# codename0og/codename-rvc-fork-3

Measured on AMD Instinct MI355X. Metric: 48 kHz audio samples/sec end-to-end VC, higher is better.
Workload: dtype f32 (vocoder ResBlock convs and upsamplers, HuBERT, RMVPE's U-Net convs: fp32 operands as exact bf16x3 splits on the bf16 matrix cores -- six products of order <= 2^-16 per multiply-add, fp32 accumulate; everything else fp32 / fp64)

## Files before the change

codename-rvc-fork-3_amd/csrc/decoder.h:

```cpp
#pragma once
#include <atomic>
#include <map>
#include <mutex>
#include <string>
#include <vector>

#include "conv.h"

namespace rvc {

constexpr int MRF_MAX_DIM = 9;

struct HostTensor {
    std::vector<float> data;
    std::vector<int64_t> shape;
    int64_t numel() const { int64_t n = 1; for (auto s : shape) n *= s; return n; }
};

struct DevBuf {
    float *p = nullptr;
    ~DevBuf() { if (p) (void)hipFree(p); }
    int upload(const std::vector<float> &h) {
        if (p) { (void)hipFree(p); p = nullptr; }
        hipError_t e = hipMalloc((void **)&p, h.size() * sizeof(float));
        if (e == hipSuccess) e = hipMemcpy(p, h.data(), h.size() * sizeof(float), hipMemcpyHostToDevice);
        return e == hipSuccess ? 0 : fail("device upload of %zu floats failed: %s", h.size(), hipGetErrorString(e));
    }
};

struct DevBuf16 {
    uint16_t *p = nullptr;
    ~DevBuf16() { if (p) (void)hipFree(p); }
    int upload(const std::vector<uint16_t> &h) {
        if (p) { (void)hipFree(p); p = nullptr; }
        hipError_t e = hipMalloc((void **)&p, h.size() * sizeof(uint16_t));
        if (e == hipSuccess) e = hipMemcpy(p, h.data(), h.size() * sizeof(uint16_t), hipMemcpyHostToDevice);
        return e == hipSuccess ? 0 : fail("device upload of %zu bf16 values failed: %s", h.size(), hipGetErrorString(e));
    }
};

struct ConvW {
    DevBuf w, b;
    DevBuf16 w16;
    DevBuf wu;
    DevBuf16 wu16;
    DevBuf16 wx;
    DevBuf16 wd;
    DevBuf16 wh;
    int c_in = 0, c_out = 0, k = 0;
};

struct Stage {
    int c_in = 0, c_out = 0, rate = 0, ksize = 0, pad = 0, opad = 0;
    int taps = 0;
    bool interleave = false;
    int nc_stride = 0, nc_k = 0, nc_pad = 0;
    int vk = 0, vk_rows = 0;
    int64_t S = 0, P = 0;
    DevBuf w, b;
    DevBuf16 wub;
    int ub_vk = 0;
    int nc_rows = 0;
    DevBuf nc_w;
    std::vector<ConvW> c1, c2;
    std::vector<DevBuf16> pair;
    int pair_splits = 3;
};

constexpr int MAX_BRANCH_LANES = 7;
struct BranchLanes {
    hipStream_t side[MAX_BRANCH_LANES] = {};
    hipEvent_t fork = nullptr;
    hipEvent_t last[MAX_BRANCH_LANES + 1] = {};
    int n_side = 0;
    int create(int n);
    ~BranchLanes();
};

struct RefineStage {
    int ch_in = 0, ch_out = 0, rate = 0, down_c = 0, down_k = 0, down_stride = 0, down_pad = 0;
    DevBuf down_w, down_b;
    ConvW input_conv;
    DevBuf adain1[4], adain2[4];
    std::vector<ConvW> c1, c2;
    std::vector<DevBuf16> pair;
};

}

struct rvc_decoder {
    rvc_decoder_config cfg;
    std::map<std::string, rvc::HostTensor> host;
    bool finalized = false;
    int arithmetic = 0;
    int upp = 1;
    int dim = 1;
    float lin_w[rvc::MRF_MAX_DIM] = {0};
    float lin_b = 0.f;
    rvc::ConvW pre;
    rvc::DevBuf cond_w, cond_b;
    std::vector<rvc::Stage> stages;
    rvc::DevBuf post_w;
    float post_b = 0.f;
    int post_cin = 0;
    float merge_w = 1.f;
    rvc::DevBuf pre_w, pre_b;
    rvc::ConvW mel;
    std::vector<rvc::RefineStage> rstages;
    std::atomic<int> concurrency{0};
    std::atomic<int> branch_parallel{0};
    std::mutex lanes_mu;
    std::map<hipStream_t, rvc::BranchLanes *> lanes;
    ~rvc_decoder() { for (auto &kv : lanes) delete kv.second; }
    int tap_stage = -2;
    float *tap_dev = nullptr;
};


namespace rvc {
const HostTensor *find(const rvc_decoder *d, const std::string &name);
int need(const rvc_decoder *d, const std::string &name, const HostTensor **out, std::vector<int64_t> shape);
int build_conv(const rvc_decoder *d, const std::string &prefix, int c_out, int c_in, int k, bool bias, ConvW *out, bool as_bf16 = false);

int launch_unfold_src(const float *har, int batch, int64_t L, int64_t S, int64_t P, int k_valid, int k_rows, int64_t nq, float *V,
                      hipStream_t stream);
int launch_cond_bias(const float *pre_b, const float *cond_w, const float *cond_b, const float *g, int batch, int gin, int c0,
                     float *out, hipStream_t stream);
int launch_conv_post(const float *x, const float *w, float bias, int batch, int c_in, int64_t L, float slope, float *out,
                     hipStream_t stream);

int refine_finalize(rvc_decoder *d);
size_t refine_workspace_bytes(const rvc_decoder *d, int batch, int64_t T);
int refine_forward(rvc_decoder *d, const float *z_dev, const float *f0_dev, const float *g_dev, const rvc_decoder_noise *noise,
                   int batch, int64_t T, float *out_dev, void *workspace_dev, size_t workspace_bytes, hipStream_t stream);
}
```

codename-rvc-fork-3_amd/csrc/decoder.hip:

```cpp
#include <stdlib.h>

#include "decoder.h"

namespace rvc {


constexpr int CARRY_CHUNK = 4096;
__global__ void __launch_bounds__(256)
nsf_carry_kernel(const float *__restrict__ f0, int64_t T, float sr, float upp, float *__restrict__ carry) {
    __shared__ double pre[CARRY_CHUNK];
    __shared__ double part[257];
    __shared__ double cum_s;
    constexpr int SEG = CARRY_CHUNK / 256;
    const int64_t b = blockIdx.x;
    const float *f = f0 + b * T;
    float *c = carry + b * T;
    if (threadIdx.x == 0) {
        c[0] = 0.f;
        cum_s = 0.0;
    }
    for (int64_t base = 0; base + 1 < T; base += CARRY_CHUNK) {
        const int n = (int)((T - 1 - base) < CARRY_CHUNK ? (T - 1 - base) : CARRY_CHUNK);
        for (int i = threadIdx.x; i < n; i += 256) {
            const float last = __fmul_rn(__fdiv_rn(f[base + i], sr), upp);
            pre[i] = (double)__fsub_rn(fmodf(__fadd_rn(last, 0.5f), 1.0f), 0.5f);
        }
        __syncthreads();
        const int lo = threadIdx.x * SEG, hi = lo + SEG < n ? lo + SEG : n;
        double run = 0.0;
        for (int i = lo; i < hi; ++i) {
            run += pre[i];
            pre[i] = run;
        }
        part[threadIdx.x + 1] = run;
        __syncthreads();
        if (threadIdx.x == 0) {
            double cum = cum_s;
            part[0] = cum;
            for (int i = 1; i <= 256; ++i) {
                cum += part[i];
                part[i] = cum;
            }
            cum_s = cum;
        }
        __syncthreads();
        const double off = part[threadIdx.x];
        for (int i = lo; i < hi; ++i) pre[i] += off;
        __syncthreads();
        for (int i = threadIdx.x; i < n; i += 256) c[base + i + 1] = fmodf((float)pre[i], 1.0f);
        __syncthreads();
    }
}

__global__ void __launch_bounds__(256)
nsf_source_kernel(const float *__restrict__ f0, const float *__restrict__ carry, const float *__restrict__ randn,
                  int64_t T, int upp, float sr, float lin_w, float lin_b, float *__restrict__ har) {
    const int64_t L = T * upp;
    const int64_t b = blockIdx.y;
    const int64_t t = (int64_t)blockIdx.x * blockDim.x + threadIdx.x;
    if (t >= L) return;
    const int64_t i = t / upp;
    const int j = (int)(t - i * upp);
    const float f = f0[b * T + i];
    const float r = __fdiv_rn(f, sr);
    const float phase = __fadd_rn(__fmul_rn(r, (float)(j + 1)), carry[b * T + i]);
    const float sine = __fmul_rn(sinf(__fmul_rn(6.2831853071795864769f, phase)), 0.1f);
    const float uv = f > 0.f ? 1.f : 0.f;
    const float amp = __fadd_rn(__fmul_rn(uv, 0.003f), __fmul_rn(1.f - uv, (float)(0.1 / 3)));
    const float v = __fadd_rn(__fmul_rn(sine, uv), __fmul_rn(amp, randn[b * L + t]));
    har[b * L + t] = tanhf(__fadd_rn(__fmul_rn(v, lin_w), lin_b));
}


struct MrfSrcParams {
    const float *f0; const float *rand_ini; const float *randn; float *har;
    double *p1; double *p2; int *wraps; float *tot_unused;
    int64_t T; int upp; int dim; float sr;
    float lin_w[MRF_MAX_DIM]; float lin_b;
};

__device__ __forceinline__ float mrf_rad(float f0, int h, float sr) {
    const float fh = (h == 0) ? f0 : __fmul_rn(f0, (float)(h + 1));
    const float q = __fdiv_rn(fh, sr);
    return q - floorf(q);
}

constexpr int MRF_CH = 384;
constexpr int MRF_CS = MRF_CH + 1;

template <int PASS>
__device__ __forceinline__ double mrf_prefix_term(const MrfSrcParams &p, int b, int h, int64_t i) {
    const float rho = mrf_rad(p.f0[b * p.T + i], h, p.sr);
    if constexpr (PASS == 1) {
        if (i == 0) {
            const float r0 = __fadd_rn(rho, h == 0 ? 0.f : p.rand_ini[b * p.dim + h]);
            return (double)r0 + (double)(p.upp - 1) * (double)rho;
        }
        return (double)p.upp * (double)rho;
    } else {
        const float rho_m1 = __fadd_rn(rho, -1.0f);
        const int w = p.wraps[((int64_t)b * p.dim + h) * p.T + i];
        if (i == 0) {
            const float r0 = __fadd_rn(rho, h == 0 ? 0.f : p.rand_ini[b * p.dim + h]);
            return (double)r0 + (double)(p.upp - 1 - w) * (double)rho + (double)w * (double)rho_m1;
        }
        return (double)(p.upp - w) * (double)rho + (double)w * (double)rho_m1;
    }
}

template <int PASS>
__global__ void __launch_bounds__(256) mrf_prefix_kernel(MrfSrcParams p) {
    __shared__ double term[MRF_MAX_DIM * MRF_CS];
    const int b = blockIdx.x, tid = threadIdx.x;
    double *const P = (PASS == 1 ? p.p1 : p.p2) + (int64_t)b * p.dim * p.T;
    double cum = 0.0;
    for (int64_t base = 0; base < p.T; base += MRF_CH) {
        const int n = (int)(p.T - base < MRF_CH ? p.T - base : MRF_CH);
        for (int idx = tid; idx < p.dim * n; idx += 256) {
            const int h = idx / n, i = idx - h * n;
            term[h * MRF_CS + i] = mrf_prefix_term<PASS>(p, b, h, base + i);
        }
        __syncthreads();
        if (tid < p.dim) {
            double *row = term + tid * MRF_CS;
            int i = 0;
            for (; i + 8 <= n; i += 8) {
                double v[8];
#pragma unroll
                for (int j = 0; j < 8; ++j) v[j] = row[i + j];
#pragma unroll
                for (int j = 0; j < 8; ++j) {
                    row[i + j] = cum;
                    cum += v[j];
                }
            }
            for (; i < n; ++i) {
                const double v = row[i];
                row[i] = cum;
                cum += v;
            }
        }
        __syncthreads();
        for (int idx = tid; idx < p.dim * n; idx += 256) {
            const int h = idx / n, i = idx - h * n;
            P[(int64_t)h * p.T + base + i] = term[h * MRF_CS + i];
        }
        __syncthreads();
    }
}

__device__ __forceinline__ float mrf_tmp(const MrfSrcParams &p, const double *P1, int b, int h, int64_t i, int j) {
    const float rho = mrf_rad(p.f0[b * p.T + i], h, p.sr);
    double s = P1[i];
    if (i == 0) {
        const float r0 = __fadd_rn(rho, h == 0 ? 0.f : p.rand_ini[b * p.dim + h]);
        s += (double)r0 + (double)j * (double)rho;
    } else {
        s += (double)(j + 1) * (double)rho;
    }
    const float c = (float)s;
    return c - floorf(c);
}

__global__ void __launch_bounds__(64) mrf_wraps_kernel(MrfSrcParams p) {
    const int64_t i = blockIdx.x;
    const int h = blockIdx.y, b = blockIdx.z;
    const double *P1 = p.p1 + ((int64_t)b * p.dim + h) * p.T;
    int cnt = 0;
    for (int j = threadIdx.x; j < p.upp; j += 64) {
        if (i == 0 && j == 0) continue;
        const float cur = mrf_tmp(p, P1, b, h, i, j);
        const float prev = (j == 0) ? mrf_tmp(p, P1, b, h, i - 1, p.upp - 1) : mrf_tmp(p, P1, b, h, i, j - 1);
        if (__fsub_rn(cur, prev) < 0.f) ++cnt;
    }
#pragma unroll
    for (int o = 32; o > 0; o >>= 1) cnt += __shfl_xor(cnt, o);
    if (threadIdx.x == 0) p.wraps[((int64_t)b * p.dim + h) * p.T + i] = cnt;
}


__global__ void __launch_bounds__(256) mrf_source_kernel(MrfSrcParams p) {
    __shared__ int wave_tot[4];
    const int64_t i = blockIdx.x;
    const int b = blockIdx.y;
    const int lane = threadIdx.x & 63, wave = threadIdx.x >> 6;
    const int64_t L = p.T * p.upp;
    const float f = p.f0[b * p.T + i];
    const float uv = f > 0.f ? 1.f : 0.f;
    const float amp = __fadd_rn(__fmul_rn(uv, 0.003f), __fdiv_rn(__fmul_rn(1.f - uv, 0.1f), 3.f));
    const int n_it = (p.upp + 255) / 256;
    float out_acc[4] = {0.f, 0.f, 0.f, 0.f};
    for (int h = 0; h < p.dim; ++h) {
        const double *P1 = p.p1 + ((int64_t)b * p.dim + h) * p.T;
        const double P2 = p.p2[((int64_t)b * p.dim + h) * p.T + i];
        const float rho = mrf_rad(f, h, p.sr);
        const float rho_m1 = __fadd_rn(rho, -1.0f);
        const float r0 = (i == 0) ? __fadd_rn(rho, h == 0 ? 0.f : p.rand_ini[b * p.dim + h]) : rho;
        const float lw = p.lin_w[h];
        int base = 0;
#pragma unroll
        for (int it = 0; it < 4; ++it) {
            if (it < n_it) {
                const int j = it * 256 + threadIdx.x;
                int flag = 0;
                if (j < p.upp && !(i == 0 && j == 0)) {
                    const float cur = mrf_tmp(p, P1, b, h, i, j);
                    const float prev = (j == 0) ? mrf_tmp(p, P1, b, h, i - 1, p.upp - 1) : mrf_tmp(p, P1, b, h, i, j - 1);
                    flag = __fsub_rn(cur, prev) < 0.f ? 1 : 0;
                }
                int incl = flag;
#pragma unroll
                for (int o = 1; o < 64; o <<= 1) {
                    const int v = __shfl_up(incl, o);
                    if (lane >= o) incl += v;
                }
                __syncthreads();
                if (lane == 63) wave_tot[wave] = incl;
                __syncthreads();
                int before = base;
                for (int w = 0; w < wave; ++w) before += wave_tot[w];
                const int total = wave_tot[0] + wave_tot[1] + wave_tot[2] + wave_tot[3];
                const int wcount = before + incl;
                if (j < p.upp) {
                    double s = P2;
                    if (i == 0) s += (double)r0 + (double)(j - wcount) * (double)rho + (double)wcount * (double)rho_m1;
                    else s += (double)(j + 1 - wcount) * (double)rho + (double)wcount * (double)rho_m1;
                    const float c = (float)s;
                    const float sine = __fmul_rn(sinf(__fmul_rn(__fmul_rn(c, 2.f), 3.14159265358979323846f)), 0.1f);
                    const int64_t t = i * p.upp + j;
                    const float nz = p.randn[((int64_t)b * L + t) * p.dim + h];
                    const float v = __fadd_rn(__fmul_rn(sine, uv), __fmul_rn(amp, nz));
                    out_acc[it] = fmaf(v, lw, out_acc[it]);
                }
                base += total;
            }
        }
    }
#pragma unroll
    for (int it = 0; it < 4; ++it) {
        const int j = it * 256 + threadIdx.x;
        if (it < n_it && j < p.upp) p.har[(int64_t)b * L + i * p.upp + j] = tanhf(out_acc[it] + p.lin_b);
    }
}

__global__ void __launch_bounds__(256)
unfold_src_kernel(const float *__restrict__ har, int64_t L, int64_t S, int64_t P, int k_valid, int k_rows, int64_t nq,
                  float *__restrict__ V) {
    const int64_t q = (int64_t)blockIdx.x * blockDim.x + threadIdx.x;
    const int k = blockIdx.y;
    const int64_t b = blockIdx.z;
    if (q >= nq) return;
    float v = 0.f;
    if (k < k_valid) {
        const int64_t idx = q * S + k - P;
        if (idx >= 0 && idx < L) v = har[b * L + idx];
    }
    V[(b * k_rows + k) * nq + q] = v;
}

__global__ void __launch_bounds__(64)
cond_bias_kernel(const float *__restrict__ pre_b, const float *__restrict__ cond_w, const float *__restrict__ cond_b,
                 const float *__restrict__ g, int gin, int c0, float *__restrict__ out) {
    const int co = blockIdx.x, b = blockIdx.y, lane = threadIdx.x;
    float s = 0.f;
    for (int c = lane; c < gin; c += 64) s = fmaf(cond_w[(int64_t)co * gin + c], g[(int64_t)b * gin + c], s);
#pragma unroll
    for (int o = 32; o > 0; o >>= 1) s += __shfl_xor(s, o);
    if (lane == 0) out[(int64_t)b * c0 + co] = pre_b[co] + (cond_b[co] + s);
}

constexpr int POST_OUT = 4;
__global__ void __launch_bounds__(256)
conv_post_kernel(const float *__restrict__ x, const float *__restrict__ w, float bias, int c_in, int64_t L, float slope,
                 float *__restrict__ out) {
    const int64_t b = blockIdx.y;
    const int64_t t0 = ((int64_t)blockIdx.x * blockDim.x + threadIdx.x) * POST_OUT;
    const int64_t blk0 = (int64_t)blockIdx.x * blockDim.x * POST_OUT;
    const float *xb = x + b * c_in * L;
    const bool fast = (L & 3) == 0 && (c_in & 3) == 0 && blk0 >= 4 && blk0 + (int64_t)blockDim.x * POST_OUT + 4 <= L;
    if (fast) {
        float acc[POST_OUT];
#pragma unroll
        for (int o = 0; o < POST_OUT; ++o) acc[o] = bias;
        for (int c0 = 0; c0 < c_in; c0 += 4) {
            f32x4 q[4][3];
#pragma unroll
            for (int u = 0; u < 4; ++u) {
                const f32x4 *xr = reinterpret_cast<const f32x4 *>(xb + (int64_t)(c0 + u) * L + t0 - 4);
#pragma unroll
                for (int j = 0; j < 3; ++j) q[u][j] = xr[j];
            }
#pragma unroll
            for (int u = 0; u < 4; ++u) {
                float v[12];
#pragma unroll
                for (int j = 0; j < 3; ++j)
#pragma unroll
                    for (int e = 0; e < 4; ++e) v[4 * j + e] = q[u][j][e];
#pragma unroll
                for (int i = 1; i < 11; ++i) v[i] = lrelu(v[i], slope);
#pragma unroll
                for (int k = 0; k < 7; ++k) {
                    const float wk = w[(c0 + u) * 7 + k];
#pragma unroll
                    for (int o = 0; o < POST_OUT; ++o) acc[o] = fmaf(wk, v[o + k + 1], acc[o]);
                }
            }
        }
        *reinterpret_cast<f32x4 *>(out + b * L + t0) = f32x4{tanhf(acc[0]), tanhf(acc[1]), tanhf(acc[2]), tanhf(acc[3])};
        return;
    }
    if (t0 >= L) return;
    float acc[POST_OUT];
#pragma unroll
    for (int o = 0; o < POST_OUT; ++o) acc[o] = bias;
    for (int ci = 0; ci < c_in; ++ci) {
        const float *xr = xb + (int64_t)ci * L;
        float v[POST_OUT + 6];
#pragma unroll
        for (int i = 0; i < POST_OUT + 6; ++i) {
            const int64_t tt = t0 + i - 3;
            const int64_t tc = tt < 0 ? 0 : (tt >= L ? L - 1 : tt);
            const float raw = xr[tc];
            v[i] = (tt >= 0 && tt < L) ? lrelu(raw, slope) : 0.f;
        }
#pragma unroll
        for (int k = 0; k < 7; ++k) {
            const float wk = w[ci * 7 + k];
#pragma unroll
            for (int o = 0; o < POST_OUT; ++o) acc[o] = fmaf(wk, v[o + k], acc[o]);
        }
    }
#pragma unroll
    for (int o = 0; o < POST_OUT; ++o)
        if (t0 + o < L) out[b * L + t0 + o] = tanhf(acc[o]);
}

int launch_unfold_src(const float *har, int batch, int64_t L, int64_t S, int64_t P, int k_valid, int k_rows, int64_t nq, float *V,
                      hipStream_t stream) {
    hipLaunchKernelGGL(unfold_src_kernel, dim3((unsigned)ceil_div(nq, 256), k_rows, batch), dim3(256), 0, stream, har, L, S, P,
                       k_valid, k_rows, nq, V);
    RVC_LAUNCH_CHECK();
    return 0;
}

int launch_cond_bias(const float *pre_b, const float *cond_w, const float *cond_b, const float *g, int batch, int gin, int c0,
                     float *out, hipStream_t stream) {
    hipLaunchKernelGGL(cond_bias_kernel, dim3(c0, batch), dim3(64), 0, stream, pre_b, cond_w, cond_b, g, gin, c0, out);
    RVC_LAUNCH_CHECK();
    return 0;
}

int launch_conv_post(const float *x, const float *w, float bias, int batch, int c_in, int64_t L, float slope, float *out,
                     hipStream_t stream) {
    hipLaunchKernelGGL(conv_post_kernel, dim3((unsigned)ceil_div(L, 256 * POST_OUT), batch), dim3(256), 0, stream, x, w, bias, c_in, L, slope,
                       out);
    RVC_LAUNCH_CHECK();
    return 0;
}


}

using namespace rvc;

namespace rvc {
const HostTensor *find(const rvc_decoder *d, const std::string &name) {
    auto it = d->host.find(name);
    return it == d->host.end() ? nullptr : &it->second;
}

int need(const rvc_decoder *d, const std::string &name, const HostTensor **out, std::vector<int64_t> shape) {
    const HostTensor *t = find(d, name);
    if (!t) return fail("decoder: tensor '%s' was never set", name.c_str());
    if (t->shape != shape) {
        std::string got, want;
        for (auto s : t->shape) got += std::to_string(s) + ",";
        for (auto s : shape) want += std::to_string(s) + ",";
        return fail("decoder: tensor '%s' has shape [%s], expected [%s]", name.c_str(), got.c_str(), want.c_str());
    }
    *out = t;
    return 0;
}

int build_conv(const rvc_decoder *d, const std::string &prefix, int c_out, int c_in, int k, bool bias, ConvW *out, bool as_bf16) {
    const HostTensor *w, *b;
    if (need(d, prefix + ".weight", &w, {c_out, c_in, k})) return 1;
    std::vector<float> packed((size_t)c_out * c_in * k);
    for (int co = 0; co < c_out; ++co)
        for (int ci = 0; ci < c_in; ++ci)
            for (int t = 0; t < k; ++t)
                packed[((size_t)t * c_in + ci) * c_out + co] = w->data[((size_t)co * c_in + ci) * k + t];
    if (as_bf16) {
        std::vector<uint16_t> half(packed.size());
        for (size_t i = 0; i < packed.size(); ++i) half[i] = bf16_rne(packed[i]);
        if (out->w16.upload(half)) return 1;
    } else if (out->w.upload(packed)) {
        return 1;
    }
    if (c_in == c_out && c_out % 32 == 0 && wino_supported(k, 1)) {
        if (as_bf16) {
            std::vector<uint32_t> words;
            wino_pack_host_bf16(w->data.data(), c_out, c_in, k, &words);
            std::vector<uint16_t> halves(words.size() * 2);
            memcpy(halves.data(), words.data(), words.size() * 4);
            if (out->wu16.upload(halves)) return 1;
            if (convbf1_supported(c_out, k, 1) && convbf1_preferred(CB1_BF16W, c_out, k)) {
                std::vector<uint16_t> frags;
                convbf1_pack_host(CB1_BF16W, w->data.data(), c_out, k, &frags);
                if (out->wd.upload(frags)) return 1;
            }
            if (winobf_enabled() && winobf_supported(c_in, c_out, k, 1)) {
                std::vector<float> vals((size_t)c_out * c_in * k);
                for (size_t i = 0; i < vals.size(); ++i) {
                    const uint32_t bits = (uint32_t)bf16_rne(w->data[i]) << 16;
                    memcpy(&vals[i], &bits, 4);
                }
                std::vector<uint16_t> frags;
                winobf_pack_host(vals.data(), c_out, c_in, k, &frags);
                if (out->wx.upload(frags)) return 1;
            }
        } else {
            wino_pack_host(w->data.data(), c_out, c_in, k, &packed);
            if (out->wu.upload(packed)) return 1;
            if (d->arithmetic == 1 && convbf1_supported(c_out, k, 1) && convbf1_preferred(CB1_F16X2, c_out, k)) {
                std::vector<uint16_t> frags;
                if (!convbf1_pack_host(CB1_F16X2, w->data.data(), c_out, k, &frags) && out->wh.upload(frags)) return 1;
            }
            if (winobf_enabled() && winobf_supported(c_in, c_out, k, 1)) {
                std::vector<uint16_t> frags;
                winobf_pack_host(w->data.data(), c_out, c_in, k, &frags);
                if (out->wx.upload(frags)) return 1;
            }
        }
    }
    if (c_in != c_out && !as_bf16 && k >= 7 && winobf_enabled() && winobf_supported(c_in, c_out, k, 1)) {
        std::vector<uint16_t> frags;
        winobf_pack_host(w->data.data(), c_out, c_in, k, &frags);
        if (out->wx.upload(frags)) return 1;
    }
    if (bias) {
        if (need(d, prefix + ".bias", &b, {c_out})) return 1;
        if (out->b.upload(b->data)) return 1;
    }
    out->c_in = c_in; out->c_out = c_out; out->k = k;
    return 0;
}
}

extern "C" int rvc_decoder_create(const rvc_decoder_config *cfg, rvc_decoder **out) {
    if (!cfg || !out) return fail("rvc_decoder_create: null pointer");
    if (cfg->kind != RVC_DEC_NSF && cfg->kind != RVC_DEC_MRF && cfg->kind != RVC_DEC_REFINE)
        return fail("rvc_decoder_create: unknown decoder kind %d", cfg->kind);
    if (cfg->n_ups < 1 || cfg->n_ups > 8) return fail("rvc_decoder_create: n_ups out of range");
    if (cfg->n_res_kernels < 1 || cfg->n_res_kernels > 4 || cfg->n_res_dilations < 1 || cfg->n_res_dilations > 4)
        return fail("rvc_decoder_create: resblock configuration out of range");
    if (cfg->weight_storage != 0 && cfg->weight_storage != 1) return fail("rvc_decoder_create: weight_storage must be 0 (fp32) or 1 (bf16)");
    if (cfg->weight_storage == 1 && cfg->kind == RVC_DEC_REFINE)
        return fail("rvc_decoder_create: bf16 weight storage is built for the NSF / MRF decoders (BASELINE cfg 4), not RefineGAN");
    if (cfg->in_channels % 8 || cfg->upsample_initial_channel % (32 << cfg->n_ups))
        return fail("rvc_decoder_create: channel counts must keep every stage a multiple of 32");
    rvc_decoder *d = new rvc_decoder();
    d->cfg = *cfg;
    d->upp = 1;
    for (int i = 0; i < cfg->n_ups; ++i) d->upp *= cfg->upsample_rates[i];
    if (d->upp > 1024) { delete d; return fail("rvc_decoder_create: prod(upsample_rates) > 1024"); }
    d->dim = cfg->kind == RVC_DEC_MRF ? 9 : 1;
    *out = d;
    return 0;
}

extern "C" int rvc_decoder_set_arithmetic(rvc_decoder *dec, int mode) {
    if (!dec) return fail("rvc_decoder_set_arithmetic: null decoder");
    if (mode != 0 && mode != 1) return fail("rvc_decoder_set_arithmetic: mode must be 0 (exact) or 1 (fp16 pairs), got %d", mode);
    if (dec->finalized) return fail("rvc_decoder_set_arithmetic: decoder already finalized (the tap slabs are packed at finalize)");
    if (mode == 1 && dec->cfg.weight_storage == 1)
        return fail("rvc_decoder_set_arithmetic: fp16 pairs are for fp32 taps; a weight_storage = 1 handle's bf16 taps already cost three products");
    dec->arithmetic = mode;
    return 0;
}

extern "C" int rvc_decoder_set_tensor(rvc_decoder *dec, const char *name, const float *data_host, const int64_t *shape,
                                      int ndim) {
    if (!dec || !name || !data_host || !shape || ndim < 1 || ndim > 4) return fail("rvc_decoder_set_tensor: bad argument");
    if (dec->finalized) return fail("rvc_decoder_set_tensor: decoder already finalized");
    HostTensor t;
    t.shape.assign(shape, shape + ndim);
    const int64_t n = t.numel();
    if (n <= 0) return fail("rvc_decoder_set_tensor: empty tensor '%s'", name);
    t.data.assign(data_host, data_host + n);
    dec->host[name] = std::move(t);
    return 0;
}

extern "C" int rvc_decoder_finalize(rvc_decoder *d) {
    if (!d) return fail("rvc_decoder_finalize: null decoder");
    if (d->finalized) return 0;
    if (d->cfg.kind == RVC_DEC_REFINE) {
        if (refine_finalize(d)) return 1;
        d->host.clear();
        d->finalized = true;
        return 0;
    }
    const rvc_decoder_config &c = d->cfg;
    const bool mrf = c.kind == RVC_DEC_MRF;
    const HostTensor *t;
    if (need(d, "m_source.l_linear.weight", &t, {1, d->dim})) return 1;
    for (int h = 0; h < d->dim; ++h) d->lin_w[h] = t->data[h];
    if (need(d, "m_source.l_linear.bias", &t, {1})) return 1;
    d->lin_b = t->data[0];
    const int c0 = c.upsample_initial_channel;
    if (build_conv(d, "conv_pre", c0, c.in_channels, 7, true, &d->pre)) return 1;
    if (need(d, "cond.weight", &t, {c0, c.gin_channels, 1})) return 1;
    if (d->cond_w.upload(t->data)) return 1;
    if (need(d, "cond.bias", &t, {c0})) return 1;
    if (d->cond_b.upload(t->data)) return 1;
    d->stages.clear();
    d->stages.resize(c.n_ups);
    for (int i = 0; i < c.n_ups; ++i) {
        Stage &s = d->stages[i];
        s.c_in = c0 >> i;
        s.c_out = c0 >> (i + 1);
        s.rate = c.upsample_rates[i];
        s.ksize = c.upsample_kernel_sizes[i];
        s.pad = (s.rate % 2 == 0) ? (s.ksize - s.rate) / 2 : s.rate / 2 + s.rate % 2;
        s.opad = s.rate % 2;
        s.taps = (s.ksize + s.rate - 1) / s.rate;
        if (s.taps > 2) return fail("decoder: upsample kernel %d with rate %d needs %d polyphase taps (max 2)", s.ksize, s.rate, s.taps);
        if (s.taps < 2) s.taps = 2;
        int stride_f0 = 1;
        for (int j = i + 1; j < c.n_ups; ++j) stride_f0 *= c.upsample_rates[j];
        s.nc_stride = stride_f0;
        s.nc_k = stride_f0 == 1 ? 1 : stride_f0 * 2 - stride_f0 % 2;
        s.nc_pad = stride_f0 == 1 ? 0 : (s.nc_k - stride_f0) / 2;
        s.vk = (s.rate - 1) * s.nc_stride + s.nc_k;
        s.vk_rows = (s.vk + 7) / 8 * 8;
        s.S = (int64_t)s.rate * s.nc_stride;
        s.P = (int64_t)s.pad * s.nc_stride + s.nc_pad;
        static const int nc_sep_env = knob("RVC_NC_SEPARATE", 1);
        const bool nc_separate = nc_sep_env && s.vk_rows * 2 >= s.c_in;
        if (nc_separate) {
            s.nc_rows = (s.nc_k + 7) / 8 * 8;
            s.vk = 0;
            s.vk_rows = 0;
        }

        const std::string up = (mrf ? "upsamples." : "ups.") + std::to_string(i);
        const std::string nc = "noise_convs." + std::to_string(i);
        const HostTensor *uw, *ub, *nw, *nb;
        if (need(d, up + ".weight", &uw, {s.c_in, s.c_out, s.ksize})) return 1;
        if (need(d, up + ".bias", &ub, {s.c_out})) return 1;
        if (need(d, nc + ".weight", &nw, {s.c_out, 1, s.nc_k})) return 1;
        if (need(d, nc + ".bias", &nb, {s.c_out})) return 1;
        const int ctot = s.c_in + s.vk_rows;
        const int m_total = s.rate * s.c_out;
        s.interleave = s.rate % 2 == 0;
        auto mrow = [&](int ph, int co) { return s.interleave ? co * s.rate + ph : ph * s.c_out + co; };
        std::vector<float> packed((size_t)s.taps * ctot * m_total, 0.f);
        for (int tp = 0; tp < s.taps; ++tp) {
            const int j = s.taps - 1 - tp;
            for (int ci = 0; ci < s.c_in; ++ci)
                for (int ph = 0; ph < s.rate; ++ph) {
                    const int kk = ph + j * s.rate;
                    if (kk >= s.ksize) continue;
                    for (int co = 0; co < s.c_out; ++co)
                        packed[((size_t)tp * ctot + ci) * m_total + mrow(ph, co)] =
                            uw->data[((size_t)ci * s.c_out + co) * s.ksize + kk];
                }
        }
        const int tp0 = s.taps - 1;
        for (int kq = 0; kq < s.vk; ++kq)
            for (int ph = 0; ph < s.rate; ++ph) {
                const int k = kq - ph * s.nc_stride;
                if (k < 0 || k >= s.nc_k) continue;
                for (int co = 0; co < s.c_out; ++co)
                    packed[((size_t)tp0 * ctot + s.c_in + kq) * m_total + mrow(ph, co)] = nw->data[(size_t)co * s.nc_k + k];
            }
        if (s.w.upload(packed)) return 1;
        std::vector<float> bias(s.c_out);
        for (int co = 0; co < s.c_out; ++co) bias[co] = ub->data[co] + nb->data[co];
        {
            static const int ups_bf = knob("RVC_UPS_BF", 1);
            const int k_n = s.nc_rows > 0 ? 0 : s.nc_k;
            const int vk = upsbf_fold_noise(k_n) ? (s.rate - 1) * s.nc_stride + k_n : 0;
            if (ups_bf && s.opad == 0 && s.rate * s.c_out >= 128 && upsbf_supported(s.c_in, s.c_out, s.rate, s.ksize, vk)) {
                std::vector<uint16_t> frags;
                upsbf_pack_host(uw->data.data(), k_n ? nw->data.data() : nullptr, bias.data(), s.c_in, s.c_out, s.rate, s.ksize, vk, k_n, s.nc_stride, &frags);
                if (s.wub.upload(frags)) return 1;
                s.ub_vk = vk;
            }
        }
        if (s.nc_rows) {
            std::vector<float> ncw((size_t)s.nc_rows * s.c_out, 0.f);
            for (int k = 0; k < s.nc_k; ++k)
                for (int co = 0; co < s.c_out; ++co) ncw[(size_t)k * s.c_out + co] = nw->data[(size_t)co * s.nc_k + k];
            if (s.nc_w.upload(ncw)) return 1;
        }
        if (s.b.upload(bias)) return 1;

        const int nb_ = c.n_res_kernels * c.n_res_dilations;
        s.c1 = std::vector<ConvW>(nb_);
        s.c2 = std::vector<ConvW>(nb_);
        s.pair = std::vector<DevBuf16>(nb_);
        for (int m = 0; m < c.n_res_kernels; ++m)
            for (int j = 0; j < c.n_res_dilations; ++j) {
                std::string p1, p2;
                if (mrf) {
                    const std::string base = "mrfs." + std::to_string(i) + "." + std::to_string(m) + ".layers." + std::to_string(j);
                    p1 = base + ".conv1";
                    p2 = base + ".conv2";
                } else {
                    const std::string base = "resblocks." + std::to_string(i * c.n_res_kernels + m);
                    p1 = base + ".convs1." + std::to_string(j);
                    p2 = base + ".convs2." + std::to_string(j);
                }
                const int k = c.res_kernel_sizes[m];
                const bool b16 = c.weight_storage == 1 && (k == 3 || k == 7 || k == 11);
                if (build_conv(d, p1, s.c_out, s.c_out, k, true, &s.c1[m * c.n_res_dilations + j], b16)) return 1;
                if (build_conv(d, p2, s.c_out, s.c_out, k, true, &s.c2[m * c.n_res_dilations + j], b16)) return 1;
                const int nts = b16 ? 1 : 3;
                if (resblock_bf_enabled() && resblock_bf_supported(s.c_out, k, 1) && resblock_bf_preferred(s.c_out, k, nts)) {
                    const HostTensor *w1, *w2;
                    if (need(d, p1 + ".weight", &w1, {s.c_out, s.c_out, k}) || need(d, p2 + ".weight", &w2, {s.c_out, s.c_out, k})) return 1;
                    std::vector<uint16_t> frags;
                    resblock_bf_pack_host(w1->data.data(), w2->data.data(), s.c_out, k, &frags, nts);
                    s.pair_splits = nts;
                    if (s.pair[m * c.n_res_dilations + j].upload(frags)) return 1;
                }
            }
    }
    d->post_cin = c0 >> c.n_ups;
    if (need(d, "conv_post.weight", &t, {1, d->post_cin, 7})) return 1;
    if (d->post_w.upload(t->data)) return 1;
    d->post_b = 0.f;
    if (mrf) {
        if (need(d, "conv_post.bias", &t, {1})) return 1;
        d->post_b = t->data[0];
    }
    d->host.clear();
    d->finalized = true;
    return 0;
}

extern "C" int rvc_decoder_destroy(rvc_decoder *dec) {
    delete dec;
    return 0;
}

extern "C" int rvc_decoder_upp(const rvc_decoder *dec) { return dec ? dec->upp : 0; }

namespace {
struct Carve {
    size_t off = 0;
    size_t take(size_t bytes) { size_t o = off; off += align_up(bytes, 256); return o; }
};
struct Layout {
    size_t har, carry, biasp, V, p1, p2, wraps, buf[2 + 2 * (MAX_BRANCH_LANES + 1)], total;
    int n_buf;
    int64_t max_cl;
};
constexpr int64_t BRANCH_PARALLEL_MAX_ELEMS = (int64_t)3 * 256 * 128 * 256;
int branch_lanes_wanted(const rvc_decoder *d) {
    const int nk = d->cfg.n_res_kernels, want = d->branch_parallel.load(std::memory_order_relaxed);
    const int most = nk - 1 < MAX_BRANCH_LANES ? nk - 1 : MAX_BRANCH_LANES;
    return want < 0 || want > most ? most : want;
}
Layout make_layout(const rvc_decoder *d, int batch, int64_t T) {
    Layout l;
    Carve c;
    const int64_t L = T * d->upp;
    l.har = c.take((size_t)batch * L * 4);
    l.carry = c.take((size_t)batch * T * 4);
    l.biasp = c.take((size_t)batch * d->cfg.upsample_initial_channel * 4);
    int64_t len = T, max_cl = (int64_t)d->cfg.upsample_initial_channel * T, max_v = 0;
    for (const Stage &s : d->stages) {
        const int64_t nq = len + 1;
        max_v = std::max<int64_t>(max_v, (int64_t)s.vk_rows * nq);
        len = (len - 1) * s.rate - 2 * s.pad + s.ksize + s.opad;
        max_v = std::max<int64_t>(max_v, (int64_t)s.nc_rows * len);
        max_cl = std::max<int64_t>(max_cl, (int64_t)s.c_out * len);
    }
    l.V = c.take((size_t)batch * max_v * 4);
    const size_t scan = d->dim > 1 ? (size_t)batch * d->dim * T : 0;
    l.p1 = c.take(scan * 8);
    l.p2 = c.take(scan * 8);
    l.wraps = c.take(scan * 4);
    l.n_buf = 2 + 2 * (branch_lanes_wanted(d) + 1);
    for (int i = 0; i < l.n_buf; ++i) l.buf[i] = c.take((size_t)batch * max_cl * 4);
    l.total = c.off;
    l.max_cl = max_cl;
    return l;
}
}

extern "C" int rvc_decoder_workspace_bytes(const rvc_decoder *dec, int batch, int64_t n_frames, size_t *bytes) {
    if (!dec || !bytes || batch <= 0 || n_frames <= 0) return fail("rvc_decoder_workspace_bytes: bad argument");
    if (!dec->finalized) return fail("rvc_decoder_workspace_bytes: decoder not finalized");
    *bytes = dec->cfg.kind == RVC_DEC_REFINE ? refine_workspace_bytes(dec, batch, n_frames) : make_layout(dec, batch, n_frames).total;
    return 0;
}

extern "C" int rvc_decoder_set_tap(rvc_decoder *dec, int stage, float *tap_dev) {
    if (!dec) return fail("rvc_decoder_set_tap: null decoder");
    dec->tap_stage = tap_dev ? stage : -2;
    dec->tap_dev = tap_dev;
    return 0;
}

int rvc::BranchLanes::create(int n) {
    n_side = n;
    for (int i = 0; i < n; ++i) RVC_HIP(hipStreamCreateWithFlags(&side[i], hipStreamNonBlocking));
    RVC_HIP(hipEventCreateWithFlags(&fork, hipEventDisableTiming));
    for (int i = 0; i <= MAX_BRANCH_LANES; ++i) RVC_HIP(hipEventCreateWithFlags(&last[i], hipEventDisableTiming));
    return 0;
}
rvc::BranchLanes::~BranchLanes() {
    for (int i = 0; i < n_side; ++i) if (side[i]) { (void)hipStreamSynchronize(side[i]); (void)hipStreamDestroy(side[i]); }
    if (fork) (void)hipEventDestroy(fork);
    for (int i = 0; i <= MAX_BRANCH_LANES; ++i) if (last[i]) (void)hipEventDestroy(last[i]);
}

namespace {
int lanes_for(rvc_decoder *d, hipStream_t stream, int n_side, BranchLanes **out) {
    std::lock_guard<std::mutex> g(d->lanes_mu);
    BranchLanes *&l = d->lanes[stream];
    if (l && l->n_side != n_side) { delete l; l = nullptr; }
    if (!l) {
        l = new BranchLanes();
        if (l->create(n_side)) { delete l; l = nullptr; return 1; }
    }
    *out = l;
    return 0;
}
}

extern "C" int rvc_decoder_set_branch_parallel(rvc_decoder *dec, int side_streams) {
    if (!dec) return fail("rvc_decoder_set_branch_parallel: null decoder");
    dec->branch_parallel.store(side_streams, std::memory_order_relaxed);
    return 0;
}

extern "C" int rvc_decoder_set_concurrency_hint(rvc_decoder *dec, int utterances_in_flight) {
    if (!dec) return fail("rvc_decoder_set_concurrency_hint: null decoder");
    if (utterances_in_flight < 0) return fail("rvc_decoder_set_concurrency_hint: negative hint %d", utterances_in_flight);
    dec->concurrency.store(utterances_in_flight, std::memory_order_relaxed);
    return 0;
}

extern "C" int rvc_decoder_forward(rvc_decoder *d, const float *z_dev, const float *f0_dev, const float *g_dev,
                                   const rvc_decoder_noise *noise, int batch, int64_t T, float *out_dev,
                                   void *workspace_dev, size_t workspace_bytes, void *stream_) {
    if (!d || !z_dev || !f0_dev || !g_dev || !noise || !out_dev || !workspace_dev) return fail("rvc_decoder_forward: null pointer");
    ConcurrencyScope scope(d->concurrency.load(std::memory_order_relaxed));
    if (!d->finalized) return fail("rvc_decoder_forward: decoder not finalized");
    if (batch <= 0 || T <= 0) return fail("rvc_decoder_forward: empty batch");
    if (!noise->src_randn_dev) return fail("rvc_decoder_forward: src_randn_dev is required");
    if (d->cfg.kind == RVC_DEC_REFINE)
        return refine_forward(d, z_dev, f0_dev, g_dev, noise, batch, T, out_dev, workspace_dev, workspace_bytes, (hipStream_t)stream_);
    const rvc_decoder_config &c = d->cfg;
    const bool mrf = c.kind == RVC_DEC_MRF;
    if (mrf && !noise->src_rand_dev) return fail("rvc_decoder_forward: src_rand_dev is required for the MRF decoder");
    hipStream_t stream = (hipStream_t)stream_;
    const Layout lay = make_layout(d, batch, T);
    if (workspace_bytes < lay.total) return fail("rvc_decoder_forward: workspace too small (%zu < %zu)", workspace_bytes, lay.total);
    char *ws = (char *)workspace_dev;
    float *har = (float *)(ws + lay.har);
    float *carry = (float *)(ws + lay.carry);
    float *biasp = (float *)(ws + lay.biasp);
    float *V = (float *)(ws + lay.V);
    float *buf[2 + 2 * (MAX_BRANCH_LANES + 1)];
    for (int i = 0; i < lay.n_buf; ++i) buf[i] = (float *)(ws + lay.buf[i]);
    const int n_side = (lay.n_buf - 4) / 2;
    BranchLanes *lanes = nullptr;
    if (n_side > 0 && lanes_for(d, stream, n_side, &lanes)) return 1;
    const int64_t L = T * d->upp;
    const float sr = (float)c.sample_rate;

    if (!mrf) {
        hipLaunchKernelGGL(nsf_carry_kernel, dim3(batch), dim3(256), 0, stream, f0_dev, T, sr, (float)d->upp, carry);
        RVC_LAUNCH_CHECK();
        hipLaunchKernelGGL(nsf_source_kernel, dim3((unsigned)ceil_div(L, 256), batch), dim3(256), 0, stream, f0_dev, carry,
                           noise->src_randn_dev, T, d->upp, sr, d->lin_w[0], d->lin_b, har);
        RVC_LAUNCH_CHECK();
    } else {
        MrfSrcParams sp;
        sp.f0 = f0_dev; sp.rand_ini = noise->src_rand_dev; sp.randn = noise->src_randn_dev; sp.har = har;
        sp.p1 = (double *)(ws + lay.p1); sp.p2 = (double *)(ws + lay.p2); sp.wraps = (int *)(ws + lay.wraps);
        sp.tot_unused = nullptr;
        sp.T = T; sp.upp = d->upp; sp.dim = d->dim; sp.sr = sr;
        for (int h = 0; h < MRF_MAX_DIM; ++h) sp.lin_w[h] = d->lin_w[h];
        sp.lin_b = d->lin_b;
        hipLaunchKernelGGL(mrf_prefix_kernel<1>, dim3(batch), dim3(256), 0, stream, sp);
        RVC_LAUNCH_CHECK();
        hipLaunchKernelGGL(mrf_wraps_kernel, dim3((unsigned)T, d->dim, batch), dim3(64), 0, stream, sp);
        RVC_LAUNCH_CHECK();
        hipLaunchKernelGGL(mrf_prefix_kernel<3>, dim3(batch), dim3(256), 0, stream, sp);
        RVC_LAUNCH_CHECK();
        hipLaunchKernelGGL(mrf_source_kernel, dim3((unsigned)T, batch), dim3(256), 0, stream, sp);
        RVC_LAUNCH_CHECK();
    }
    if (d->tap_stage == -1 && d->tap_dev)
        RVC_HIP(hipMemcpyAsync(d->tap_dev, har, (size_t)batch * L * 4, hipMemcpyDeviceToDevice, stream));

    const int c0 = c.upsample_initial_channel;
    hipLaunchKernelGGL(cond_bias_kernel, dim3(c0, batch), dim3(64), 0, stream, d->pre.b.p, d->cond_w.p, d->cond_b.p, g_dev,
                       c.gin_channels, c0, biasp);
    RVC_LAUNCH_CHECK();
    float *cur = buf[0];
    {
        ConvParams p;
        p.x1 = z_dev; p.c1 = c.in_channels; p.slope1 = 1.f; p.x1_bstride = (int64_t)c.in_channels * T; p.l_in = T;
        p.w = d->pre.w.p; p.bias = biasp; p.bias_bstride = c0;
        p.y = cur; p.y_bstride = (int64_t)c0 * T; p.m_total = c0; p.c_out = c0; p.n_cols = T; p.l_out = T;
        p.kw = 7; p.dil = 1; p.padl = 3; p.batch = batch;
        if (launch_conv(p, stream)) return 1;
    }

    int64_t len = T;
    const int nd = c.n_res_dilations, nk = c.n_res_kernels;
    for (int i = 0; i < c.n_ups; ++i) {
        Stage &s = d->stages[i];
        const int64_t nq = len + 1;
        const int64_t len_out = (len - 1) * s.rate - 2 * s.pad + s.ksize + s.opad;
        float *X = buf[1];
        if (s.wub.p && fits_2gib((int64_t)s.c_in * len, 4) && fits_2gib((int64_t)s.c_out * len_out, 4) && fits_2gib(L, 4)) {
            if (launch_upsbf(cur, har, L, s.wub.p, s.b.p, X, batch, s.c_in, s.c_out, len, len_out, s.rate, s.ksize, s.pad, s.ub_vk, s.S, s.P, 0.1f, stream))
                return 1;
        } else {
        if (s.vk_rows) {
            hipLaunchKernelGGL(unfold_src_kernel, dim3((unsigned)ceil_div(nq, 256), s.vk_rows, batch), dim3(256), 0, stream, har, L,
                               s.S, s.P, s.vk, s.vk_rows, nq, V);
            RVC_LAUNCH_CHECK();
        }
        {
            ConvParams p;
            p.x1 = cur; p.c1 = s.c_in; p.slope1 = 0.1f; p.x1_bstride = (int64_t)s.c_in * len;
            if (s.vk_rows) { p.x2 = V; p.c2 = s.vk_rows; p.slope2 = 1.f; p.x2_bstride = (int64_t)s.vk_rows * nq; }
            p.l_in = len;
            p.w = s.w.p; p.bias = s.b.p;
            p.y = X; p.y_bstride = (int64_t)s.c_out * len_out;
            p.m_total = s.rate * s.c_out; p.c_out = s.c_out; p.n_cols = nq; p.l_out = len_out;
            p.kw = s.taps; p.dil = 1; p.padl = s.taps - 1;
            p.up_stride = s.rate; p.up_pad = s.pad; p.up_interleave = s.interleave ? 1 : 0; p.batch = batch;
            p.l_in2 = nq;
            if (launch_conv(p, stream)) return 1;
        }
        }
        if (s.nc_rows) {
            hipLaunchKernelGGL(unfold_src_kernel, dim3((unsigned)ceil_div(len_out, 256), s.nc_rows, batch), dim3(256), 0, stream, har,
                               L, (int64_t)s.nc_stride, (int64_t)s.nc_pad, s.nc_k, s.nc_rows, len_out, V);
            RVC_LAUNCH_CHECK();
            ConvParams p;
            p.x1 = V; p.c1 = s.nc_rows; p.slope1 = 1.f; p.x1_bstride = (int64_t)s.nc_rows * len_out; p.l_in = len_out;
            p.w = s.nc_w.p; p.accin = X; p.y = X; p.y_bstride = (int64_t)s.c_out * len_out;
            p.m_total = s.c_out; p.c_out = s.c_out; p.n_cols = len_out; p.l_out = len_out;
            p.kw = 1; p.dil = 1; p.padl = 0; p.batch = batch;
            if (launch_conv(p, stream)) return 1;
        }
        len = len_out;
        const int64_t bs = (int64_t)s.c_out * len;
        const bool short_stage = (int64_t)batch * bs <= BRANCH_PARALLEL_MAX_ELEMS;
        const bool par = lanes && short_stage;
        if (par) {
            RVC_HIP(hipEventRecord(lanes->fork, stream));
            for (int q = 0; q < n_side; ++q) RVC_HIP(hipStreamWaitEvent(lanes->side[q], lanes->fork, 0));
        }
        const hipStream_t main_stream = stream;
        for (int r = 0; r < nk; ++r) {
            const int m = r;
            const bool first_branch = r == 0, final_branch = r + 1 == nk;
            const int k = c.res_kernel_sizes[m];
            const float *xin = X;
            const int off = nk - 1 - n_side;
            const int lane = par && r > off ? r - off : 0, lane_prev = par && r - 1 > off ? r - 1 - off : 0;
            const hipStream_t stream = lane > 0 ? lanes->side[lane - 1] : main_stream;
            float *const Y = buf[2 + 2 * lane], *const T1 = buf[3 + 2 * lane];
            auto before_last = [&]() -> int {
                if (par && r > 0 && lane_prev != lane) RVC_HIP(hipStreamWaitEvent(stream, lanes->last[r - 1], 0));
                return 0;
            };
            auto after_last = [&]() -> int {
                if (par) RVC_HIP(hipEventRecord(lanes->last[r], stream));
                return 0;
            };
            bool f16_branch = true;
            for (int j = 0; j < nd; ++j) f16_branch = f16_branch && s.c1[m * nd + j].wh.p && s.c2[m * nd + j].wh.p;
            if (s.pair[m * nd].p && !f16_branch && resblock_bf_fits(s.c_out, len)) {
                for (int j = 0; j < nd; ++j) {
                    const bool last = j + 1 == nd;
                    float *yout = last ? cur : (j % 2 == 0 ? Y : T1);
                    const float *acc_in = (last && !first_branch) ? cur : nullptr;
                    const float scale = (last && final_branch) ? 1.f / (float)nk : 1.f;
                    if (last && before_last()) return 1;
                    if (launch_resblock_bf(xin, s.pair[m * nd + j].p, s.c1[m * nd + j].b.p, s.c2[m * nd + j].b.p, acc_in, yout, batch,
                                           s.c_out, len, k, c.res_dilations[j], 0.1f, scale, stream, s.pair_splits))
                        return 1;
                    xin = yout;
                }
                if (after_last()) return 1;
                continue;
            }
            if (resblock_layer_supported(s.c_out, k) && !s.c1[m * nd].w16.p) {
                for (int j = 0; j < nd; ++j) {
                    const bool last = j + 1 == nd;
                    float *yout = last ? cur : (j % 2 == 0 ? Y : T1);
                    const float *acc_in = (last && !first_branch) ? cur : nullptr;
                    const float scale = (last && final_branch) ? 1.f / (float)nk : 1.f;
                    if (last && before_last()) return 1;
                    if (launch_resblock_layer(xin, s.c1[m * nd + j].w.p, s.c1[m * nd + j].b.p, s.c2[m * nd + j].w.p,
                                              s.c2[m * nd + j].b.p, acc_in, yout, batch, s.c_out, len, k, c.res_dilations[j], 0.1f,
                                              scale, stream))
                        return 1;
                    xin = yout;
                }
                if (after_last()) return 1;
                continue;
            }
            for (int j = 0; j < nd; ++j) {
                const int dil = c.res_dilations[j];
                ConvParams p;
                p.x1 = xin; p.c1 = s.c_out; p.slope1 = 0.1f; p.x1_bstride = bs; p.l_in = len;
                p.w = s.c1[m * nd + j].w.p; p.w16 = s.c1[m * nd + j].w16.p; p.bias = s.c1[m * nd + j].b.p; p.w_wino = s.c1[m * nd + j].wu.p; p.w_winobf = s.c1[m * nd + j].wx.p; p.w_direct1 = s.c1[m * nd + j].wd.p; p.w_f16x2 = s.c1[m * nd + j].wh.p;
                p.w_wino16 = reinterpret_cast<const uint32_t *>(s.c1[m * nd + j].wu16.p);
                p.y = T1; p.y_bstride = bs; p.m_total = s.c_out; p.c_out = s.c_out; p.n_cols = len; p.l_out = len;
                p.kw = k; p.dil = dil; p.padl = (k - 1) / 2 * dil; p.batch = batch;
                if (launch_conv(p, stream)) return 1;
                ConvParams q;
                q.x1 = T1; q.c1 = s.c_out; q.slope1 = 0.1f; q.x1_bstride = bs; q.l_in = len;
                q.w = s.c2[m * nd + j].w.p; q.w16 = s.c2[m * nd + j].w16.p; q.bias = s.c2[m * nd + j].b.p; q.w_wino = s.c2[m * nd + j].wu.p; q.w_winobf = s.c2[m * nd + j].wx.p; q.w_direct1 = s.c2[m * nd + j].wd.p; q.w_f16x2 = s.c2[m * nd + j].wh.p;
                q.w_wino16 = reinterpret_cast<const uint32_t *>(s.c2[m * nd + j].wu16.p);
                q.res = xin;
                q.y_bstride = bs; q.m_total = s.c_out; q.c_out = s.c_out; q.n_cols = len; q.l_out = len;
                q.kw = k; q.dil = 1; q.padl = (k - 1) / 2;  q.batch = batch;
                if (j + 1 < nd) {
                    q.y = Y;
                } else {
                    q.y = cur;
                    q.accin = first_branch ? nullptr : cur;
                    q.out_scale = final_branch ? 1.f / (float)nk : 1.f;
                    if (before_last()) return 1;
                }
                if (launch_conv(q, stream)) return 1;
                xin = Y;
            }
            if (after_last()) return 1;
        }
        if (par) RVC_HIP(hipStreamWaitEvent(main_stream, lanes->last[nk - 1], 0));
        if (d->tap_stage == i && d->tap_dev)
            RVC_HIP(hipMemcpyAsync(d->tap_dev, cur, (size_t)batch * bs * 4, hipMemcpyDeviceToDevice, stream));
    }
    if (len != L) return fail("decoder: internal length mismatch (%lld vs %lld)", (long long)len, (long long)L);
    return launch_conv_post(cur, d->post_w.p, d->post_b, batch, d->post_cin, L, 0.01f, out_dev, stream);
}
```

codename-rvc-fork-3_amd/rvc_amd/_native.py:

```python
from __future__ import annotations

import ctypes
import threading
import os
from ctypes import POINTER, c_char_p, c_float, c_int, c_int64, c_size_t, c_void_p

import torch

_HERE = os.path.dirname(os.path.abspath(__file__))
LIB_PATH = os.path.join(_HERE, "_lib", "librvc_amd.so")
if os.environ.get("RVC_AMD_LIB"):
    LIB_PATH = os.path.abspath(os.environ["RVC_AMD_LIB"])
    print(f"[rvc_amd] RVC_AMD_LIB: loading {LIB_PATH} instead of the product library", flush=True)


class NativeError(RuntimeError):
    pass


if not os.path.isfile(LIB_PATH):
    raise ImportError(
        f"{LIB_PATH} is missing: build it with `python -c 'import __graft_entry__ as g; g.build()'` "
        "(hipcc --offload-arch=gfx950).  rvc_amd has no fallback path without its HIP library.")

_lib = ctypes.CDLL(LIB_PATH)


class DecoderConfig(ctypes.Structure):
    _fields_ = [
        ("kind", c_int), ("sample_rate", c_int), ("in_channels", c_int), ("upsample_initial_channel", c_int),
        ("gin_channels", c_int), ("n_ups", c_int), ("upsample_rates", c_int * 8), ("upsample_kernel_sizes", c_int * 8),
        ("n_res_kernels", c_int), ("res_kernel_sizes", c_int * 4), ("res_dilations", c_int * 4),
        ("n_res_dilations", c_int), ("weight_storage", c_int),
    ]


class DecoderNoise(ctypes.Structure):
    _fields_ = [("src_rand_dev", c_void_p), ("src_randn_dev", c_void_p), ("adain_randn_dev", c_void_p)]


SYMBOLS = {
    "rvc_abi_version": (c_int, []),
    "rvc_last_error": (c_char_p, []),
    "rvc_knn_index_aux_bytes": (c_int, [c_int64, c_int, POINTER(c_size_t)]),
    "rvc_knn_index_build": (c_int, [c_void_p, c_int64, c_int, c_void_p, c_size_t, c_void_p]),
    "rvc_knn_set_mode": (c_int, [c_int]),
    "rvc_knn_rank_candidates": (c_int, [c_void_p, c_void_p, c_int64, c_int, c_void_p, c_int64, c_void_p, c_int, c_int, c_void_p,
                                        c_void_p, c_void_p]),
    "rvc_knn_workspace_bytes": (c_int, [c_int64, c_int64, c_int, c_int, POINTER(c_size_t)]),
    "rvc_knn_search": (c_int, [c_void_p, c_void_p, c_int64, c_int, c_void_p, c_int64, c_int, c_void_p, c_void_p,
                               c_void_p, c_size_t, c_void_p]),
    "rvc_knn_blend": (c_int, [c_void_p, c_int, c_void_p, c_void_p, c_void_p, c_int64, c_int, c_float, c_void_p,
                              c_void_p]),
    "rvc_logmel_workspace_bytes": (c_int, [c_int, c_int64, POINTER(c_size_t)]),
    "rvc_logmel_rmvpe": (c_int, [c_void_p, c_int, c_int64, c_void_p, c_int64, c_void_p, c_size_t, c_void_p]),
    "rvc_mel_create": (c_int, [c_int, c_int, c_int, c_int, c_float, c_float, c_void_p, c_int, POINTER(c_void_p)]),
    "rvc_mel_destroy": (c_int, [c_void_p]),
    "rvc_mel_frames": (c_int, [c_void_p, c_int64, POINTER(c_int64)]),
    "rvc_mel_workspace_bytes": (c_int, [c_void_p, c_int, c_int64, POINTER(c_size_t)]),
    "rvc_mel_forward": (c_int, [c_void_p, c_void_p, c_int, c_int64, c_void_p, c_void_p, c_void_p, c_size_t, c_void_p]),
    "rvc_resample_poly_f64": (c_int, [c_void_p, c_int64, c_int, c_int, c_void_p, c_int64, c_void_p, c_int64, c_void_p]),
    "rvc_filtfilt_workspace_bytes": (c_int, [c_int64, POINTER(c_size_t)]),
    "rvc_filtfilt_order5": (c_int, [c_void_p, c_int64, c_void_p, c_void_p, c_void_p, c_size_t, c_void_p]),
    "rvc_bigru_workspace_bytes": (c_int, [c_int, POINTER(c_size_t)]),
    "rvc_bigru_forward": (c_int, [c_void_p, c_void_p, c_void_p, c_void_p, c_int, c_int64, c_int, c_void_p, c_size_t,
                                  c_void_p]),
    "rvc_bigru_status": (c_int, [c_void_p, c_int, POINTER(c_int), c_void_p]),
    "rvc_bigru_set_spin_limit": (c_int, [ctypes.c_uint]),
    "rvc_attention_workspace_bytes": (c_int, [c_int, c_int64, c_int, c_int, POINTER(c_size_t)]),
    "rvc_attention_qkv_f32": (c_int, [c_void_p, c_void_p, c_void_p, c_void_p, c_int, c_int64, c_int, c_int, c_float,
                                      c_void_p, c_size_t, c_void_p]),
    "rvc_bias_relu_add_f32": (c_int, [c_void_p, c_void_p, c_void_p, c_void_p, c_int, c_int, c_int64, c_int, c_void_p]),
    "rvc_gate_tanh_sigmoid_f32": (c_int, [c_void_p, c_void_p, c_int, c_int, c_int64, c_void_p]),
    "rvc_rownorm_gelu_f32": (c_int, [c_void_p, c_void_p, c_void_p, c_void_p, c_int, c_int, c_int64, ctypes.c_float, c_void_p]),
    "rvc_set_concurrency_hint": (c_int, [c_int]),
    "rvc_decoder_create": (c_int, [POINTER(DecoderConfig), POINTER(c_void_p)]),
    "rvc_decoder_set_tensor": (c_int, [c_void_p, c_char_p, c_void_p, POINTER(c_int64), c_int]),
    "rvc_decoder_finalize": (c_int, [c_void_p]),
    "rvc_decoder_destroy": (c_int, [c_void_p]),
    "rvc_decoder_upp": (c_int, [c_void_p]),
    "rvc_decoder_workspace_bytes": (c_int, [c_void_p, c_int, c_int64, POINTER(c_size_t)]),
    "rvc_decoder_forward": (c_int, [c_void_p, c_void_p, c_void_p, c_void_p, POINTER(DecoderNoise), c_int, c_int64,
                                    c_void_p, c_void_p, c_size_t, c_void_p]),
    "rvc_decoder_set_tap": (c_int, [c_void_p, c_int, c_void_p]),
    "rvc_decoder_set_concurrency_hint": (c_int, [c_void_p, c_int]),
    "rvc_decoder_set_branch_parallel": (c_int, [c_void_p, c_int]),
    "rvc_posconv_bf16x3_weight_bytes": (c_int, [c_int, c_int, c_int, POINTER(c_size_t)]),
    "rvc_posconv_bf16x3_pack_weight": (c_int, [c_void_p, c_int, c_int, c_int, c_void_p, c_void_p]),
    "rvc_posconv_gelu_bf16x3": (c_int, [c_void_p, c_void_p, c_void_p, c_void_p, c_int64, c_int, c_int, c_int, c_int, c_void_p]),
    "rvc_hubert_conv0_workspace_bytes": (c_int, [c_int, POINTER(c_size_t)]),
    "rvc_hubert_conv0_frames_bf16x3": (c_int, [c_void_p, c_int64, c_void_p, c_int, c_int, c_int, c_void_p, c_void_p, c_float, c_void_p,
                                               c_size_t, c_void_p, c_int64, c_void_p]),
    "rvc_conv1d_frames_bf16x3": (c_int, [c_void_p, c_int64, c_int64, c_int, c_int, c_int, c_void_p, c_void_p, c_void_p, c_void_p, c_int64,
                                         c_int, c_int, c_void_p]),
    "rvc_conv1d_pack_weight": (c_int, [c_void_p, c_int, c_int, c_int, c_void_p, c_void_p]),
    "rvc_conv1d_forward": (c_int, [c_void_p, c_void_p, c_void_p, c_void_p, c_void_p, c_void_p, c_int, c_int, c_int,
                                   c_int64, c_int, c_int, c_float, c_float, c_void_p]),
    "rvc_conv1d_wino_pack_weight": (c_int, [c_void_p, c_int, c_int, c_int, c_void_p, c_void_p]),
    "rvc_conv1d_wino_forward": (c_int, [c_void_p, c_void_p, c_void_p, c_void_p, c_void_p, c_void_p, c_int, c_int, c_int,
                                        c_int64, c_int, c_int, c_float, c_float, c_void_p]),
    "rvc_conv1d_winobf_weight_bytes": (c_int, [c_int, c_int, c_int, POINTER(c_size_t)]),
    "rvc_conv1d_winobf_pack_weight": (c_int, [c_void_p, c_int, c_int, c_int, c_void_p, c_void_p]),
    "rvc_conv1d_winobf_forward": (c_int, [c_void_p, c_void_p, c_void_p, c_void_p, c_void_p, c_void_p, c_int, c_int, c_int,
                                          c_int64, c_int, c_int, c_float, c_float, c_void_p]),
    "rvc_resblock_bf16x3_weight_bytes": (c_int, [c_int, c_int, POINTER(c_size_t)]),
    "rvc_resblock_bf16x3_pack_weight": (c_int, [c_void_p, c_void_p, c_int, c_int, c_void_p, c_void_p]),
    "rvc_resblock_bf16x3_forward": (c_int, [c_void_p, c_void_p, c_void_p, c_void_p, c_void_p, c_void_p, c_int, c_int, c_int64, c_int,
                                            c_int, c_float, c_float, c_void_p]),
    "rvc_resblock_bf16w_weight_bytes": (c_int, [c_int, c_int, POINTER(c_size_t)]),
    "rvc_resblock_bf16w_pack_weight": (c_int, [c_void_p, c_void_p, c_int, c_int, c_void_p, c_void_p]),
    "rvc_resblock_bf16w_forward": (c_int, [c_void_p, c_void_p, c_void_p, c_void_p, c_void_p, c_void_p, c_int, c_int, c_int64, c_int,
                                           c_int, c_float, c_float, c_void_p]),
    "rvc_resblock_bf16x3_set_enabled": (c_int, [c_int]),
    "rvc_upsample_bf16x3_weight_bytes": (c_int, [c_int, c_int, c_int, c_int, c_int, c_int, POINTER(c_size_t)]),
    "rvc_upsample_bf16x3_pack_weight": (c_int, [c_void_p, c_void_p, c_void_p, c_int, c_int, c_int, c_int, c_int, c_int, c_void_p, c_void_p]),
    "rvc_upsample_bf16x3_forward": (c_int, [c_void_p, c_void_p, c_int64, c_void_p, c_void_p, c_void_p, c_int, c_int, c_int, c_int64, c_int, c_int,
                                            c_int, c_int, c_int, c_int, c_float, c_void_p]),
    "rvc_conv1d_f16x2_weight_bytes": (c_int, [c_int, c_int, POINTER(c_size_t)]),
    "rvc_conv1d_f16x2_pack_weight": (c_int, [c_void_p, c_int, c_int, c_void_p, c_void_p]),
    "rvc_conv1d_f16x2_forward": (c_int, [c_void_p, c_void_p, c_void_p, c_void_p, c_void_p, c_void_p, c_int, c_int, c_int64, c_int,
                                         c_int, c_float, c_float, c_void_p]),
    "rvc_decoder_set_arithmetic": (c_int, [c_void_p, c_int]),
    "rvc_conv1d_bf16w_weight_bytes": (c_int, [c_int, c_int, POINTER(c_size_t)]),
    "rvc_conv1d_bf16w_pack_weight": (c_int, [c_void_p, c_int, c_int, c_void_p, c_void_p]),
    "rvc_conv1d_bf16w_forward": (c_int, [c_void_p, c_void_p, c_void_p, c_void_p, c_void_p, c_void_p, c_int, c_int, c_int64, c_int,
                                         c_int, c_float, c_float, c_void_p]),
    "rvc_gemm_bf16x3_weight_bytes": (c_int, [c_int, c_int, POINTER(c_size_t)]),
    "rvc_gemm_bf16x3_pack_weight": (c_int, [c_void_p, c_int, c_int, c_int, c_void_p, c_void_p]),
    "rvc_linear_bf16x3": (c_int, [c_void_p, c_void_p, c_void_p, c_void_p, c_void_p, c_int64, c_int, c_int, c_int, c_void_p]),
    "rvc_conv1d_bf16x3": (c_int, [c_void_p, c_void_p, c_void_p, c_void_p, c_int, c_int, c_int, c_int64, c_int, c_int, c_int, c_int,
                                  c_void_p]),
    "rvc_split_rows_bf16x3": (c_int, [c_void_p, c_void_p, c_int64, c_int64, c_int, c_void_p]),
    "rvc_linear_bf16x3_presplit": (c_int, [c_void_p, c_void_p, c_void_p, c_void_p, c_void_p, c_int64, c_int64, c_int, c_int, c_int, c_int,
                                           c_void_p]),
    "rvc_bias_residual_layernorm_bf16x3": (c_int, [c_void_p, c_int, c_void_p, c_void_p, c_void_p, c_void_p, c_float, c_void_p, c_void_p,
                                                   c_int64, c_int64, c_int, c_void_p]),
    "rvc_conv2d_packed_floats": (c_int, [c_int, c_int, c_int, c_int, POINTER(c_size_t)]),
    "rvc_conv2d_pack_weight": (c_int, [c_void_p, c_int, c_int, c_int, c_int, c_void_p, c_void_p]),
    "rvc_conv2d_workspace_bytes": (c_int, [c_int, c_int, c_int, c_int, c_int, c_int, c_int, POINTER(c_size_t)]),
    "rvc_conv2d_bf16x3_supported": (c_int, [c_int, c_int, c_int, c_int]),
    "rvc_conv2d_bf16x3_weight_bytes": (c_int, [c_int, c_int, c_int, c_int, POINTER(c_size_t)]),
    "rvc_conv2d_bf16x3_pack_weight": (c_int, [c_void_p, c_int, c_int, c_int, c_int, c_void_p, c_void_p]),
    "rvc_conv2d_bf16x3_workspace_bytes": (c_int, [c_int, c_int, c_int, c_int, c_int, POINTER(c_size_t)]),
    "rvc_conv2d_bf16x3_forward": (c_int, [c_void_p, c_void_p, c_void_p, c_void_p, c_void_p, c_int, c_int, c_int, c_int, c_int, c_int,
                                          c_void_p, c_size_t, c_void_p]),
    "rvc_conv2d_forward": (c_int, [c_void_p, c_void_p, c_void_p, c_void_p, c_void_p, c_int, c_int, c_int, c_int, c_int, c_int,
                                   c_int, c_int, c_void_p, c_size_t, c_void_p]),
    "rvc_comm_unique_id": (c_int, [c_void_p]),
    "rvc_comm_create": (c_int, [c_void_p, c_int, c_int, POINTER(c_void_p)]),
    "rvc_comm_destroy": (c_int, [c_void_p]),
    "rvc_comm_info": (c_int, [c_void_p, POINTER(c_int), POINTER(c_int), POINTER(c_int), c_char_p, c_size_t]),
    "rvc_index_broadcast": (c_int, [c_void_p, c_void_p, c_size_t, c_int, c_void_p]),
    "rvc_checksum64": (c_int, [c_void_p, c_size_t, c_void_p, c_void_p]),
    "rvc_glu_dwconv_silu_f32": (c_int, [c_void_p, c_void_p, c_void_p, c_void_p, c_int64, c_int, c_int, c_void_p]),
    "rvc_layernorm_rows_f32": (c_int, [c_void_p, c_void_p, c_void_p, c_float, c_void_p, c_int64, c_int, c_void_p]),
    "rvc_groupnorm_workspace_bytes": (c_int, [c_int, c_int64, c_int, POINTER(c_size_t)]),
    "rvc_groupnorm_lrelu_f32": (c_int, [c_void_p, c_void_p, c_void_p, c_int, c_float, c_float, c_void_p, c_int, c_int64, c_void_p,
                                        c_size_t, c_void_p]),
    "rvc_fcpe_decode_f32": (c_int, [c_void_p, c_void_p, c_int, c_int, c_float, c_float, c_void_p, c_void_p, c_int64, c_void_p]),
    "rvc_kmeans_workspace_bytes": (c_int, [c_int64, c_int64, c_int, POINTER(c_size_t)]),
    "rvc_kmeans_assign": (c_int, [c_void_p, c_int64, c_int, c_void_p, c_int64, c_void_p, c_void_p, c_void_p, c_size_t, c_void_p]),
    "rvc_kmeans_update": (c_int, [c_void_p, c_int64, c_int, c_void_p, c_void_p, c_int64, c_void_p, c_void_p, c_void_p, c_size_t,
                                  c_void_p]),
}

for _name, (_res, _args) in SYMBOLS.items():
    _fn = getattr(_lib, _name)
    _fn.restype = _res
    _fn.argtypes = _args

ABI_VERSION = 4
if _lib.rvc_abi_version() != ABI_VERSION:
    raise ImportError(f"librvc_amd.so ABI {_lib.rvc_abi_version()} != {ABI_VERSION}: rebuild it")


def _check(rc: int, what: str):
    if rc != 0:
        raise NativeError(f"{what}: {_lib.rvc_last_error().decode(errors='replace')}")


def _stream() -> int:
    return torch.cuda.current_stream().cuda_stream


def _dev_f32(t: torch.Tensor, name: str) -> torch.Tensor:
    if not t.is_cuda:
        raise NativeError(f"{name} must live in HBM (got a {t.device} tensor); the HIP path has no CPU fallback")
    if t.dtype != torch.float32:
        raise NativeError(f"{name} must be float32, got {t.dtype}")
    return t.contiguous()


class _Workspace:

    def __init__(self):
        self._buf = {}
        self._lock = threading.Lock()

    def get(self, tag: str, nbytes: int, device) -> torch.Tensor:
        key = (tag, str(device), torch.cuda.current_stream(device).cuda_stream)
        with self._lock:
            buf = self._buf.get(key)
            if buf is None or buf.numel() < nbytes:
                buf = torch.empty(max(nbytes, 256), dtype=torch.uint8, device=device)
                self._buf[key] = buf
        return buf


_ws = _Workspace()


def knn_index_build(index: torch.Tensor) -> torch.Tensor:
    index = _dev_f32(index, "index")
    need = c_size_t()
    _check(_lib.rvc_knn_index_aux_bytes(index.shape[0], index.shape[1], ctypes.byref(need)), "rvc_knn_index_aux_bytes")
    aux = torch.empty(need.value, dtype=torch.uint8, device=index.device)
    _check(_lib.rvc_knn_index_build(index.data_ptr(), index.shape[0], index.shape[1], aux.data_ptr(), aux.numel(), _stream()),
           "rvc_knn_index_build")
    return aux


knn_index_norms = knn_index_build


def knn_set_mode(mode: int) -> None:
    _check(_lib.rvc_knn_set_mode(int(mode)), "rvc_knn_set_mode")


def knn_search(index: torch.Tensor, aux: torch.Tensor, queries: torch.Tensor, k: int = 8):
    index, queries = _dev_f32(index, "index"), _dev_f32(queries, "queries")
    if not aux.is_cuda or aux.dtype != torch.uint8:
        raise NativeError("aux must be the uint8 HBM blob returned by knn_index_build")
    nq = queries.shape[0]
    d2 = torch.empty((nq, k), dtype=torch.float32, device=index.device)
    ids = torch.empty((nq, k), dtype=torch.int64, device=index.device)
    if nq == 0:
        return d2, ids
    need = c_size_t()
    _check(_lib.rvc_knn_workspace_bytes(index.shape[0], nq, index.shape[1], k, ctypes.byref(need)), "rvc_knn_workspace_bytes")
    ws = _ws.get("knn", need.value, index.device)
    _check(_lib.rvc_knn_search(index.data_ptr(), aux.data_ptr(), index.shape[0], index.shape[1], queries.data_ptr(),
                               nq, k, d2.data_ptr(), ids.data_ptr(), ws.data_ptr(), ws.numel(), _stream()),
           "rvc_knn_search")
    return d2, ids


def knn_rank_candidates(index: torch.Tensor, aux: torch.Tensor, queries: torch.Tensor, cand: torch.Tensor, k: int = 8):
    index, queries = _dev_f32(index, "index"), _dev_f32(queries, "queries")
    if not cand.is_cuda or cand.dtype != torch.int32 or cand.dim() != 2 or cand.shape[0] != queries.shape[0]:
        raise NativeError("cand must be an int32 HBM tensor [n_queries, cap]")
    cand = cand.contiguous()
    nq = queries.shape[0]
    d2 = torch.empty((nq, k), dtype=torch.float32, device=index.device)
    ids = torch.empty((nq, k), dtype=torch.int64, device=index.device)
    _check(_lib.rvc_knn_rank_candidates(index.data_ptr(), aux.data_ptr(), index.shape[0], index.shape[1], queries.data_ptr(), nq,
                                        cand.data_ptr(), cand.shape[1], k, d2.data_ptr(), ids.data_ptr(), _stream()),
           "rvc_knn_rank_candidates")
    return d2, ids


def knn_blend(index: torch.Tensor, feats: torch.Tensor, d2: torch.Tensor, ids: torch.Tensor, index_rate: float):
    index, feats, d2 = _dev_f32(index, "index"), _dev_f32(feats, "feats"), _dev_f32(d2, "d2")
    ids = ids.contiguous()
    out = torch.empty_like(feats)
    _check(_lib.rvc_knn_blend(index.data_ptr(), index.shape[1], feats.data_ptr(), d2.data_ptr(), ids.data_ptr(),
                              feats.shape[0], d2.shape[1], float(index_rate), out.data_ptr(), _stream()),
           "rvc_knn_blend")
    return out


def _kmeans_workspace(n_rows: int, n_centroids: int, dim: int, device) -> torch.Tensor:
    need = c_size_t()
    _check(_lib.rvc_kmeans_workspace_bytes(n_rows, n_centroids, dim, ctypes.byref(need)), "rvc_kmeans_workspace_bytes")
    return _ws.get("kmeans", need.value, device)


def kmeans_assign(x: torch.Tensor, centroids: torch.Tensor):
    x, centroids = _dev_f32(x, "x"), _dev_f32(centroids, "centroids")
    if x.dim() != 2 or centroids.dim() != 2 or x.shape[1] != centroids.shape[1]:
        raise NativeError(f"x {tuple(x.shape)} and centroids {tuple(centroids.shape)} must be [n, d] and [k, d]")
    n, d = x.shape
    ids = torch.empty(n, dtype=torch.int32, device=x.device)
    d2 = torch.empty(n, dtype=torch.float32, device=x.device)
    if n == 0:
        return ids, d2
    ws = _kmeans_workspace(n, centroids.shape[0], d, x.device)
    _check(_lib.rvc_kmeans_assign(x.data_ptr(), n, d, centroids.data_ptr(), centroids.shape[0], ids.data_ptr(), d2.data_ptr(),
                                  ws.data_ptr(), ws.numel(), _stream()), "rvc_kmeans_assign")
    return ids, d2


def kmeans_update(x: torch.Tensor, order: torch.Tensor, offsets: torch.Tensor, old: torch.Tensor) -> torch.Tensor:
    x, old = _dev_f32(x, "x"), _dev_f32(old, "old")
    n, d = x.shape
    k = old.shape[0]
    if (not order.is_cuda or order.dtype != torch.int32 or order.numel() != n or not offsets.is_cuda
            or offsets.dtype != torch.int64 or offsets.numel() != k + 1 or old.shape[1] != d):
        raise NativeError("order must be an int32 HBM tensor [n], offsets an int64 HBM tensor [k + 1], old [k, d]")
    if n == 0:
        return old.clone()
    order, offsets = order.contiguous(), offsets.contiguous()
    out = torch.empty_like(old)
    ws = _kmeans_workspace(n, k, d, x.device)
    _check(_lib.rvc_kmeans_update(x.data_ptr(), n, d, order.data_ptr(), offsets.data_ptr(), k, old.data_ptr(), out.data_ptr(),
                                  ws.data_ptr(), ws.numel(), _stream()), "rvc_kmeans_update")
    return out


def knn_roofline_report(n_rows: int, n_queries: int, dim: int, seconds: float, peak_hbm_gbs: float,
                        peak_f32_tflops: float, peak_f16_tflops: float, traffic=None, traffic_source=None) -> dict:
    screened = n_queries > 64 and n_rows >= 16384 and dim % 256 == 0
    stream = n_queries <= 64
    q_tile = 256 if screened else (32 if stream else 128)
    passes = -(-n_queries // q_tile)
    bytes_8d = passes * n_rows * dim * 4.0
    bytes_moved = passes * n_rows * dim * (2.0 if screened else 4.0) + (8.0 * n_queries * dim * 4 if screened else 0.0)
    flops = 2.0 * n_queries * n_rows * dim
    mfma_peak = peak_f16_tflops if screened else peak_f32_tflops
    hbm_gbs = bytes_moved / seconds / 1e9
    mfma_tf = flops / seconds / 1e12
    bound = "hbm" if stream else "mfma"
    out = {"kernel": ("knn_screen_kernel<false> (sample) + knn_select_kernel + knn_screen_kernel<true> (main, fp16 MFMA) + "
                      "knn_finalize_kernel (exact fp32 re-scoring)" if screened else
                      ("knn_direct_kernel" if stream else "knn_partial_kernel") + " + knn_finalize_kernel"),
           "regime": "fp16-screened, exact re-scoring" if screened else ("fp32 streaming" if stream else "fp32 GEMM"),
           "shape": f"{n_queries} queries x {n_rows} rows x {dim}", "bound": bound, "query_tile": q_tile, "passes": passes,
           "bytes_per_pass_8d": n_rows * dim * 4}
    if bound == "hbm":
        out.update({"achieved": round(hbm_gbs, 1), "peak": peak_hbm_gbs, "unit": "GB/s", "frac": round(hbm_gbs / peak_hbm_gbs, 4),
                    "frac_is": "physical: bytes the pass reads (n_rows x dim x 4) / search time / HBM peak"})
    else:
        out.update({"achieved": round(mfma_tf, 2), "peak": mfma_peak, "unit": "TFLOP/s", "frac": round(mfma_tf / mfma_peak, 4),
                    "frac_is": "2 x queries x rows x dim / search time / the dense " + ("fp16" if screened else "fp32") + " MFMA peak "
                               "(round 5 and earlier printed an HBM fraction here: now hbm_frac_physical / frac_8d)"})
    out.update({"bytes_moved_per_search": bytes_moved,
                "hbm_gbs_physical": round(hbm_gbs, 1), "hbm_frac_physical": round(hbm_gbs / peak_hbm_gbs, 4),
                "achieved_8d": round(bytes_8d / seconds / 1e9, 1), "frac_8d": round(bytes_8d / seconds / 1e9 / peak_hbm_gbs, 4),
                "frac_8d_is": "SURVEY 8d's formula (passes x n_rows x dim x 4 B / t / 8 TB/s): fp32 bytes the screened kernel never reads -- a footnote",
                "traffic": traffic, "traffic_source": traffic_source,
                "mfma_tflops": round(mfma_tf, 2), "mfma_frac": round(mfma_tf / mfma_peak, 4),
                "mfma_peak_used": "fp16 dense 2500 TF" if screened else "fp32 157.3 TF",
                "avg_search_ms": round(seconds * 1e3, 4)})
    return out


def logmel_rmvpe(audio: torch.Tensor, pad_to: int = 32) -> tuple[torch.Tensor, int]:
    audio = _dev_f32(audio, "audio")
    b, n = audio.shape
    t = n // 160 + 1
    t_pad = pad_to * ((t - 1) // pad_to + 1) if pad_to > 1 else t
    mel = torch.empty((b, 128, t_pad), dtype=torch.float32, device=audio.device)
    need = c_size_t()
    _check(_lib.rvc_logmel_workspace_bytes(b, n, ctypes.byref(need)), "rvc_logmel_workspace_bytes")
    ws = _ws.get("logmel", need.value, audio.device)
    _check(_lib.rvc_logmel_rmvpe(audio.data_ptr(), b, n, mel.data_ptr(), t_pad, ws.data_ptr(), ws.numel(), _stream()),
           "rvc_logmel_rmvpe")
    return mel, t


class MelTransform:

    def __init__(self, n_fft: int, hop: int, win_length: int, pad: int, mel_matrix, mag_eps: float = 0.0, log_floor: float = 1e-5):
        import numpy as np
        m = np.ascontiguousarray(mel_matrix, dtype=np.float32)
        if m.ndim != 2 or m.shape[1] != n_fft // 2 + 1:
            raise NativeError(f"mel matrix must be [n_mels, {n_fft // 2 + 1}], got {m.shape}")
        self.n_fft, self.hop, self.n_mels, self.bins = n_fft, hop, m.shape[0], n_fft // 2 + 1
        self._h = c_void_p()
        _check(_lib.rvc_mel_create(n_fft, hop, win_length, pad, float(mag_eps), float(log_floor), m.ctypes.data, m.shape[0],
                                   ctypes.byref(self._h)), "rvc_mel_create")

    def __del__(self):
        if getattr(self, "_h", None) and _lib is not None:
            _lib.rvc_mel_destroy(self._h)
            self._h = None

    def n_frames(self, n_samples: int) -> int:
        t = c_int64()
        _check(_lib.rvc_mel_frames(self._h, n_samples, ctypes.byref(t)), "rvc_mel_frames")
        return t.value

    def forward(self, audio: torch.Tensor, want_mel: bool = True, want_spec: bool = False):
        audio = _dev_f32(audio, "audio")
        b, n = audio.shape
        t = self.n_frames(n)
        mel = torch.empty((b, self.n_mels, t), dtype=torch.float32, device=audio.device) if want_mel else None
        spec = torch.empty((b, self.bins, t), dtype=torch.float32, device=audio.device) if want_spec else None
        need = c_size_t()
        _check(_lib.rvc_mel_workspace_bytes(self._h, b, n, ctypes.byref(need)), "rvc_mel_workspace_bytes")
        ws = _ws.get("mel", need.value, audio.device)
        _check(_lib.rvc_mel_forward(self._h, audio.data_ptr(), b, n, mel.data_ptr() if mel is not None else None,
                                    spec.data_ptr() if spec is not None else None, ws.data_ptr(), ws.numel(), _stream()),
               "rvc_mel_forward")
        return mel, spec


def resample_poly(x: torch.Tensor, up: int, down: int, h: torch.Tensor) -> torch.Tensor:
    if not (x.is_cuda and x.dtype == torch.float64 and x.dim() == 1 and h.is_cuda and h.dtype == torch.float64):
        raise NativeError("resample_poly wants 1-D float64 HBM tensors")
    x, h = x.contiguous(), h.contiguous()
    n_out = -(-x.numel() * up // down)
    y = torch.empty(n_out, dtype=torch.float64, device=x.device)
    _check(_lib.rvc_resample_poly_f64(x.data_ptr(), x.numel(), int(up), int(down), h.data_ptr(), h.numel(), y.data_ptr(), n_out,
                                      _stream()), "rvc_resample_poly_f64")
    return y


_ff_coef_cache = {}


def _filtfilt_coef(b, a):
    import numpy as np
    from scipy import signal
    key = (tuple(b), tuple(a))
    if key not in _ff_coef_cache:
        b = np.asarray(b, dtype=np.float64)
        a = np.asarray(a, dtype=np.float64)
        assert b.shape == (6,) and a.shape == (6,) and a[0] == 1.0
        _ff_coef_cache[key] = np.ascontiguousarray(np.concatenate([b, a, signal.lfilter_zi(b, a)]))
    return _ff_coef_cache[key]


def filtfilt_order5(x: torch.Tensor, b, a) -> torch.Tensor:
    if not x.is_cuda or x.dtype != torch.float64 or x.dim() != 1:
        raise NativeError("filtfilt_order5 wants a 1-D float64 HBM tensor")
    x = x.contiguous()
    coef = _filtfilt_coef(b, a)
    y = torch.empty_like(x)
    need = c_size_t()
    _check(_lib.rvc_filtfilt_workspace_bytes(x.numel(), ctypes.byref(need)), "rvc_filtfilt_workspace_bytes")
    ws = _ws.get("filtfilt", need.value, x.device)
    _check(_lib.rvc_filtfilt_order5(x.data_ptr(), x.numel(), coef.ctypes.data, y.data_ptr(), ws.data_ptr(),
                                    ws.numel(), _stream()), "rvc_filtfilt_order5")
    return y


def bigru_forward(gi: torch.Tensor, whh_t: torch.Tensor, bhh: torch.Tensor, multi_cu: bool = True) -> torch.Tensor:
    gi, whh_t, bhh = _dev_f32(gi, "gi"), _dev_f32(whh_t, "whh_t"), _dev_f32(bhh, "bhh")
    b, t = gi.shape[0], gi.shape[1]
    out = torch.empty((b, t, 512), dtype=torch.float32, device=gi.device)
    ws_ptr, ws_bytes = None, 0
    if multi_cu:
        need = c_size_t()
        _check(_lib.rvc_bigru_workspace_bytes(b, ctypes.byref(need)), "rvc_bigru_workspace_bytes")
        ws = _ws.get("bigru", need.value, gi.device)
        ws_ptr, ws_bytes = ws.data_ptr(), ws.numel()
    _check(_lib.rvc_bigru_forward(gi.data_ptr(), whh_t.data_ptr(), bhh.data_ptr(), out.data_ptr(), b, t, 256, ws_ptr,
                                  ws_bytes, _stream()), "rvc_bigru_forward")
    return out


def bigru_redone(batch: int = 1, device=None) -> int:
    device = device if device is not None else torch.device("cuda", torch.cuda.current_device())
    need = c_size_t()
    _check(_lib.rvc_bigru_workspace_bytes(batch, ctypes.byref(need)), "rvc_bigru_workspace_bytes")
    ws = _ws.get("bigru", need.value, device)
    n = c_int()
    _check(_lib.rvc_bigru_status(ws.data_ptr(), batch, ctypes.byref(n), _stream()), "rvc_bigru_status")
    return n.value


def bigru_set_spin_limit(polls: int) -> None:
    _check(_lib.rvc_bigru_set_spin_limit(int(polls)), "rvc_bigru_set_spin_limit")


def attention_qkv(qkv: torch.Tensor, n_heads: int, scale: float, emb_rel_k: torch.Tensor = None,
                  emb_rel_v: torch.Tensor = None) -> torch.Tensor:
    assert qkv.is_cuda and qkv.dtype == torch.float32 and qkv.is_contiguous() and qkv.dim() == 3
    b, t, c = qkv.shape
    hd = c // (3 * n_heads)
    rel = emb_rel_k is not None
    if rel:
        for e in (emb_rel_k, emb_rel_v):
            assert e.is_cuda and e.dtype == torch.float32 and e.is_contiguous() and tuple(e.shape) == (21, hd)
    out = torch.empty(b, t, n_heads * hd, dtype=torch.float32, device=qkv.device)
    need = c_size_t()
    _check(_lib.rvc_attention_workspace_bytes(b, t, n_heads, hd, ctypes.byref(need)), "rvc_attention_workspace_bytes")
    ws = _ws.get("attention", need.value, qkv.device)
    _check(_lib.rvc_attention_qkv_f32(qkv.data_ptr(), emb_rel_k.data_ptr() if rel else None,
                                      emb_rel_v.data_ptr() if rel else None, out.data_ptr(), b, t, n_heads, hd,
                                      float(scale), ws.data_ptr(), ws.numel(), _stream()), "rvc_attention_qkv_f32")
    return out


def bias_relu_add_(x: torch.Tensor, bias: torch.Tensor = None, res: torch.Tensor = None, relu: bool = True) -> torch.Tensor:
    assert x.is_cuda and x.dtype == torch.float32 and x.is_contiguous() and x.dim() >= 3
    b, c = x.shape[0], x.shape[1]
    inner = x.numel() // (b * c)
    if res is not None:
        assert res.is_cuda and res.dtype == torch.float32 and res.is_contiguous() and res.shape == x.shape
    _check(_lib.rvc_bias_relu_add_f32(x.data_ptr(), bias.data_ptr() if bias is not None else None,
                                      res.data_ptr() if res is not None else None, x.data_ptr(), b, c, inner, int(relu),
                                      _stream()), "rvc_bias_relu_add_f32")
    return x


def rownorm_gelu_(x: torch.Tensor, gamma: torch.Tensor = None, beta: torch.Tensor = None, eps: float = 1e-5) -> torch.Tensor:
    assert x.is_cuda and x.dtype == torch.float32 and x.is_contiguous() and x.dim() == 3
    b, c, length = x.shape
    _check(_lib.rvc_rownorm_gelu_f32(x.data_ptr(), gamma.data_ptr() if gamma is not None else None,
                                     beta.data_ptr() if beta is not None else None, x.data_ptr(), b, c, length, float(eps), _stream()),
           "rvc_rownorm_gelu_f32")
    return x


def gate_tanh_sigmoid(x: torch.Tensor) -> torch.Tensor:
    assert x.is_cuda and x.dtype == torch.float32 and x.is_contiguous() and x.dim() == 3 and x.shape[1] % 2 == 0
    b, c2, t = x.shape
    out = torch.empty(b, c2 // 2, t, dtype=torch.float32, device=x.device)
    _check(_lib.rvc_gate_tanh_sigmoid_f32(x.data_ptr(), out.data_ptr(), b, c2 // 2, t, _stream()), "rvc_gate_tanh_sigmoid_f32")
    return out


def set_concurrency_hint(utterances_in_flight: int) -> None:
    _check(_lib.rvc_set_concurrency_hint(int(utterances_in_flight)), "rvc_set_concurrency_hint")


COMM_ID_BYTES = 128


def comm_unique_id() -> bytes:
    buf = ctypes.create_string_buffer(COMM_ID_BYTES)
    _check(_lib.rvc_comm_unique_id(buf), "rvc_comm_unique_id")
    return buf.raw


class Comm:

    def __init__(self, unique_id: bytes, n_ranks: int, rank: int):
        assert len(unique_id) == COMM_ID_BYTES
        self._h = c_void_p()
        _check(_lib.rvc_comm_create(ctypes.create_string_buffer(unique_id, COMM_ID_BYTES), int(n_ranks), int(rank),
                                    ctypes.byref(self._h)), "rvc_comm_create")

    def info(self) -> dict:
        n, r, v = c_int(), c_int(), c_int()
        path = ctypes.create_string_buffer(512)
        _check(_lib.rvc_comm_info(self._h, ctypes.byref(n), ctypes.byref(r), ctypes.byref(v), path, 512), "rvc_comm_info")
        return {"n_ranks": n.value, "rank": r.value, "rccl_version": v.value, "library": path.value.decode()}

    def broadcast_(self, t: torch.Tensor, root: int = 0) -> torch.Tensor:
        if not t.is_cuda or not t.is_contiguous():
            raise NativeError("Comm.broadcast_ wants a contiguous HBM tensor")
        _check(_lib.rvc_index_broadcast(self._h, t.data_ptr(), t.numel() * t.element_size(), int(root), _stream()),
               "rvc_index_broadcast")
        return t

    def destroy(self):
        h, self._h = self._h, None
        if h:
            _check(_lib.rvc_comm_destroy(h), "rvc_comm_destroy")

    def __del__(self):
        if getattr(self, "_h", None) and _lib is not None:
            _lib.rvc_comm_destroy(self._h)
            self._h = None


def checksum64(t: torch.Tensor) -> torch.Tensor:
    if not t.is_cuda or not t.is_contiguous():
        raise NativeError("checksum64 wants a contiguous HBM tensor")
    out = torch.empty(2, dtype=torch.int64, device=t.device)
    _check(_lib.rvc_checksum64(t.data_ptr(), t.numel() * t.element_size(), out.data_ptr(), _stream()), "rvc_checksum64")
    return out


def conv1d_pack_weight(w: torch.Tensor, device) -> torch.Tensor:
    w = w.detach().float().cpu().contiguous()
    packed = torch.empty(w.numel(), dtype=torch.float32, device=device)
    _check(_lib.rvc_conv1d_pack_weight(w.data_ptr(), w.shape[0], w.shape[1], w.shape[2], packed.data_ptr(), _stream()),
           "rvc_conv1d_pack_weight")
    return packed


def conv1d_forward(x, w_packed, bias, c_out, k, dilation=1, slope_in=1.0, res=None, acc=None, out_scale=1.0):
    return conv1d_forward_into(x, w_packed, bias, c_out, k, dilation, slope_in, res=res, acc=acc, out_scale=out_scale)


def conv1d_forward_into(x, w_packed, bias, c_out, k, dilation=1, slope_in=1.0, res=None, acc=None, out_scale=1.0, out=None):
    x = _dev_f32(x, "x")
    b, c_in, length = x.shape
    y = out if out is not None else torch.empty((b, c_out, length), dtype=torch.float32, device=x.device)
    _check(_lib.rvc_conv1d_forward(x.data_ptr(), w_packed.data_ptr(), bias.data_ptr() if bias is not None else None,
                                   res.data_ptr() if res is not None else None,
                                   acc.data_ptr() if acc is not None else None, y.data_ptr(), b, c_in, c_out, length, k,
                                   dilation, float(slope_in), float(out_scale), _stream()), "rvc_conv1d_forward")
    return y


def conv1d_wino_pack_weight(w: torch.Tensor, device) -> torch.Tensor:
    w = w.detach().float().cpu().contiguous()
    c_out, c_in, k = w.shape
    u = torch.empty(3 * ((k + 2) // 3) * c_in * c_out, dtype=torch.float32, device=device)
    _check(_lib.rvc_conv1d_wino_pack_weight(w.data_ptr(), c_out, c_in, k, u.data_ptr(), _stream()), "rvc_conv1d_wino_pack_weight")
    return u


def conv1d_wino_forward(x, u_packed, bias, c_out, k, dilation=1, slope_in=1.0, res=None, acc=None, out_scale=1.0, out=None):
    x = _dev_f32(x, "x")
    b, c_in, length = x.shape
    y = out if out is not None else torch.empty((b, c_out, length), dtype=torch.float32, device=x.device)
    _check(_lib.rvc_conv1d_wino_forward(x.data_ptr(), u_packed.data_ptr(), bias.data_ptr() if bias is not None else None,
                                        res.data_ptr() if res is not None else None,
                                        acc.data_ptr() if acc is not None else None, y.data_ptr(), b, c_in, c_out, length, k,
                                        dilation, float(slope_in), float(out_scale), _stream()), "rvc_conv1d_wino_forward")
    return y


def conv1d_winobf_pack_weight(w: torch.Tensor, device) -> torch.Tensor:
    w = w.detach().float().cpu().contiguous()
    c_out, c_in, k = w.shape
    n = c_size_t()
    _check(_lib.rvc_conv1d_winobf_weight_bytes(c_out, c_in, k, ctypes.byref(n)), "rvc_conv1d_winobf_weight_bytes")
    u = torch.empty(n.value // 2, dtype=torch.int16, device=device)
    _check(_lib.rvc_conv1d_winobf_pack_weight(w.data_ptr(), c_out, c_in, k, u.data_ptr(), _stream()), "rvc_conv1d_winobf_pack_weight")
    return u


def conv1d_winobf_forward(x, u_packed, bias, c_out, k, dilation=1, slope_in=1.0, res=None, acc=None, out_scale=1.0, out=None):
    x = _dev_f32(x, "x")
    b, c_in, length = x.shape
    y = out if out is not None else torch.empty((b, c_out, length), dtype=torch.float32, device=x.device)
    _check(_lib.rvc_conv1d_winobf_forward(x.data_ptr(), u_packed.data_ptr(), bias.data_ptr() if bias is not None else None,
                                          res.data_ptr() if res is not None else None,
                                          acc.data_ptr() if acc is not None else None, y.data_ptr(), b, c_in, c_out, length, k,
                                          dilation, float(slope_in), float(out_scale), _stream()), "rvc_conv1d_winobf_forward")
    return y


def resblock_bf16x3_pack_weight(w1: torch.Tensor, w2: torch.Tensor, device, bf16_taps: bool = False) -> torch.Tensor:
    w1 = w1.detach().float().cpu().contiguous()
    w2 = w2.detach().float().cpu().contiguous()
    c, c_in, k = w1.shape
    if c != c_in or w2.shape != w1.shape:
        raise NativeError(f"resblock pair: square convs of one shape expected, got {tuple(w1.shape)} and {tuple(w2.shape)}")
    stem = "rvc_resblock_bf16w" if bf16_taps else "rvc_resblock_bf16x3"
    n = c_size_t()
    _check(getattr(_lib, stem + "_weight_bytes")(c, k, ctypes.byref(n)), stem + "_weight_bytes")
    u = torch.empty(n.value // 2, dtype=torch.int16, device=device)
    _check(getattr(_lib, stem + "_pack_weight")(w1.data_ptr(), w2.data_ptr(), c, k, u.data_ptr(), _stream()), stem + "_pack_weight")
    return u


def resblock_bf16x3_forward(x, u_packed, b1, b2, k, dilation=1, slope=0.1, acc=None, out_scale=1.0, out=None, bf16_taps: bool = False):
    x = _dev_f32(x, "x")
    b, c, length = x.shape
    y = out if out is not None else torch.empty_like(x)
    if y.data_ptr() == x.data_ptr():
        raise NativeError("resblock pair: x and y must not alias")
    name = "rvc_resblock_bf16w_forward" if bf16_taps else "rvc_resblock_bf16x3_forward"
    _check(getattr(_lib, name)(x.data_ptr(), u_packed.data_ptr(), b1.data_ptr() if b1 is not None else None,
                               b2.data_ptr() if b2 is not None else None, acc.data_ptr() if acc is not None else None,
                               y.data_ptr(), b, c, length, k, dilation, float(slope), float(out_scale), _stream()), name)
    return y


def _conv1d_direct_pack(stem: str, label: str, w: torch.Tensor, device) -> torch.Tensor:
    w = w.detach().float().cpu().contiguous()
    c, c_in, k = w.shape
    if c != c_in:
        raise NativeError(f"{label}: a square conv expected, got {tuple(w.shape)}")
    n = c_size_t()
    _check(getattr(_lib, stem + "_weight_bytes")(c, k, ctypes.byref(n)), stem + "_weight_bytes")
    u = torch.empty(n.value // 2, dtype=torch.int16, device=device)
    _check(getattr(_lib, stem + "_pack_weight")(w.data_ptr(), c, k, u.data_ptr(), _stream()), stem + "_pack_weight")
    return u


def _conv1d_direct_forward(stem: str, label: str, x, u_packed, bias, k, dilation, slope_in, res, acc, out_scale, out):
    x = _dev_f32(x, "x")
    b, c, length = x.shape
    y = out if out is not None else torch.empty_like(x)
    if y.data_ptr() == x.data_ptr():
        raise NativeError(f"{label}: x and y must not alias")
    _check(getattr(_lib, stem + "_forward")(x.data_ptr(), u_packed.data_ptr(), bias.data_ptr() if bias is not None else None,
                                            res.data_ptr() if res is not None else None, acc.data_ptr() if acc is not None else None,
                                            y.data_ptr(), b, c, length, k, dilation, float(slope_in), float(out_scale), _stream()),
           stem + "_forward")
    return y


def conv1d_bf16w_pack_weight(w: torch.Tensor, device) -> torch.Tensor:
    return _conv1d_direct_pack("rvc_conv1d_bf16w", "conv1d_bf16w", w, device)


def conv1d_bf16w_forward(x, u_packed, bias, k, dilation=1, slope_in=1.0, res=None, acc=None, out_scale=1.0, out=None):
    return _conv1d_direct_forward("rvc_conv1d_bf16w", "conv1d_bf16w", x, u_packed, bias, k, dilation, slope_in, res, acc, out_scale, out)


def conv1d_f16x2_pack_weight(w: torch.Tensor, device) -> torch.Tensor:
    return _conv1d_direct_pack("rvc_conv1d_f16x2", "conv1d_f16x2", w, device)


def conv1d_f16x2_forward(x, u_packed, bias, k, dilation=1, slope_in=1.0, res=None, acc=None, out_scale=1.0, out=None):
    return _conv1d_direct_forward("rvc_conv1d_f16x2", "conv1d_f16x2", x, u_packed, bias, k, dilation, slope_in, res, acc, out_scale, out)


def upsample_bf16x3_pack_weight(up_w: torch.Tensor, noise_w, bias, rate: int, nc_stride: int, device):
    up_w = up_w.detach().float().cpu().contiguous()
    c_in, c_out, ksize = up_w.shape
    nc_k, nw = 0, None
    if noise_w is not None:
        nw = noise_w.detach().float().cpu().reshape(c_out, -1).contiguous()
        nc_k = nw.shape[1]
    b = bias.detach().float().cpu().contiguous() if bias is not None else None
    n = c_size_t()
    _check(_lib.rvc_upsample_bf16x3_weight_bytes(c_in, c_out, rate, ksize, nc_k, nc_stride, ctypes.byref(n)), "rvc_upsample_bf16x3_weight_bytes")
    u = torch.empty(n.value // 2, dtype=torch.int16, device=device)
    _check(_lib.rvc_upsample_bf16x3_pack_weight(up_w.data_ptr(), nw.data_ptr() if nw is not None else None, b.data_ptr() if b is not None else None,
                                                c_in, c_out, rate, ksize, nc_k, nc_stride, u.data_ptr(), _stream()), "rvc_upsample_bf16x3_pack_weight")
    return u, (nw.to(device) if nw is not None else None), (b.to(device) if b is not None else None)


def upsample_bf16x3_forward(x, har, packed, c_out, rate, ksize, pad, nc_stride=1, nc_pad=0, slope=0.1):
    u, nw, bias = packed
    x = _dev_f32(x, "x")
    b, c_in, length = x.shape
    l_out = (length - 1) * rate - 2 * pad + ksize
    y = torch.empty((b, c_out, l_out), dtype=torch.float32, device=x.device)
    if har is not None:
        har = _dev_f32(har, "har")
    _check(_lib.rvc_upsample_bf16x3_forward(x.data_ptr(), har.data_ptr() if har is not None else None, har.shape[-1] if har is not None else 0,
                                            u.data_ptr(), bias.data_ptr() if bias is not None else None,
                                            y.data_ptr(), b, c_in, c_out, length, rate, ksize, pad, nw.shape[1] if nw is not None else 0, nc_stride,
                                            nc_pad, float(slope), _stream()), "rvc_upsample_bf16x3_forward")
    return y


def resblock_bf16x3_set_enabled(enabled: bool) -> None:
    _check(_lib.rvc_resblock_bf16x3_set_enabled(1 if enabled else 0), "rvc_resblock_bf16x3_set_enabled")


def gemm_bf16x3_pack_weight(w: torch.Tensor, device) -> torch.Tensor:
    w = w.detach().float().cpu().contiguous()
    taps = w.shape[2] if w.dim() == 3 else 1
    m, k_total = w.shape[0], w.shape[1] * taps
    n = c_size_t()
    _check(_lib.rvc_gemm_bf16x3_weight_bytes(m, k_total, ctypes.byref(n)), "rvc_gemm_bf16x3_weight_bytes")
    a = torch.empty(n.value // 2, dtype=torch.int16, device=device)
    _check(_lib.rvc_gemm_bf16x3_pack_weight(w.data_ptr(), m, k_total, taps, a.data_ptr(), _stream()), "rvc_gemm_bf16x3_pack_weight")
    return a


def linear_bf16x3(x: torch.Tensor, a_packed: torch.Tensor, bias, out_features: int, act: str = "none", res=None) -> torch.Tensor:
    x = _dev_f32(x, "x")
    in_features = x.shape[-1]
    n_rows = x.numel() // in_features
    y = torch.empty(x.shape[:-1] + (out_features,), dtype=torch.float32, device=x.device)
    if res is not None:
        res = _dev_f32(res, "res")
        assert res.shape == y.shape
    _check(_lib.rvc_linear_bf16x3(x.data_ptr(), a_packed.data_ptr(), bias.data_ptr() if bias is not None else None,
                                  res.data_ptr() if res is not None else None, y.data_ptr(), n_rows, in_features, out_features,
                                  {"none": 0, "gelu": 1}[act], _stream()), "rvc_linear_bf16x3")
    return y


def glu_dwconv_silu(x: torch.Tensor, w: torch.Tensor, bias: torch.Tensor) -> torch.Tensor:
    x, w, bias = _dev_f32(x, "x"), _dev_f32(w, "w"), _dev_f32(bias, "bias")
    n_rows, c = x.shape[0], x.shape[1] // 2
    y = torch.empty((n_rows, c), dtype=torch.float32, device=x.device)
    _check(_lib.rvc_glu_dwconv_silu_f32(x.data_ptr(), w.data_ptr(), bias.data_ptr(), y.data_ptr(), n_rows, c, w.shape[1], _stream()),
           "rvc_glu_dwconv_silu_f32")
    return y


def layernorm_rows(x: torch.Tensor, gamma: torch.Tensor, beta: torch.Tensor, eps: float = 1e-5) -> torch.Tensor:
    x = _dev_f32(x, "x")
    f = x.shape[-1]
    y = torch.empty_like(x)
    _check(_lib.rvc_layernorm_rows_f32(x.data_ptr(), _dev_f32(gamma, "gamma").data_ptr(), _dev_f32(beta, "beta").data_ptr(), float(eps),
                                       y.data_ptr(), x.numel() // f, f, _stream()), "rvc_layernorm_rows_f32")
    return y


def groupnorm_lrelu(x: torch.Tensor, gamma: torch.Tensor, beta: torch.Tensor, groups: int, eps: float = 1e-5,
                    slope: float = 0.01) -> torch.Tensor:
    x = _dev_f32(x, "x")
    c, length = x.shape
    need = c_size_t()
    _check(_lib.rvc_groupnorm_workspace_bytes(c, length, groups, ctypes.byref(need)), "rvc_groupnorm_workspace_bytes")
    ws = _ws.get("groupnorm", need.value, x.device)
    y = torch.empty_like(x)
    _check(_lib.rvc_groupnorm_lrelu_f32(x.data_ptr(), _dev_f32(gamma, "gamma").data_ptr(), _dev_f32(beta, "beta").data_ptr(), groups,
                                        float(eps), float(slope), y.data_ptr(), c, length, ws.data_ptr(), ws.numel(), _stream()),
           "rvc_groupnorm_lrelu_f32")
    return y


def fcpe_decode(logits: torch.Tensor, cent_table: torch.Tensor, out_dims: int, threshold: float, f0_min: float,
                want_latent: bool = False):
    logits, cent_table = _dev_f32(logits, "logits"), _dev_f32(cent_table, "cent_table")
    n_rows, ld = logits.shape
    if cent_table.numel() != out_dims:
        raise NativeError(f"cent_table has {cent_table.numel()} entries, out_dims is {out_dims}")
    f0 = torch.empty(n_rows, dtype=torch.float32, device=logits.device)
    latent = torch.empty((n_rows, out_dims), dtype=torch.float32, device=logits.device) if want_latent else None
    _check(_lib.rvc_fcpe_decode_f32(logits.data_ptr(), cent_table.data_ptr(), out_dims, ld, float(threshold), float(f0_min),
                                    f0.data_ptr(), latent.data_ptr() if latent is not None else None, n_rows, _stream()),
           "rvc_fcpe_decode_f32")
    return f0, latent


def rows_padded(n_rows: int, tile: int = 128) -> int:
    return -(-n_rows // tile) * tile


def planes_empty(n_rows: int, features: int, device) -> torch.Tensor:
    return torch.empty((3, rows_padded(n_rows), features), dtype=torch.bfloat16, device=device)


def split_rows_bf16x3(x: torch.Tensor, out: torch.Tensor | None = None) -> torch.Tensor:
    x = _dev_f32(x, "x")
    n_rows, k = x.shape
    xs = out if out is not None else planes_empty(n_rows, k, x.device)
    _check(_lib.rvc_split_rows_bf16x3(x.data_ptr(), xs.data_ptr(), n_rows, xs.shape[1], k, _stream()), "rvc_split_rows_bf16x3")
    return xs


def linear_bf16x3_presplit(xs: torch.Tensor, a_packed: torch.Tensor, bias, n_rows: int, out_features: int, mode: str = "f32",
                           k_parts: int = 1, out: torch.Tensor | None = None) -> torch.Tensor:
    _, n_pad, in_features = xs.shape
    m = {"f32": 0, "gelu_planes": 1, "parts": 2, "gelu_f32": 3}[mode]
    if m in (0, 3):
        y = out if out is not None else torch.empty((n_rows, out_features), dtype=torch.float32, device=xs.device)
    elif m == 1:
        y = out if out is not None else torch.empty((3, n_pad, out_features), dtype=torch.bfloat16, device=xs.device)
    else:
        y = out if out is not None else torch.empty((k_parts, n_rows, out_features), dtype=torch.float32, device=xs.device)
    _check(_lib.rvc_linear_bf16x3_presplit(xs.data_ptr(), a_packed.data_ptr(), bias.data_ptr() if bias is not None else None,
                                           y.data_ptr() if m != 1 else None, y.data_ptr() if m == 1 else None, n_rows, n_pad,
                                           in_features, out_features, m, k_parts, _stream()), "rvc_linear_bf16x3_presplit")
    return y


def posconv_bf16x3_pack_weight(w: torch.Tensor, groups: int, device) -> torch.Tensor:
    w = w.detach().float().cpu().contiguous()
    d, cg, taps = w.shape
    need = c_size_t()
    _check(_lib.rvc_posconv_bf16x3_weight_bytes(d, groups, taps, ctypes.byref(need)), "rvc_posconv_bf16x3_weight_bytes")
    a = torch.empty(need.value // 2, dtype=torch.int16, device=device)
    with torch.cuda.device(a.device):
        _check(_lib.rvc_posconv_bf16x3_pack_weight(w.data_ptr(), d, groups, taps, a.data_ptr(), _stream()), "rvc_posconv_bf16x3_pack_weight")
    return a


def posconv_gelu_bf16x3(x: torch.Tensor, a_packed: torch.Tensor, bias, groups: int, taps: int, padding: int) -> torch.Tensor:
    x = _dev_f32(x, "x")
    t, d = x.shape
    y = torch.empty_like(x)
    _check(_lib.rvc_posconv_gelu_bf16x3(x.data_ptr(), a_packed.data_ptr(), bias.data_ptr() if bias is not None else None, y.data_ptr(),
                                        t, d, groups, taps, padding, _stream()), "rvc_posconv_gelu_bf16x3")
    return y


def hubert_conv0_frames_bf16x3(wav: torch.Tensor, w: torch.Tensor, gamma, beta, eps: float, stride: int = 5) -> tuple[torch.Tensor, int]:
    wav = _dev_f32(wav, "wav")
    w2 = _dev_f32(w.reshape(w.shape[0], -1), "w")
    c, taps = w2.shape
    n = wav.numel()
    frames = (n - taps) // stride + 1
    ys = planes_empty(frames, c, wav.device)
    need = c_size_t()
    _check(_lib.rvc_hubert_conv0_workspace_bytes(c, ctypes.byref(need)), "rvc_hubert_conv0_workspace_bytes")
    ws = _ws.get("hubert_conv0", need.value, wav.device)
    _check(_lib.rvc_hubert_conv0_frames_bf16x3(wav.data_ptr(), n, w2.data_ptr(), c, taps, stride,
                                               gamma.data_ptr() if gamma is not None else None,
                                               beta.data_ptr() if beta is not None else None, float(eps), ws.data_ptr(), ws.numel(),
                                               ys.data_ptr(), ys.shape[1], _stream()), "rvc_hubert_conv0_frames_bf16x3")
    return ys, frames


def conv1d_frames_bf16x3(xs: torch.Tensor, n_frames_in: int, a_packed: torch.Tensor, bias, out_channels: int, taps: int, stride: int,
                         mode: str = "gelu_planes") -> tuple[torch.Tensor, int]:
    _, n_pad_in, c = xs.shape
    m = {"f32": 0, "gelu_planes": 1, "gelu_f32": 3}[mode]
    frames = (n_frames_in - taps) // stride + 1
    if frames <= 0:
        raise NativeError("conv1d_frames_bf16x3: the input is shorter than one window")
    y = planes_empty(frames, out_channels, xs.device) if m == 1 else torch.empty((frames, out_channels), dtype=torch.float32, device=xs.device)
    _check(_lib.rvc_conv1d_frames_bf16x3(xs.data_ptr(), n_frames_in, n_pad_in, c, taps, stride, a_packed.data_ptr(),
                                         bias.data_ptr() if bias is not None else None, y.data_ptr() if m != 1 else None,
                                         y.data_ptr() if m == 1 else None, rows_padded(frames), out_channels, m, _stream()),
           "rvc_conv1d_frames_bf16x3")
    return y, frames


def bias_residual_layernorm_bf16x3(parts: torch.Tensor, bias, res, gamma, beta, eps: float, want_planes: bool = True,
                                   y: torch.Tensor | None = None, ys: torch.Tensor | None = None):
    n_parts, n_rows, m = parts.shape
    y = y if y is not None else torch.empty((n_rows, m), dtype=torch.float32, device=parts.device)
    if want_planes and ys is None:
        ys = planes_empty(n_rows, m, parts.device)
    _check(_lib.rvc_bias_residual_layernorm_bf16x3(parts.data_ptr(), n_parts, bias.data_ptr() if bias is not None else None,
                                                   res.data_ptr() if res is not None else None,
                                                   gamma.data_ptr() if gamma is not None else None,
                                                   beta.data_ptr() if beta is not None else None, float(eps), y.data_ptr(),
                                                   ys.data_ptr() if ys is not None else None, n_rows, ys.shape[1] if ys is not None else n_rows,
                                                   m, _stream()), "rvc_bias_residual_layernorm_bf16x3")
    return y, ys


def conv1d_bf16x3(x: torch.Tensor, a_packed: torch.Tensor, bias, c_out: int, k: int, stride: int = 1, padding: int = 0,
                  act: str = "none") -> torch.Tensor:
    x = _dev_f32(x, "x")
    b, c_in, l_in = x.shape
    l_out = max((l_in + 2 * padding - k) // stride + 1, 0)
    y = torch.empty((b, c_out, l_out), dtype=torch.float32, device=x.device)
    if y.numel() == 0:
        return y
    _check(_lib.rvc_conv1d_bf16x3(x.data_ptr(), a_packed.data_ptr(), bias.data_ptr() if bias is not None else None, y.data_ptr(), b,
                                  c_in, c_out, l_in, k, stride, padding, {"none": 0, "gelu": 1}[act], _stream()), "rvc_conv1d_bf16x3")
    return y


def conv2d_pack_weight(w: torch.Tensor, device) -> torch.Tensor:
    w = w.detach().float().cpu().contiguous()
    c_out, c_in, kh, kw = w.shape
    n = c_size_t()
    _check(_lib.rvc_conv2d_packed_floats(c_out, c_in, kh, kw, ctypes.byref(n)), "rvc_conv2d_packed_floats")
    out = torch.empty(n.value, dtype=torch.float32, device=device)
    _check(_lib.rvc_conv2d_pack_weight(w.data_ptr(), c_out, c_in, kh, kw, out.data_ptr(), _stream()), "rvc_conv2d_pack_weight")
    return out


def conv2d_supported(c_in: int, width: int) -> bool:
    return c_in % 8 == 0 and 4 <= width <= 128 and width & (width - 1) == 0


def conv2d_forward(x, w_packed, bias, c_out, ksize=3, relu=False, res=None, out=None):
    x = _dev_f32(x, "x")
    b, c_in, h, wd = x.shape
    y = out if out is not None else torch.empty((b, c_out, h, wd), dtype=torch.float32, device=x.device)
    need = c_size_t()
    _check(_lib.rvc_conv2d_workspace_bytes(b, c_in, c_out, h, wd, ksize, ksize, ctypes.byref(need)), "rvc_conv2d_workspace_bytes")
    ws = _ws.get("conv2d", need.value, x.device) if need.value else None
    _check(_lib.rvc_conv2d_forward(x.data_ptr(), w_packed.data_ptr(), bias.data_ptr() if bias is not None else None,
                                   res.data_ptr() if res is not None else None, y.data_ptr(), b, c_in, c_out, h, wd, ksize, ksize,
                                   1 if relu else 0, ws.data_ptr() if ws is not None else None, need.value, _stream()),
           "rvc_conv2d_forward")
    return y


def conv2d_bf16x3_supported(c_in: int, c_out: int, height: int, width: int) -> bool:
    return bool(_lib.rvc_conv2d_bf16x3_supported(c_in, c_out, height, width))


def conv2d_bf16x3_packable(c_in: int, c_out: int) -> bool:
    m_pad = (c_out + 31) // 32 * 32
    return c_in % 16 == 0 and (m_pad in (32, 64) or m_pad % 128 == 0)


def conv2d_bf16x3_pack_weight(w: torch.Tensor, device) -> torch.Tensor:
    w = w.detach().float().cpu().contiguous()
    c_out, c_in, kh, kw = w.shape
    n = c_size_t()
    _check(_lib.rvc_conv2d_bf16x3_weight_bytes(c_out, c_in, kh, kw, ctypes.byref(n)), "rvc_conv2d_bf16x3_weight_bytes")
    out = torch.empty(n.value // 2, dtype=torch.int16, device=device)
    _check(_lib.rvc_conv2d_bf16x3_pack_weight(w.data_ptr(), c_out, c_in, kh, kw, out.data_ptr(), _stream()), "rvc_conv2d_bf16x3_pack_weight")
    return out


def conv2d_bf16x3_forward(x, u, bias, c_out, relu=False, res=None, out=None):
    x = _dev_f32(x, "x")
    b, c_in, h, wd = x.shape
    y = out if out is not None else torch.empty((b, c_out, h, wd), dtype=torch.float32, device=x.device)
    need = c_size_t()
    _check(_lib.rvc_conv2d_bf16x3_workspace_bytes(b, c_in, c_out, h, wd, ctypes.byref(need)), "rvc_conv2d_bf16x3_workspace_bytes")
    ws = _ws.get("conv2d", need.value, x.device) if need.value else None
    _check(_lib.rvc_conv2d_bf16x3_forward(x.data_ptr(), u.data_ptr(), bias.data_ptr() if bias is not None else None,
                                          res.data_ptr() if res is not None else None, y.data_ptr(), b, c_in, c_out, h, wd,
                                          1 if relu else 0, ws.data_ptr() if ws is not None else None, need.value, _stream()),
           "rvc_conv2d_bf16x3_forward")
    return y


DEC_KINDS = {"HiFi-GAN": 0, "MRF HiFi-GAN": 1, "RefineGAN": 2}
DEC_ARITHMETIC = {"exact": 0, "fp16x2": 1}


class Decoder:

    def __init__(self, vocoder: str, sr: int, folded_weights: dict, *, in_channels=192, upsample_initial_channel=512,
                 gin_channels=256, upsample_rates=(12, 10, 2, 2), upsample_kernel_sizes=(24, 20, 4, 4),
                 res_kernel_sizes=(3, 7, 11), res_dilations=(1, 3, 5), weight_storage: str = "f32",
                 arithmetic: str = "exact"):
        if not torch.cuda.is_available():
            raise NativeError("rvc_amd.Decoder needs a HIP device (no CPU fallback)")
        if arithmetic not in DEC_ARITHMETIC:
            raise NativeError(f"rvc_amd.Decoder: arithmetic must be one of {sorted(DEC_ARITHMETIC)}, got {arithmetic!r}")
        cfg = DecoderConfig()
        cfg.kind = DEC_KINDS[vocoder]
        cfg.sample_rate = sr
        cfg.in_channels = in_channels
        cfg.upsample_initial_channel = upsample_initial_channel
        cfg.gin_channels = gin_channels
        cfg.n_ups = len(upsample_rates)
        for i, (u, k) in enumerate(zip(upsample_rates, upsample_kernel_sizes)):
            cfg.upsample_rates[i] = int(u)
            cfg.upsample_kernel_sizes[i] = int(k)
        cfg.n_res_kernels = len(res_kernel_sizes)
        for i, k in enumerate(res_kernel_sizes):
            cfg.res_kernel_sizes[i] = int(k)
        cfg.weight_storage = {"f32": 0, "bf16": 1}[weight_storage]
        cfg.n_res_dilations = len(res_dilations)
        for i, d in enumerate(res_dilations):
            cfg.res_dilations[i] = int(d)
        self._h = c_void_p()
        self.vocoder = vocoder
        _check(_lib.rvc_decoder_create(ctypes.byref(cfg), ctypes.byref(self._h)), "rvc_decoder_create")
        self.arithmetic = arithmetic
        if arithmetic != "exact":
            _check(_lib.rvc_decoder_set_arithmetic(self._h, DEC_ARITHMETIC[arithmetic]), "rvc_decoder_set_arithmetic")
        for name, t in folded_weights.items():
            t = t.detach().float().cpu().contiguous()
            shape = (c_int64 * t.dim())(*t.shape)
            _check(_lib.rvc_decoder_set_tensor(self._h, name.encode(), t.data_ptr(), shape, t.dim()),
                   f"rvc_decoder_set_tensor({name})")
        _check(_lib.rvc_decoder_finalize(self._h), "rvc_decoder_finalize")
        self.upp = _lib.rvc_decoder_upp(self._h)

    def __del__(self):
        h = getattr(self, "_h", None)
        if h and _lib is not None:
            _lib.rvc_decoder_destroy(h)
            self._h = None

    def set_concurrency_hint(self, utterances_in_flight: int):
        _check(_lib.rvc_decoder_set_concurrency_hint(self._h, int(utterances_in_flight)), "rvc_decoder_set_concurrency_hint")

    def set_branch_parallel(self, side_streams: int):
        _check(_lib.rvc_decoder_set_branch_parallel(self._h, int(side_streams)), "rvc_decoder_set_branch_parallel")

    def set_tap(self, stage: int, tap: torch.Tensor | None):
        _check(_lib.rvc_decoder_set_tap(self._h, stage, tap.data_ptr() if tap is not None else None),
               "rvc_decoder_set_tap")

    def forward(self, z: torch.Tensor, f0: torch.Tensor, g: torch.Tensor, *, src_randn: torch.Tensor,
                src_rand: torch.Tensor | None = None, adain_randn: torch.Tensor | None = None) -> torch.Tensor:
        z, f0, g = _dev_f32(z, "z"), _dev_f32(f0, "f0"), _dev_f32(g, "g")
        b, _, t = z.shape
        noise = DecoderNoise()
        src_randn = _dev_f32(src_randn, "src_randn")
        noise.src_randn_dev = src_randn.data_ptr()
        if src_rand is not None:
            src_rand = _dev_f32(src_rand, "src_rand")
            noise.src_rand_dev = src_rand.data_ptr()
        if adain_randn is not None:
            adain_randn = _dev_f32(adain_randn, "adain_randn")
            noise.adain_randn_dev = adain_randn.data_ptr()
        out = torch.empty((b, 1, t * self.upp), dtype=torch.float32, device=z.device)
        need = c_size_t()
        _check(_lib.rvc_decoder_workspace_bytes(self._h, b, t, ctypes.byref(need)), "rvc_decoder_workspace_bytes")
        ws = _ws.get("decoder", need.value, z.device)
        _check(_lib.rvc_decoder_forward(self._h, z.data_ptr(), f0.data_ptr(), g.data_ptr(), ctypes.byref(noise), b, t,
                                        out.data_ptr(), ws.data_ptr(), ws.numel(), _stream()), "rvc_decoder_forward")
        return out
```

codename-rvc-fork-3_amd/rvc_amd/infer/infer.py:

```python
from __future__ import annotations

import os
import time
import traceback
import wave

import numpy as np
import torch

from rvc_amd.configs.config import Config
from rvc_amd.infer.pipeline import Pipeline as VC
from rvc_amd.lib.audio import load_audio_infer
from rvc_amd.lib.algorithm.synthesizers import Synthesizer
from rvc_amd.lib.hubert import HubertModelWithFinalProj
from rvc_amd.lib.tools.split_audio import merge_audio, process_audio


def _write_wav(path, audio, sr):
    pcm = np.clip(audio, -1.0, 1.0)
    pcm = (pcm * 32767.0).astype("<i2")
    with wave.open(path, "wb") as f:
        f.setnchannels(1)
        f.setsampwidth(2)
        f.setframerate(int(sr))
        f.writeframes(pcm.tobytes())


class VoiceConverter:
    def __init__(self, device: str | None = None):
        self.config = Config(device)
        self.hubert_model = None
        self.last_embedder_model = None
        self.tgt_sr = None
        self.net_g = None
        self.vc = None
        self.cpt = None
        self.version = None
        self.n_spk = None
        self.use_f0 = None
        self.loaded_model = None
        self.dec_weight_dtype = "f32"
        self.dec_arithmetic = "exact"
        self.branch_streams = 0

    def load_hubert(self, embedder_model: str, embedder_model_custom: str = None):
        root = os.path.join(os.getcwd(), "rvc", "models", "embedders")
        path = embedder_model_custom if embedder_model == "custom" and embedder_model_custom else \
            os.path.join(root, {"chinese-hubert-base": "chinese_hubert_base", "japanese-hubert-base": "japanese_hubert_base",
                                "korean-hubert-base": "korean_hubert_base"}.get(embedder_model, embedder_model))
        sd = torch.load(os.path.join(path, "pytorch_model.bin"), map_location="cpu", weights_only=True)
        self.load_hubert_state_dict(sd)

    def load_hubert_state_dict(self, sd):
        self.hubert_model = HubertModelWithFinalProj(sd, device=self.config.device).float().eval()

    def get_vc(self, weight_root, sid):
        if not self.loaded_model or self.loaded_model != weight_root:
            self.load_model(weight_root)
            if self.cpt is not None:
                self.setup_network()
                self.setup_vc_instance()
            self.loaded_model = weight_root

    def load_model(self, weight_root):
        self.cpt = torch.load(weight_root, map_location="cpu", weights_only=True) if os.path.isfile(weight_root) else None

    def load_checkpoint_dict(self, cpt: dict):
        self.cpt = dict(cpt)
        self.cpt["config"] = list(cpt["config"])
        self.setup_network()
        self.setup_vc_instance()
        self.loaded_model = cpt.get("model_name", "<dict>")

    def setup_network(self):
        if self.cpt is not None:
            self.tgt_sr = self.cpt["config"][-1]
            self.cpt["config"][-3] = self.cpt["weight"]["emb_g.weight"].shape[0]
            self.use_f0 = self.cpt.get("f0", 1)
            self.version = self.cpt.get("version", "v1")
            self.text_enc_hidden_dim = 768 if self.version == "v2" else 256
            self.vocoder = self.cpt.get("vocoder", "HiFi-GAN")
            self.net_g = Synthesizer(*self.cpt["config"], use_f0=self.use_f0,
                                     text_enc_hidden_dim=self.text_enc_hidden_dim, vocoder=self.vocoder)
            del self.net_g.enc_q
            self.net_g.dec_weight_dtype = self.dec_weight_dtype
            self.net_g.dec_arithmetic = self.dec_arithmetic
            self.net_g.load_state_dict(self.cpt["weight"], strict=False)
            self.net_g = self.net_g.to(self.config.device).float()
            self.net_g.eval()

    def setup_vc_instance(self):
        if self.cpt is not None:
            self.vc = VC(self.tgt_sr, self.config)
            self.n_spk = self.cpt["config"][-3]

    def convert_array(self, audio: np.ndarray, *, index_path: str = "", pitch: int = 0, f0_file=None,
                      f0_method: str = "rmvpe", index_rate: float = 0.75, volume_envelope: float = 1,
                      protect: float = 0.5, hop_length: int = 128, f0_autotune: bool = False,
                      f0_autotune_strength: float = 1, filter_radius: float = 3.0, sid: int = 0, noise_seed=None,
                      split_audio: bool = False):
        if torch.is_tensor(audio):
            audio = audio.to(device=self.config.device, dtype=torch.float64)
            audio_max = audio.abs().max() / 0.95
            audio = torch.where(audio_max > 1, audio / audio_max, audio)
        else:
            audio = np.asarray(audio, dtype=np.float64).copy()
            audio_max = np.abs(audio).max() / 0.95
            if audio_max > 1:
                audio /= audio_max
        file_index = index_path.strip().strip('"').strip("\n").strip('"').strip().replace("trained", "added")

        def run(chunk):
            return self.vc.pipeline(model=self.hubert_model, net_g=self.net_g, sid=sid, audio=chunk, pitch=pitch,
                                    f0_method=f0_method, file_index=file_index, index_rate=index_rate,
                                    pitch_guidance=self.use_f0, filter_radius=filter_radius,
                                    volume_envelope=volume_envelope, version=self.version, protect=protect,
                                    hop_length=hop_length, f0_autotune=f0_autotune,
                                    f0_autotune_strength=f0_autotune_strength, f0_file=f0_file, noise_seed=noise_seed)

        if not split_audio:
            return run(audio)
        host = audio.cpu().numpy() if torch.is_tensor(audio) else audio
        chunks, intervals = process_audio(host, 16000)
        print(f"Audio split into {len(chunks)} chunks for processing.")
        converted = []
        for c in chunks:
            out = run(torch.from_numpy(np.ascontiguousarray(c)).to(audio.device) if torch.is_tensor(audio) else c)
            converted.append(out.cpu().numpy() if torch.is_tensor(out) else out)
            print(f"Converted audio chunk {len(converted)}")
        merged = merge_audio(chunks, converted, intervals, 16000, self.tgt_sr)
        return torch.from_numpy(merged).to(audio.device) if torch.is_tensor(audio) else merged

    def convert_batch(self, audios, *, inflight: int = 3, **kwargs):
        import threading
        audios = list(audios)
        results = [None] * len(audios)
        errors = []
        dev = self.config.device
        n_workers = max(1, min(int(inflight), len(audios)))
        if kwargs.get("noise_seed") is not None:
            n_workers = 1
        if not hasattr(self, "_batch_streams"):
            self._batch_streams = []
            self._batch_slots = {}
        while len(self._batch_streams) < n_workers:
            self._batch_streams.append(torch.cuda.Stream(device=dev))
        ready = torch.cuda.Event()
        ready.record(torch.cuda.current_stream(dev))
        lock, cursor = threading.Lock(), [0]

        def work(tid):
            slots = self._batch_slots.setdefault(tid, [dict(inp=None, out=None, up=None, done=None, idx=None, n=0) for _ in range(2)])
            for slot in slots:
                slot["idx"] = None

            def finish(slot):
                if slot["idx"] is not None:
                    slot["done"].synchronize()
                    results[slot["idx"]] = slot["out"][:slot["n"]].numpy().copy()
                    slot["idx"] = None

            try:
                stream = self._batch_streams[tid]
                stream.wait_event(ready)
                k = 0
                with torch.cuda.stream(stream):
                    while True:
                        with lock:
                            i = cursor[0]
                            cursor[0] += 1
                        if i >= len(audios):
                            break
                        a = audios[i]
                        long_host = not torch.is_tensor(a) and len(a) + self.vc.window > self.vc.t_max
                        if torch.is_tensor(a) or long_host or kwargs.get("split_audio") or kwargs.get("noise_seed") is not None:
                            results[i] = self.convert_array(a, **kwargs)
                            continue
                        slot = slots[k & 1]
                        k += 1
                        finish(slot)
                        a = np.ascontiguousarray(a, dtype=np.float64)
                        if slot["inp"] is None or slot["inp"].numel() < a.shape[0]:
                            slot["inp"] = torch.empty(max(a.shape[0], 1 << 16), dtype=torch.float64, pin_memory=True)
                            slot["up"] = torch.cuda.Event()
                        else:
                            slot["up"].synchronize()
                        slot["inp"][:a.shape[0]].numpy()[:] = a
                        a_dev = slot["inp"][:a.shape[0]].to(dev, non_blocking=True)
                        slot["up"].record(stream)
                        out = self.convert_array(a_dev, **kwargs).contiguous()
                        if slot["out"] is None or slot["out"].numel() < out.shape[0] or slot["out"].dtype != out.dtype:
                            slot["out"] = torch.empty(max(out.shape[0], 1 << 16), dtype=out.dtype, pin_memory=True)
                            slot["done"] = torch.cuda.Event()
                        slot["out"][:out.shape[0]].copy_(out, non_blocking=True)
                        slot["done"].record(stream)
                        slot["idx"], slot["n"] = i, out.shape[0]
                for slot in slots:
                    finish(slot)
            except Exception as error:
                errors.append(error)

        self.net_g.dec.set_concurrency_hint(n_workers)
        self.net_g.dec.set_branch_parallel(self.branch_streams or 0)
        threads = [threading.Thread(target=work, args=(t,)) for t in range(n_workers)]
        try:
            for t in threads:
                t.start()
            for t in threads:
                t.join()
        finally:
            self.net_g.dec.set_concurrency_hint(0)
        for stream in self._batch_streams[:n_workers]:
            torch.cuda.current_stream(dev).wait_stream(stream)
        if errors:
            raise errors[0]
        return results

    def convert_audio(self, audio_input_path: str, audio_output_path: str, model_path: str, index_path: str,
                      pitch: int = 0, f0_file: str = None, f0_method: str = "rmvpe", index_rate: float = 0.75,
                      volume_envelope: float = 1, protect: float = 0.5, hop_length: int = 128,
                      split_audio: bool = False, f0_autotune: bool = False, f0_autotune_strength: float = 1,
                      filter_radius: float = 3.0, embedder_model: str = "contentvec",
                      embedder_model_custom: str = None, clean_audio: bool = False, clean_strength: float = 0.5,
                      export_format: str = "WAV", post_process: bool = False, resample_sr: int = 0, sid: int = 0,
                      **kwargs):
        if not model_path:
            print("No model path provided. Aborting conversion.")
            return
        self.get_vc(model_path, sid)
        try:
            start_time = time.time()
            print(f"Converting audio '{audio_input_path}'...")
            if clean_audio or post_process or export_format != "WAV":
                raise NotImplementedError("clean_audio / post_process / non-WAV export are outside the hot path "
                                          "(SURVEY §2 items 2, 9)")
            audio = load_audio_infer(audio_input_path, 16000, device=self.config.device)
            if not self.hubert_model or embedder_model != self.last_embedder_model:
                self.load_hubert(embedder_model, embedder_model_custom)
                self.last_embedder_model = embedder_model
            if self.tgt_sr != resample_sr >= 16000:
                self.tgt_sr = resample_sr
            audio_opt = self.convert_array(audio, index_path=index_path, pitch=pitch, f0_file=f0_file,
                                           f0_method=f0_method, index_rate=index_rate,
                                           volume_envelope=volume_envelope, protect=protect, hop_length=hop_length,
                                           f0_autotune=f0_autotune, f0_autotune_strength=f0_autotune_strength,
                                           filter_radius=filter_radius, sid=sid, split_audio=split_audio)
            _write_wav(audio_output_path, audio_opt, self.tgt_sr)
            print(f"Conversion completed at '{audio_output_path}' in {time.time() - start_time:.2f} seconds.")
        except Exception as error:
            print(f"An error occurred during audio conversion: {error}")
            print(traceback.format_exc())

    def convert_audio_batch(self, audio_input_paths: str, audio_output_path: str, **kwargs):
        import threading
        inflight = max(1, int(kwargs.pop("inflight", 3)))
        try:
            start_time = time.time()
            print(f"Converting audio batch '{audio_input_paths}'...")
            audio_files = [f for f in sorted(os.listdir(audio_input_paths)) if f.lower().endswith("wav")]
            print(f"Detected {len(audio_files)} audio files for inference.")
            jobs = []
            for a in audio_files:
                new_input = os.path.join(audio_input_paths, a)
                new_output = os.path.join(audio_output_path, os.path.splitext(a)[0] + "_output.wav")
                if not os.path.exists(new_output):
                    jobs.append((new_input, new_output))
            if jobs:
                self.convert_audio(audio_input_path=jobs[0][0], audio_output_path=jobs[0][1], **kwargs)
            rest = jobs[1:]
            n_workers = min(inflight, len(rest))
            dev = self.config.device

            def work(tid):
                with torch.cuda.stream(torch.cuda.Stream(device=dev)):
                    for src, dst in rest[tid::n_workers]:
                        self.convert_audio(audio_input_path=src, audio_output_path=dst, **kwargs)

            threads = [threading.Thread(target=work, args=(t,)) for t in range(n_workers)]
            for t in threads:
                t.start()
            for t in threads:
                t.join()
            print(f"Batch conversion completed in {time.time() - start_time:.2f} seconds.")
        except Exception as error:
            print(f"An error occurred during audio batch conversion: {error}")
            print(traceback.format_exc())
```

codename-rvc-fork-3_amd/rvc_amd/infer/pipeline.py:

```python
from __future__ import annotations

import os
import threading

import numpy as np
import torch
import torch.nn.functional as F
from scipy import signal

from rvc_amd import _native
from rvc_amd.lib.predictors.FCPE import FCPE
from rvc_amd.lib.predictors.RMVPE import RMVPE0Predictor

FILTER_ORDER = 5
CUTOFF_FREQUENCY = 48
SAMPLE_RATE = 16000
bh, ah = signal.butter(N=FILTER_ORDER, Wn=CUTOFF_FREQUENCY, btype="high", fs=SAMPLE_RATE)


REF_FREQS = [49.00, 51.91, 55.00, 58.27, 61.74, 65.41, 69.30, 73.42, 77.78, 82.41, 87.31, 92.50, 98.00, 103.83, 110.00,
             116.54, 123.47, 130.81, 138.59, 146.83, 155.56, 164.81, 174.61, 185.00, 196.00, 207.65, 220.00, 233.08,
             246.94, 261.63, 277.18, 293.66, 311.13, 329.63, 349.23, 369.99, 392.00, 415.30, 440.00, 466.16, 493.88,
             523.25, 554.37, 587.33, 622.25, 659.25, 698.46, 739.99, 783.99, 830.61, 880.00, 932.33, 987.77, 1046.50]


class Autotune:

    def __init__(self, ref_freqs):
        self.ref_freqs = ref_freqs
        self.note_dict = self.ref_freqs

    def autotune_f0(self, f0, f0_autotune_strength):
        notes = np.asarray(self.note_dict, dtype=np.float64)
        f0 = np.asarray(f0, dtype=np.float64)
        closest = notes[np.argmin(np.abs(notes[None, :] - f0[:, None]), axis=1)]
        return f0 + (closest - f0) * f0_autotune_strength


class AudioProcessor:

    @staticmethod
    def _rms(y: torch.Tensor, frame_length: int, hop_length: int) -> torch.Tensor:
        y = F.pad(y, (frame_length // 2, frame_length // 2))
        return y.unfold(0, frame_length, hop_length).pow(2).mean(-1).sqrt()

    @staticmethod
    def change_rms(source_audio, source_rate: int, target_audio, target_rate: int, rate: float):
        as_numpy = not torch.is_tensor(target_audio)
        if as_numpy:
            target_audio = torch.from_numpy(np.ascontiguousarray(target_audio))
        if not torch.is_tensor(source_audio):
            source_audio = torch.from_numpy(np.ascontiguousarray(source_audio)).to(target_audio.device)
        n = target_audio.shape[0]
        rms1 = AudioProcessor._rms(source_audio, source_rate // 2 * 2, source_rate // 2).float()
        rms2 = AudioProcessor._rms(target_audio, target_rate // 2 * 2, target_rate // 2).float()
        rms1 = F.interpolate(rms1.view(1, 1, -1), size=n, mode="linear").view(-1)
        rms2 = F.interpolate(rms2.view(1, 1, -1), size=n, mode="linear").view(-1)
        rms2 = torch.maximum(rms2, torch.zeros_like(rms2) + 1e-6)
        out = target_audio * (torch.pow(rms1, 1 - rate) * torch.pow(rms2, rate - 1))
        return out.numpy() if as_numpy else out


def _reflect_pad(x: torch.Tensor, pad: int) -> torch.Tensor:
    n = x.shape[0]
    if pad < n:
        return F.pad(x.view(1, 1, -1), (pad, pad), mode="reflect").view(-1)
    period = 2 * (n - 1)
    m = torch.remainder(torch.arange(-pad, n + pad, device=x.device), period)
    return x[torch.where(m < n, m, period - m)]


class _PinnedIO:

    def __init__(self):
        self._buf = {}
        self._lock = threading.Lock()

    def _get(self, kind, n, dtype):
        key = (kind, torch.cuda.current_stream().cuda_stream)
        with self._lock:
            b = self._buf.get(key)
            if b is None or b.numel() < n or b.dtype != dtype:
                b = torch.empty(max(n, 1 << 16), dtype=dtype, pin_memory=True)
                self._buf[key] = b
        return b

    def upload(self, audio: np.ndarray, device) -> torch.Tensor:
        stage = self._get("in", audio.shape[0], torch.float64)[:audio.shape[0]]
        stage.numpy()[:] = audio
        return stage.to(device, non_blocking=True)

    def download(self, out: torch.Tensor) -> np.ndarray:
        stage = self._get("out", out.shape[0], out.dtype)[:out.shape[0]]
        stage.copy_(out, non_blocking=True)
        torch.cuda.current_stream().synchronize()
        return stage.numpy().copy()


_pinned = _PinnedIO()


class FeatureIndex:

    def __init__(self, big_npy, device, ivf=None, search_mode: str = "exact"):
        if isinstance(big_npy, np.ndarray):
            big_npy = torch.from_numpy(np.ascontiguousarray(big_npy, dtype=np.float32))
        self.vectors = big_npy.to(device=device, dtype=torch.float32).contiguous()
        self.aux = _native.knn_index_build(self.vectors)
        self.ntotal = int(self.vectors.shape[0])
        self.search_mode = search_mode
        self.ivf = None
        if ivf is not None:
            cent = torch.from_numpy(np.array(ivf.centroids, dtype=np.float32)).to(self.vectors.device)
            if int(ivf.nprobe) > 8:
                raise ValueError(f"IVF index asks for nprobe = {ivf.nprobe}; this build probes at most 8 lists (the reference writes 1)")
            self.ivf = {"centroids": cent, "aux": _native.knn_index_build(cent), "nprobe": max(1, int(ivf.nprobe)),
                        "lists": torch.from_numpy(np.array(ivf.padded_lists())).to(self.vectors.device)}
        elif search_mode == "ivf":
            raise ValueError("search_mode='ivf' needs the inverted lists of a faiss .index file")
        torch.cuda.current_stream(self.vectors.device).synchronize()

    def __bool__(self):
        return True

    def search_device(self, queries: torch.Tensor, k: int = 8):
        if self.search_mode == "ivf" and self.ivf is not None:
            _, near = _native.knn_search(self.ivf["centroids"], self.ivf["aux"], queries, k)
            probe = near[:, :self.ivf["nprobe"]]
            cand = self.ivf["lists"][probe.clamp_min(0)].masked_fill((probe < 0).unsqueeze(-1), -1)
            cand = cand.reshape(queries.shape[0], -1)
            return _native.knn_rank_candidates(self.vectors, self.aux, queries, cand, k)
        return _native.knn_search(self.vectors, self.aux, queries, k)

    def search(self, npy: np.ndarray, k: int = 8):
        d2, ids = self.search_device(torch.from_numpy(np.ascontiguousarray(npy, dtype=np.float32)).to(self.vectors.device), k)
        return d2.cpu().numpy(), ids.cpu().numpy()

    def reconstruct_n(self, start: int, n: int):
        return self.vectors[start:start + n].cpu().numpy()


def _load_index_file(path: str):
    if path.endswith(".npy"):
        return np.load(path), None
    from rvc_amd.lib.faiss_index import read_index
    ivf = read_index(path)
    return ivf.reconstruct_n(0, ivf.ntotal), ivf


class Pipeline:
    def __init__(self, tgt_sr, config):
        self.x_pad, self.x_query, self.x_center, self.x_max = config.x_pad, config.x_query, config.x_center, config.x_max
        self.sample_rate = 16000
        self.window = 160
        self.t_pad = self.sample_rate * self.x_pad
        self.t_pad_tgt = tgt_sr * self.x_pad
        self.t_pad2 = self.t_pad * 2
        self.t_query = self.sample_rate * self.x_query
        self.t_center = self.sample_rate * self.x_center
        self.t_max = self.sample_rate * self.x_max
        self.time_step = self.window / self.sample_rate * 1000
        self.f0_min, self.f0_max = 50, 1100
        self.f0_mel_min = 1127 * np.log(1 + self.f0_min / 700)
        self.f0_mel_max = 1127 * np.log(1 + self.f0_max / 700)
        self.device = config.device
        rmvpe_path = os.path.join("rvc", "models", "predictors", "rmvpe.pt")
        self.model_rmvpe = RMVPE0Predictor(rmvpe_path if os.path.isfile(rmvpe_path) else None, device=self.device)
        self.model_fcpe = None
        self._lock = threading.Lock()
        self._index_cache = {}
        self._preset_index = None
        self._f0_streams = {}
        self._coarse_thr = torch.from_numpy(self._coarse_thresholds()).to(self.device)
        self.index_search = "exact"
        self.debug_taps = None
        self.ref_freqs = REF_FREQS
        self.autotune = Autotune(self.ref_freqs)
        self.note_dict = self.autotune.note_dict

    def load_rmvpe_state_dict(self, sd):
        self.model_rmvpe.load_state_dict(sd)

    def load_fcpe_state_dict(self, ckpt):
        self.model_fcpe = FCPE(self.window, int(self.f0_min), int(self.f0_max), self.sample_rate, self.device, checkpoint=ckpt)

    def _fcpe(self):
        with self._lock:
            if self.model_fcpe is None:
                self.model_fcpe = FCPE(self.window, int(self.f0_min), int(self.f0_max), self.sample_rate, self.device,
                                       model_path=os.path.join("rvc", "models", "predictors", "fcpe.pt"))
            return self.model_fcpe

    def set_index(self, big_npy):
        self._preset_index = FeatureIndex(big_npy, self.device) if big_npy is not None else None

    def _get_index(self, file_index, index_rate):
        if index_rate <= 0:
            return None
        if file_index != "" and os.path.exists(file_index):
            key = (file_index, os.path.getmtime(file_index))
            with self._lock:
                index = self._index_cache.get(key)
                if index is None:
                    try:
                        big_npy, ivf = _load_index_file(file_index)
                        index = FeatureIndex(big_npy, self.device, ivf=ivf,
                                             search_mode=self.index_search if ivf is not None else "exact")
                    except Exception as error:
                        print(f"An error occurred reading the FAISS index: {error}")
                        return None
                    self._index_cache = {key: index}
            return index
        return self._preset_index

    def get_f0(self, input_audio_path, x, p_len, pitch, f0_method, filter_radius, hop_length, f0_autotune,
               f0_autotune_strength, inp_f0=None):
        if f0_method == "fcpe":
            f0 = self._fcpe().compute_f0(x, p_len=p_len, filter_radius=filter_radius)
            return self._postprocess_f0(f0, pitch, f0_autotune, inp_f0, f0_autotune_strength)
        if f0_method != "rmvpe":
            raise NotImplementedError(f"f0_method={f0_method!r}: only 'rmvpe' and 'fcpe' are implemented")
        if torch.is_tensor(x):
            f0 = self.model_rmvpe.infer_from_audio_device(x, thred=0.03).cpu().numpy()
        else:
            f0 = self.model_rmvpe.infer_from_audio(x, thred=0.03)
        return self._postprocess_f0(f0, pitch, f0_autotune, inp_f0, f0_autotune_strength)

    def _postprocess_f0(self, f0, pitch, f0_autotune=False, inp_f0=None, f0_autotune_strength=1):
        if f0_autotune is True:
            f0 = Autotune.autotune_f0(self, f0, f0_autotune_strength)
        f0 *= pow(2, pitch / 12)
        tf0 = self.sample_rate // self.window
        if inp_f0 is not None:
            delta_t = np.round((inp_f0[:, 0].max() - inp_f0[:, 0].min()) * tf0 + 1).astype("int16")
            replace_f0 = np.interp(list(range(delta_t)), inp_f0[:, 0] * 100, inp_f0[:, 1])
            shape = f0[self.x_pad * tf0: self.x_pad * tf0 + len(replace_f0)].shape[0]
            f0[self.x_pad * tf0: self.x_pad * tf0 + len(replace_f0)] = replace_f0[:shape]
        f0bak = f0.copy()
        f0_mel = 1127 * np.log(1 + f0 / 700)
        f0_mel[f0_mel > 0] = (f0_mel[f0_mel > 0] - self.f0_mel_min) * 254 / (self.f0_mel_max - self.f0_mel_min) + 1
        f0_mel[f0_mel <= 1] = 1
        f0_mel[f0_mel > 255] = 255
        return np.rint(f0_mel).astype(int), f0bak

    def _coarse_thresholds(self) -> np.ndarray:
        def coarse(f0):
            f0_mel = 1127 * np.log(1 + f0 / 700)
            f0_mel[f0_mel > 0] = (f0_mel[f0_mel > 0] - self.f0_mel_min) * 254 / (self.f0_mel_max - self.f0_mel_min) + 1
            f0_mel[f0_mel <= 1] = 1
            f0_mel[f0_mel > 255] = 255
            return np.rint(f0_mel).astype(np.int64)

        want = np.arange(2, 256, dtype=np.int64)
        lo = np.zeros(254, dtype=np.int64)
        hi = np.full(254, np.float64(1e6).view(np.int64), dtype=np.int64)
        while np.any(hi - lo > 1):
            mid = lo + (hi - lo) // 2
            ge = coarse(mid.view(np.float64).copy()) >= want
            hi, lo = np.where(ge, mid, hi), np.where(ge, lo, mid)
        return hi.view(np.float64)

    def _postprocess_f0_device(self, f0, pitch):
        f0 = f0 * pow(2, pitch / 12)
        coarse = torch.searchsorted(self._coarse_thr, f0, right=True) + 1
        return coarse, f0

    def _extract_features(self, model, audio0, index, big_npy, index_rate, version):
        if torch.is_tensor(audio0):
            feats = audio0.to(self.device).float()
        else:
            feats = torch.from_numpy(np.ascontiguousarray(audio0)).float().to(self.device)
        feats = feats.mean(-1) if feats.dim() == 2 else feats
        assert feats.dim() == 1, feats.dim()
        n_audio = feats.shape[0]
        feats = model(feats.view(1, -1))["last_hidden_state"]
        feats = model.final_proj(feats[0]).unsqueeze(0) if version == "v1" else feats
        feats0 = feats
        if index:
            feats = self._retrieve_speaker_embeddings(feats, index, big_npy, index_rate)
        feats = F.interpolate(feats.permute(0, 2, 1), scale_factor=2).permute(0, 2, 1)
        return feats, feats0, n_audio

    def _synthesize(self, net_g, sid, feats, feats0, n_audio, pitch, pitchf, protect, noise):
        p_len = min(n_audio // self.window, feats.shape[1])
        pitch, pitchf = pitch[:, :p_len], pitchf[:, :p_len]
        if protect < 0.5:
            feats0 = F.interpolate(feats0.permute(0, 2, 1), scale_factor=2).permute(0, 2, 1)
            pitchff = torch.where(pitchf < 1, torch.full_like(pitchf, protect),
                                  torch.where(pitchf > 0, torch.ones_like(pitchf), pitchf))
            feats = feats * pitchff.unsqueeze(-1) + feats0 * (1 - pitchff.unsqueeze(-1))
            feats = feats.to(feats0.dtype)
        p_len_t = torch.full((1,), p_len, device=self.device, dtype=torch.long)
        return net_g.infer(feats.float(), p_len_t, pitch, pitchf.float(), sid, noise=noise,
                           phone_lengths_host=[p_len])[0][0, 0]

    def voice_conversion(self, model, net_g, sid, audio0, pitch, pitchf, index, big_npy, index_rate, version, protect,
                         noise=None, as_tensor=False):
        with torch.no_grad():
            if pitch is None or pitchf is None:
                raise NotImplementedError("models without pitch guidance are not supported (SURVEY §2 item 3b)")
            feats, feats0, n_audio = self._extract_features(model, audio0, index, big_npy, index_rate, version)
            audio1 = self._synthesize(net_g, sid, feats, feats0, n_audio, pitch, pitchf, protect, noise)
            if as_tensor:
                return audio1
            return audio1.data.cpu().float().numpy()

    def _retrieve_speaker_embeddings(self, feats, index, big_npy, index_rate):
        if not isinstance(index, FeatureIndex):
            index = FeatureIndex(big_npy, self.device)
        q = feats[0].contiguous()
        if isinstance(getattr(self, "debug_taps", None), dict):
            self.debug_taps["knn_queries"] = q
        d2, ids = index.search_device(q, 8)
        return _native.knn_blend(index.vectors, q, d2, ids, float(index_rate)).unsqueeze(0)

    def pipeline(self, model, net_g, sid, audio, pitch, f0_method, file_index, index_rate, pitch_guidance,
                 filter_radius, volume_envelope, version, protect, hop_length, f0_autotune, f0_autotune_strength,
                 f0_file, *, noise_seed=None):
        if not pitch_guidance:
            raise NotImplementedError("models without pitch guidance are not supported (SURVEY §2 item 3b)")
        index = self._get_index(file_index, index_rate)
        big_npy = index.vectors if index is not None else None
        as_tensor = torch.is_tensor(audio)
        n_in = int(audio.shape[0])
        long_input = n_in + self.window > self.t_max
        if long_input:
            host = audio.detach().to(dtype=torch.float64).cpu().numpy() if as_tensor else np.ascontiguousarray(audio, dtype=np.float64)
            filtered = np.ascontiguousarray(signal.filtfilt(bh, ah, host))
            with torch.cuda.device(self.device):
                audio = _pinned.upload(filtered, self.device)
        else:
            if as_tensor:
                audio = audio.to(device=self.device, dtype=torch.float64)
            else:
                with torch.cuda.device(self.device):
                    audio = _pinned.upload(np.ascontiguousarray(audio, dtype=np.float64), self.device)
            audio = _native.filtfilt_order5(audio, bh, ah)
        n_audio = audio.shape[0]
        opt_ts = []
        if long_input:
            pad = F.pad(audio.view(1, 1, -1), (self.window // 2, self.window // 2), mode="reflect").view(-1)
            audio_sum = torch.zeros_like(audio)
            for i in range(self.window):
                audio_sum += pad[i: i + n_audio]
            ts = torch.arange(self.t_center, n_audio, self.t_center, device=self.device)
            if ts.numel():
                pos = ts[:, None] - self.t_query + torch.arange(2 * self.t_query, device=self.device)[None, :]
                inside = pos < n_audio
                seg = torch.where(inside, audio_sum[pos.clamp(max=n_audio - 1)].abs(), torch.full((), float("inf"), dtype=audio_sum.dtype, device=self.device))
                is_min = seg == seg.min(dim=1, keepdim=True).values
                first = torch.where(is_min, torch.arange(2 * self.t_query, device=self.device)[None, :], 2 * self.t_query).min(dim=1).values
                opt_ts = (ts - self.t_query + first).tolist()
        s = 0
        audio_opt = []
        t = None
        audio_pad = _reflect_pad(audio, self.t_pad)
        p_len = audio_pad.shape[0] // self.window
        inp_f0 = None
        if hasattr(f0_file, "name"):
            try:
                with open(f0_file.name, "r") as f:
                    lines = f.read().strip("\n").split("\n")
                inp_f0 = np.array([[float(i) for i in line.split(",")] for line in lines], dtype="float32")
            except Exception as error:
                print(f"An error occurred reading the F0 file: {error}")
        sid = torch.full((1,), int(sid), device=self.device, dtype=torch.long)
        audio_dev = audio_pad.float()

        noise = None
        if noise_seed is not None:
            torch.manual_seed(int(noise_seed))
            noise = "cpu"

        plan = []
        for t in opt_ts:
            t = t // self.window * self.window
            plan.append((slice(s, t + self.t_pad2 + self.window), slice(s // self.window, (t + self.t_pad2) // self.window)))
            s = t
        plan.append((slice(t, None), slice(t // self.window if t is not None else None, None)))

        with torch.no_grad():
            main = torch.cuda.current_stream()
            with self._lock:
                side = self._f0_streams.get(main.cuda_stream)
                if side is None:
                    side = self._f0_streams[main.cuda_stream] = torch.cuda.Stream(device=self.device)
            if f0_method not in ("rmvpe", "fcpe"):
                raise NotImplementedError(f"f0_method={f0_method!r}: only 'rmvpe' and 'fcpe' are implemented")
            if f0_method == "fcpe":
                pitch, pitchf = self.get_f0("input_audio_path", audio_dev, p_len, pitch, f0_method, filter_radius, hop_length,
                                            f0_autotune, f0_autotune_strength, inp_f0)
                pitch, pitchf = pitch[:p_len], pitchf[:p_len]
                pitch = torch.tensor(pitch, device=self.device).unsqueeze(0).long()
                pitchf = torch.tensor(pitchf, device=self.device).unsqueeze(0).float()
                feats_list = [self._extract_features(model, audio_dev[a], index, big_npy, index_rate, version) for a, _ in plan]
            else:
                gi, n_f0 = self.model_rmvpe.front_half_device(audio_dev)
                side.wait_stream(main)
                gi.record_stream(side)
                with torch.cuda.stream(side):
                    f0_dev = self.model_rmvpe.back_half_device(gi, n_f0, thred=0.03, taps=self.debug_taps)
                    if self.debug_taps is not None:
                        self.debug_taps["f0_raw"] = f0_dev
                    if inp_f0 is None and f0_autotune is not True:
                        pitch, pitchf = self._postprocess_f0_device(f0_dev, pitch)
                        pitch = pitch[:p_len].unsqueeze(0)
                        pitchf = pitchf[:p_len].unsqueeze(0).float()
                feats_list = [self._extract_features(model, audio_dev[a], index, big_npy, index_rate, version) for a, _ in plan]
                if inp_f0 is None and f0_autotune is not True:
                    main.wait_stream(side)
                    pitch.record_stream(main)
                    pitchf.record_stream(main)
                else:
                    with torch.cuda.stream(side):
                        f0_host = f0_dev.cpu().numpy()
                    pitch, pitchf = self._postprocess_f0(f0_host, pitch, f0_autotune, inp_f0, f0_autotune_strength)
                    pitch, pitchf = pitch[:p_len], pitchf[:p_len]
                    pitch = torch.tensor(pitch, device=self.device).unsqueeze(0).long()
                    pitchf = torch.tensor(pitchf, device=self.device).unsqueeze(0).float()
            for (feats, feats0, n_audio), (_, ps) in zip(feats_list, plan):
                if noise_seed is not None:
                    for _ in range(12):
                        torch.rand([])
                seg = self._synthesize(net_g, sid, feats, feats0, n_audio, pitch[:, ps], pitchf[:, ps], protect, noise)
                audio_opt.append(seg[self.t_pad_tgt: -self.t_pad_tgt])
        out = torch.cat(audio_opt) if len(audio_opt) > 1 else audio_opt[0]
        if volume_envelope != 1:
            out = AudioProcessor.change_rms(audio, self.sample_rate, out, self.sample_rate, volume_envelope)
        audio_max = out.abs().max() / 0.99
        out = torch.where(audio_max > 1, out / audio_max, out)
        if as_tensor:
            return out
        with torch.cuda.device(self.device):
            return _pinned.download(out.contiguous())
```

codename-rvc-fork-3_amd/rvc_amd/lib/algorithm/synthesizers.py:

```python
from __future__ import annotations

from typing import Dict, Optional

import numpy as np
import torch
import torch.nn.functional as F

from rvc_amd.lib.algorithm.encoders import prepare_attention_weights, text_encoder
from rvc_amd.lib.algorithm.residuals import flow_reverse, prepare_flow_weights
from rvc_amd.lib.algorithm.weights import fold_weight_norm


class Synthesizer:
    def __init__(self, spec_channels, segment_size, inter_channels, hidden_channels, filter_channels, n_heads,
                 n_layers, kernel_size, p_dropout, resblock, resblock_kernel_sizes, resblock_dilation_sizes,
                 upsample_rates, upsample_initial_channel, upsample_kernel_sizes, spk_embed_dim, gin_channels, sr,
                 use_f0, text_enc_hidden_dim=768, vocoder="HiFi-GAN", randomized=True, checkpointing=False, **kwargs):
        if not use_f0:
            raise NotImplementedError("models without pitch guidance are not supported (nor by the reference fork)")
        self.inter_channels, self.hidden_channels = inter_channels, hidden_channels
        self.n_heads, self.n_layers, self.kernel_size = n_heads, n_layers, kernel_size
        self.resblock_kernel_sizes = list(resblock_kernel_sizes)
        self.resblock_dilations = list(resblock_dilation_sizes[0])
        self.upsample_rates, self.upsample_kernel_sizes = list(upsample_rates), list(upsample_kernel_sizes)
        self.upsample_initial_channel = upsample_initial_channel
        self.gin_channels, self.sr, self.vocoder = gin_channels, int(sr), vocoder
        self.use_f0 = use_f0
        self.upp = int(np.prod(upsample_rates))
        self.enc_q = None
        self.device = torch.device("cpu")
        self.w: Dict[str, torch.Tensor] = {}
        self._dec_weights: Optional[Dict[str, torch.Tensor]] = None
        self.dec = None
        self.dec_weight_dtype = "f32"
        self.dec_arithmetic = "exact"

    def load_state_dict(self, state_dict, strict: bool = False):
        w = fold_weight_norm({k: v for k, v in state_dict.items() if not k.startswith("enc_q.")})
        self._dec_weights = {k[4:]: v for k, v in w.items() if k.startswith("dec.")}
        if self.dec_weight_dtype == "bf16":
            self._dec_weights = {k: v.float().bfloat16().float() for k, v in self._dec_weights.items()}
        self.w = {k: v for k, v in w.items() if not k.startswith("dec.")}
        self.dec = None
        if self.device.type == "cuda":
            self._to_device()
        return self

    def _to_device(self):
        from rvc_amd import _native
        self.w = {k: v.to(self.device) for k, v in self.w.items()}
        prepare_attention_weights(self.w, self.n_layers)
        prepare_flow_weights(self.w)
        torch.cuda.synchronize(self.device)
        if self._dec_weights is not None and self.dec is None:
            with torch.cuda.device(self.device):
                self.dec = _native.Decoder(self.vocoder, self.sr, self._dec_weights, in_channels=self.inter_channels,
                                           upsample_initial_channel=self.upsample_initial_channel,
                                           gin_channels=self.gin_channels, upsample_rates=self.upsample_rates,
                                           upsample_kernel_sizes=self.upsample_kernel_sizes,
                                           res_kernel_sizes=self.resblock_kernel_sizes,
                                           res_dilations=self.resblock_dilations, weight_storage=self.dec_weight_dtype,
                                           arithmetic=self.dec_arithmetic)

    def to(self, device):
        device = torch.device(device)
        if device.type != "cuda":
            raise RuntimeError("rvc_amd.Synthesizer runs on a HIP device only: the vocoder has no CPU path "
                               "(the CPU restatement lives in oracle/ and is test infrastructure)")
        self.device = device
        self._to_device()
        return self

    def float(self):
        return self

    def eval(self):
        return self

    def remove_weight_norm(self):
        return self

    def _adain_shapes(self, b, t):
        shapes, length, ch = [], t, self.upsample_initial_channel
        for r in self.upsample_rates:
            length *= r
            ch //= 2
            shapes += [(b, ch, length)] * (2 * len(self.resblock_kernel_sizes))
        return shapes

    def _draw(self, noise, b, t, t_dec=None):
        t_dec = t if t_dec is None else t_dec
        L = t_dec * self.upp
        dim = 9 if self.vocoder == "MRF HiFi-GAN" else 1
        refine = self.vocoder == "RefineGAN"
        dev = self.device
        if isinstance(noise, dict):
            return {k: (v.to(dev) if v is not None else None) for k, v in noise.items()}
        if noise == "cpu":
            z = torch.randn(b, self.inter_channels, t)
            if self.vocoder == "HiFi-GAN":
                src_rand = torch.rand(1, 1, 1)
                src_randn = torch.randn(b, L, 1)
            else:
                src_rand = torch.rand(b, dim)
                src_randn = torch.randn(b, L, dim)
            out = {"z": z.to(dev), "src_rand": src_rand.to(dev), "src_randn": src_randn.to(dev)}
            if refine:
                out["adain_randn"] = torch.cat([torch.randn(*sh).reshape(-1) for sh in self._adain_shapes(b, t_dec)]).to(dev)
            return out
        out = {"z": torch.randn(b, self.inter_channels, t, device=dev),
               "src_rand": torch.rand(b, dim, device=dev),
               "src_randn": torch.randn(b, L, dim, device=dev)}
        if refine:
            out["adain_randn"] = torch.randn(sum(int(np.prod(sh)) for sh in self._adain_shapes(b, t_dec)), device=dev)
        return out

    @torch.no_grad()
    def infer(self, phone, phone_lengths, pitch=None, nsff0=None, sid=None, rate=None, noise=None, *,
              phone_lengths_host=None):
        if self.dec is None:
            raise RuntimeError("Synthesizer.infer before load_state_dict(...).to('cuda:N')")
        w = self.w
        g = F.embedding(sid, w["emb_g.weight"]).unsqueeze(-1)
        m_p, logs_p, x_mask = text_encoder(w, phone, pitch, phone_lengths, hidden=self.hidden_channels,
                                           out_channels=self.inter_channels, n_heads=self.n_heads,
                                           n_layers=self.n_layers, kernel_size=self.kernel_size,
                                           lengths_host=phone_lengths_host)
        b, _, t = m_p.shape
        head = int(t * (1.0 - rate.item())) if rate is not None else 0
        nz = self._draw(noise, b, t, t - head)
        z_p = (m_p + torch.exp(logs_p) * nz["z"] * 0.66666) * x_mask
        if rate is not None:
            z_p, x_mask = z_p[:, :, head:], x_mask[:, :, head:]
            nsff0 = nsff0[:, head:]
        full = phone_lengths_host is not None and rate is None and all(int(n) == t for n in phone_lengths_host)
        z = flow_reverse(w, z_p, x_mask, g, half=self.inter_channels // 2, hidden=self.hidden_channels, full=full)
        o = self.dec.forward((z * x_mask).contiguous(), nsff0.float().contiguous(), g[:, :, 0].contiguous(),
                             src_randn=nz["src_randn"].contiguous(), src_rand=nz.get("src_rand"),
                             adain_randn=nz.get("adain_randn"))
        return o, x_mask, (z, z_p, m_p, logs_p)
```

include/rvc_amd.h:

```cpp
#ifndef RVC_AMD_H
#define RVC_AMD_H

#include <stddef.h>
#include <stdint.h>

#ifdef __cplusplus
extern "C" {
#endif

#define RVC_AMD_ABI_VERSION 4


int rvc_abi_version(void);
const char *rvc_last_error(void);


int rvc_knn_index_aux_bytes(int64_t n_rows, int dim, size_t *bytes);
int rvc_knn_index_build(const float *index_dev, int64_t n_rows, int dim, void *aux_dev, size_t aux_bytes, void *stream);

int rvc_knn_workspace_bytes(int64_t n_rows, int64_t n_queries, int dim, int k, size_t *bytes);

int rvc_knn_search(const float *index_dev, const void *aux_dev, int64_t n_rows, int dim,
                   const float *queries_dev, int64_t n_queries, int k,
                   float *out_d2_dev, int64_t *out_ids_dev,
                   void *workspace_dev, size_t workspace_bytes, void *stream);

int rvc_knn_rank_candidates(const float *index_dev, const void *aux_dev, int64_t n_rows, int dim, const float *queries_dev,
                            int64_t n_queries, const int32_t *cand_ids_dev, int cap, int k, float *out_d2_dev,
                            int64_t *out_ids_dev, void *stream);

int rvc_knn_set_mode(int mode);

int rvc_knn_blend(const float *index_dev, int dim, const float *feats_dev, const float *d2_dev,
                  const int64_t *ids_dev, int64_t n_queries, int k, float index_rate,
                  float *out_dev, void *stream);

int rvc_logmel_workspace_bytes(int batch, int64_t n_samples, size_t *bytes);
int rvc_logmel_rmvpe(const float *audio_dev, int batch, int64_t n_samples, float *mel_dev,
                     int64_t n_frames_padded, void *workspace_dev, size_t workspace_bytes, void *stream);

typedef struct rvc_mel rvc_mel;
int rvc_mel_create(int n_fft, int hop, int win_length, int pad, float mag_eps, float log_floor, const float *mel_host, int n_mels,
                   rvc_mel **out);
int rvc_mel_destroy(rvc_mel *h);
int rvc_mel_frames(const rvc_mel *h, int64_t n_samples, int64_t *n_frames);
int rvc_mel_workspace_bytes(const rvc_mel *h, int batch, int64_t n_samples, size_t *bytes);
int rvc_mel_forward(const rvc_mel *h, const float *audio_dev, int batch, int64_t n_samples, float *mel_dev, float *spec_dev,
                    void *workspace_dev, size_t workspace_bytes, void *stream);

int rvc_resample_poly_f64(const double *x_dev, int64_t n_in, int up, int down, const double *h_dev, int64_t n_taps,
                          double *y_dev, int64_t n_out, void *stream);

int rvc_filtfilt_workspace_bytes(int64_t n, size_t *bytes);
int rvc_filtfilt_order5(const double *x_dev, int64_t n, const double *coef_host, double *y_dev,
                        void *workspace_dev, size_t workspace_bytes, void *stream);

int rvc_bigru_workspace_bytes(int batch, size_t *bytes);
int rvc_bigru_status(const void *workspace_dev, int batch, int *n_redone_host, void *stream);
int rvc_bigru_set_spin_limit(unsigned polls);
int rvc_bigru_forward(const float *gi_dev, const float *whhT_dev, const float *bhh_dev, float *out_dev,
                      int batch, int64_t n_steps, int hidden, void *workspace_dev, size_t workspace_bytes, void *stream);

int rvc_attention_workspace_bytes(int batch, int64_t n_frames, int n_heads, int head_dim, size_t *bytes);
int rvc_attention_qkv_f32(const float *qkv_dev, const float *emb_rel_k_dev, const float *emb_rel_v_dev, float *out_dev,
                          int batch, int64_t n_frames, int n_heads, int head_dim, float scale, void *workspace_dev,
                          size_t workspace_bytes, void *stream);

int rvc_bias_relu_add_f32(const float *x_dev, const float *bias_dev, const float *res_dev, float *out_dev, int batch,
                          int channels, int64_t inner, int relu, void *stream);

int rvc_rownorm_gelu_f32(const float *x_dev, const float *gamma_dev, const float *beta_dev, float *out_dev, int batch, int channels,
                         int64_t length, float eps, void *stream);

int rvc_gate_tanh_sigmoid_f32(const float *x_dev, float *out_dev, int batch, int hidden, int64_t length, void *stream);

int rvc_set_concurrency_hint(int utterances_in_flight);

typedef struct rvc_decoder rvc_decoder;

enum { RVC_DEC_NSF = 0, RVC_DEC_MRF = 1, RVC_DEC_REFINE = 2 };

typedef struct rvc_decoder_config {
    int kind;
    int sample_rate;
    int in_channels;
    int upsample_initial_channel;
    int gin_channels;
    int n_ups;
    int upsample_rates[8];
    int upsample_kernel_sizes[8];
    int n_res_kernels;
    int res_kernel_sizes[4];
    int res_dilations[4];
    int n_res_dilations;
    int weight_storage;
} rvc_decoder_config;

int rvc_decoder_create(const rvc_decoder_config *cfg, rvc_decoder **out);
int rvc_decoder_set_tensor(rvc_decoder *dec, const char *name, const float *data_host,
                           const int64_t *shape, int ndim);
int rvc_decoder_finalize(rvc_decoder *dec);
int rvc_decoder_destroy(rvc_decoder *dec);

int rvc_decoder_upp(const rvc_decoder *dec);
int rvc_decoder_workspace_bytes(const rvc_decoder *dec, int batch, int64_t n_frames, size_t *bytes);

typedef struct rvc_decoder_noise {
    const float *src_rand_dev;
    const float *src_randn_dev;
    const float *adain_randn_dev;
} rvc_decoder_noise;

int rvc_decoder_forward(rvc_decoder *dec, const float *z_dev, const float *f0_dev, const float *g_dev,
                        const rvc_decoder_noise *noise, int batch, int64_t n_frames, float *out_dev,
                        void *workspace_dev, size_t workspace_bytes, void *stream);

int rvc_decoder_set_concurrency_hint(rvc_decoder *dec, int utterances_in_flight);

int rvc_decoder_set_branch_parallel(rvc_decoder *dec, int side_streams);

int rvc_decoder_set_arithmetic(rvc_decoder *dec, int mode);

int rvc_decoder_set_tap(rvc_decoder *dec, int stage, float *tap_dev);

int rvc_conv1d_pack_weight(const float *w_host, int c_out, int c_in, int k, float *w_packed_dev, void *stream);
int rvc_conv1d_forward(const float *x_dev, const float *w_packed_dev, const float *bias_dev,
                       const float *res_dev, const float *acc_dev, float *y_dev,
                       int batch, int c_in, int c_out, int64_t length, int k, int dilation,
                       float slope_in, float out_scale, void *stream);

typedef struct rvc_comm rvc_comm;
#define RVC_COMM_ID_BYTES 128
int rvc_comm_unique_id(unsigned char *id_host );
int rvc_comm_create(const unsigned char *id_host, int n_ranks, int rank, rvc_comm **out);
int rvc_comm_destroy(rvc_comm *comm);
int rvc_comm_info(const rvc_comm *comm, int *n_ranks, int *rank, int *rccl_version, char *library_path,
                  size_t library_path_bytes);
int rvc_index_broadcast(rvc_comm *comm, void *buf_dev, size_t bytes, int root, void *stream);
int rvc_checksum64(const void *buf_dev, size_t bytes, uint64_t *out2_dev, void *stream);

int rvc_conv2d_packed_floats(int c_out, int c_in, int kh, int kw, size_t *out);
int rvc_conv2d_pack_weight(const float *w_host, int c_out, int c_in, int kh, int kw, float *w_dev, void *stream);
int rvc_conv2d_workspace_bytes(int batch, int c_in, int c_out, int height, int width, int kh, int kw, size_t *out);
int rvc_conv2d_forward(const float *x_dev, const float *w_packed_dev, const float *bias_dev, const float *res_dev,
                       float *y_dev, int batch, int c_in, int c_out, int height, int width, int kh, int kw, int relu,
                       void *workspace_dev, size_t workspace_bytes, void *stream);

int rvc_conv2d_bf16x3_supported(int c_in, int c_out, int height, int width);
int rvc_conv2d_bf16x3_weight_bytes(int c_out, int c_in, int kh, int kw, size_t *bytes);
int rvc_conv2d_bf16x3_pack_weight(const float *w_host, int c_out, int c_in, int kh, int kw, void *u_dev, void *stream);
int rvc_conv2d_bf16x3_workspace_bytes(int batch, int c_in, int c_out, int height, int width, size_t *out);
int rvc_conv2d_bf16x3_forward(const float *x_dev, const void *u_dev, const float *bias_dev, const float *res_dev, float *y_dev,
                              int batch, int c_in, int c_out, int height, int width, int relu, void *workspace_dev,
                              size_t workspace_bytes, void *stream);

int rvc_conv1d_wino_pack_weight(const float *w_host, int c_out, int c_in, int k, float *u_dev, void *stream);
int rvc_conv1d_wino_forward(const float *x_dev, const float *u_dev, const float *bias_dev, const float *res_dev,
                            const float *acc_dev, float *y_dev, int batch, int c_in, int c_out, int64_t length, int k,
                            int dilation, float slope_in, float out_scale, void *stream);

int rvc_conv1d_winobf_weight_bytes(int c_out, int c_in, int k, size_t *bytes);
int rvc_conv1d_winobf_pack_weight(const float *w_host, int c_out, int c_in, int k, void *u_dev, void *stream);
int rvc_conv1d_winobf_forward(const float *x_dev, const void *u_dev, const float *bias_dev, const float *res_dev,
                              const float *acc_dev, float *y_dev, int batch, int c_in, int c_out, int64_t length, int k,
                              int dilation, float slope_in, float out_scale, void *stream);

int rvc_resblock_bf16x3_weight_bytes(int c, int k, size_t *bytes);
int rvc_resblock_bf16x3_pack_weight(const float *w1_host, const float *w2_host, int c, int k, void *u_dev, void *stream);
int rvc_resblock_bf16x3_forward(const float *x_dev, const void *u_dev, const float *b1_dev, const float *b2_dev,
                                const float *acc_dev, float *y_dev, int batch, int c, int64_t length, int k, int dilation,
                                float slope, float out_scale, void *stream);
int rvc_resblock_bf16w_weight_bytes(int c, int k, size_t *bytes);
int rvc_resblock_bf16w_pack_weight(const float *w1_host, const float *w2_host, int c, int k, void *u_dev, void *stream);
int rvc_resblock_bf16w_forward(const float *x_dev, const void *u_dev, const float *b1_dev, const float *b2_dev,
                               const float *acc_dev, float *y_dev, int batch, int c, int64_t length, int k, int dilation,
                               float slope, float out_scale, void *stream);
int rvc_conv1d_bf16w_weight_bytes(int c, int k, size_t *bytes);
int rvc_conv1d_bf16w_pack_weight(const float *w_host, int c, int k, void *u_dev, void *stream);
int rvc_conv1d_bf16w_forward(const float *x_dev, const void *u_dev, const float *bias_dev, const float *res_dev,
                             const float *acc_dev, float *y_dev, int batch, int c, int64_t length, int k, int dilation,
                             float slope_in, float out_scale, void *stream);
int rvc_conv1d_f16x2_weight_bytes(int c, int k, size_t *bytes);
int rvc_conv1d_f16x2_pack_weight(const float *w_host, int c, int k, void *u_dev, void *stream);
int rvc_conv1d_f16x2_forward(const float *x_dev, const void *u_dev, const float *bias_dev, const float *res_dev,
                             const float *acc_dev, float *y_dev, int batch, int c, int64_t length, int k, int dilation,
                             float slope_in, float out_scale, void *stream);
int rvc_upsample_bf16x3_weight_bytes(int c_in, int c_out, int rate, int ksize, int nc_k, int nc_stride, size_t *bytes);
int rvc_upsample_bf16x3_pack_weight(const float *up_w_host, const float *noise_w_host, const float *bias_host, int c_in, int c_out,
                                    int rate, int ksize, int nc_k, int nc_stride, void *u_dev, void *stream);
int rvc_upsample_bf16x3_forward(const float *x_dev, const float *har_dev, int64_t har_len, const void *u_dev, const float *bias_dev,
                                float *y_dev, int batch, int c_in, int c_out, int64_t length_in, int rate, int ksize, int pad,
                                int nc_k, int nc_stride, int nc_pad, float slope_in, void *stream);
int rvc_resblock_bf16x3_set_enabled(int enabled);

int rvc_gemm_bf16x3_weight_bytes(int m, int k_total, size_t *bytes);
int rvc_gemm_bf16x3_pack_weight(const float *w_host, int m, int k_total, int conv_taps, void *a_dev, void *stream);
int rvc_linear_bf16x3(const float *x_dev, const void *a_dev, const float *bias_dev, const float *res_dev, float *y_dev,
                      int64_t n_rows, int in_features, int out_features, int act, void *stream);
int rvc_conv1d_bf16x3(const float *x_dev, const void *a_dev, const float *bias_dev, float *y_dev, int batch, int c_in,
                      int c_out, int64_t l_in, int k, int stride, int padding, int act, void *stream);

int rvc_split_rows_bf16x3(const float *x_dev, void *xs_dev, int64_t n_rows, int64_t n_rows_padded, int k, void *stream);
int rvc_linear_bf16x3_presplit(const void *xs_dev, const void *a_dev, const float *bias_dev, float *y_dev, void *ys_dev,
                               int64_t n_rows, int64_t n_rows_padded, int in_features, int out_features, int mode, int k_parts,
                               void *stream);
int rvc_bias_residual_layernorm_bf16x3(const float *parts_dev, int n_parts, const float *bias_dev, const float *res_dev,
                                       const float *gamma_dev, const float *beta_dev, float eps, float *y_dev, void *ys_dev,
                                       int64_t n_rows, int64_t n_rows_padded, int features, void *stream);

int rvc_hubert_conv0_workspace_bytes(int channels, size_t *bytes);
int rvc_hubert_conv0_frames_bf16x3(const float *wav_dev, int64_t n_samples, const float *w_dev, int channels, int taps, int stride,
                                   const float *gamma_dev, const float *beta_dev, float eps, void *workspace_dev,
                                   size_t workspace_bytes, void *ys_dev, int64_t n_frames_padded, void *stream);
int rvc_conv1d_frames_bf16x3(const void *xs_dev, int64_t n_frames_in, int64_t n_frames_in_padded, int channels, int taps, int stride,
                             const void *a_dev, const float *bias_dev, float *y_dev, void *ys_dev, int64_t n_frames_out_padded,
                             int out_channels, int mode, void *stream);

int rvc_posconv_bf16x3_weight_bytes(int d, int groups, int taps, size_t *bytes);
int rvc_posconv_bf16x3_pack_weight(const float *w_host, int d, int groups, int taps, void *a_dev, void *stream);
int rvc_posconv_gelu_bf16x3(const float *x_dev, const void *a_dev, const float *bias_dev, float *y_dev, int64_t n_frames, int d,
                            int groups, int taps, int padding, void *stream);

int rvc_glu_dwconv_silu_f32(const float *x_dev, const float *w_dev, const float *bias_dev, float *y_dev, int64_t n_rows, int C, int K,
                            void *stream);
int rvc_layernorm_rows_f32(const float *x_dev, const float *gamma_dev, const float *beta_dev, float eps, float *y_dev, int64_t n_rows,
                           int F, void *stream);
int rvc_groupnorm_workspace_bytes(int C, int64_t L, int groups, size_t *bytes);
int rvc_groupnorm_lrelu_f32(const float *x_dev, const float *gamma_dev, const float *beta_dev, int groups, float eps, float slope,
                            float *y_dev, int C, int64_t L, void *workspace_dev, size_t workspace_bytes, void *stream);
int rvc_fcpe_decode_f32(const float *logits_dev, const float *cent_table_dev, int out_dims, int ld, float threshold, float f0_min,
                        float *f0_dev, float *latent_dev, int64_t n_rows, void *stream);

int rvc_kmeans_workspace_bytes(int64_t n_rows, int64_t n_centroids, int dim, size_t *bytes);
int rvc_kmeans_assign(const float *x_dev, int64_t n_rows, int dim, const float *centroids_dev, int64_t n_centroids,
                      int32_t *out_ids_dev, float *out_d2_dev, void *workspace_dev, size_t workspace_bytes, void *stream);
int rvc_kmeans_update(const float *x_dev, int64_t n_rows, int dim, const int32_t *order_dev, const int64_t *offsets_dev,
                      int64_t n_centroids, const float *old_centroids_dev, float *out_centroids_dev, void *workspace_dev,
                      size_t workspace_bytes, void *stream);

#ifdef __cplusplus
}
#endif
#endif
```

Baseline: 59.86 million.

## Run vocoder only on kept window plus receptive-field margin, skipping trimmed padding

Result: faster. 61.59 million (median of 6 runs) (+2.9%).

```diff
diff --git a/codename-rvc-fork-3_amd/csrc/decoder.h b/codename-rvc-fork-3_amd/csrc/decoder.h
--- a/codename-rvc-fork-3_amd/csrc/decoder.h
+++ b/codename-rvc-fork-3_amd/csrc/decoder.h
@@ -127,7 +127,7 @@
 int launch_cond_bias(const float *pre_b, const float *cond_w, const float *cond_b, const float *g, int batch, int gin, int c0,
                      float *out, hipStream_t stream);
 int launch_conv_post(const float *x, const float *w, float bias, int batch, int c_in, int64_t L, float slope, float *out,
-                     hipStream_t stream);
+                     hipStream_t stream, int64_t o_lo = 0, int64_t n_out = -1);
 
 int refine_finalize(rvc_decoder *d);
 size_t refine_workspace_bytes(const rvc_decoder *d, int batch, int64_t T);
diff --git a/codename-rvc-fork-3_amd/csrc/decoder.hip b/codename-rvc-fork-3_amd/csrc/decoder.hip
--- a/codename-rvc-fork-3_amd/csrc/decoder.hip
+++ b/codename-rvc-fork-3_amd/csrc/decoder.hip
@@ -54,11 +54,12 @@
 
 __global__ void __launch_bounds__(256)
 nsf_source_kernel(const float *__restrict__ f0, const float *__restrict__ carry, const float *__restrict__ randn,
-                  int64_t T, int upp, float sr, float lin_w, float lin_b, float *__restrict__ har) {
-    const int64_t L = T * upp;
+                  int64_t T, int64_t i0, int64_t Tw, int upp, float sr, float lin_w, float lin_b, float *__restrict__ har) {
+    const int64_t L = T * upp, Lw = Tw * upp;
     const int64_t b = blockIdx.y;
-    const int64_t t = (int64_t)blockIdx.x * blockDim.x + threadIdx.x;
-    if (t >= L) return;
+    const int64_t tw = (int64_t)blockIdx.x * blockDim.x + threadIdx.x;
+    if (tw >= Lw) return;
+    const int64_t t = tw + i0 * upp;
     const int64_t i = t / upp;
     const int j = (int)(t - i * upp);
     const float f = f0[b * T + i];
@@ -68,7 +69,7 @@
     const float uv = f > 0.f ? 1.f : 0.f;
     const float amp = __fadd_rn(__fmul_rn(uv, 0.003f), __fmul_rn(1.f - uv, (float)(0.1 / 3)));
     const float v = __fadd_rn(__fmul_rn(sine, uv), __fmul_rn(amp, randn[b * L + t]));
-    har[b * L + t] = tanhf(__fadd_rn(__fmul_rn(v, lin_w), lin_b));
+    har[b * Lw + tw] = tanhf(__fadd_rn(__fmul_rn(v, lin_w), lin_b));
 }
 
 
@@ -76,6 +77,7 @@
     const float *f0; const float *rand_ini; const float *randn; float *har;
     double *p1; double *p2; int *wraps; float *tot_unused;
     int64_t T; int upp; int dim; float sr;
+    int64_t i0, Tw;
     float lin_w[MRF_MAX_DIM]; float lin_b;
 };
 
@@ -181,7 +183,7 @@
 
 __global__ void __launch_bounds__(256) mrf_source_kernel(MrfSrcParams p) {
     __shared__ int wave_tot[4];
-    const int64_t i = blockIdx.x;
+    const int64_t i = blockIdx.x + p.i0;
     const int b = blockIdx.y;
     const int lane = threadIdx.x & 63, wave = threadIdx.x >> 6;
     const int64_t L = p.T * p.upp;
@@ -239,7 +241,7 @@
 #pragma unroll
     for (int it = 0; it < 4; ++it) {
         const int j = it * 256 + threadIdx.x;
-        if (it < n_it && j < p.upp) p.har[(int64_t)b * L + i * p.upp + j] = tanhf(out_acc[it] + p.lin_b);
+        if (it < n_it && j < p.upp) p.har[((int64_t)b * p.Tw + (i - p.i0)) * p.upp + j] = tanhf(out_acc[it] + p.lin_b);
     }
 }
 
@@ -271,13 +273,15 @@
 
 constexpr int POST_OUT = 4;
 __global__ void __launch_bounds__(256)
-conv_post_kernel(const float *__restrict__ x, const float *__restrict__ w, float bias, int c_in, int64_t L, float slope,
-                 float *__restrict__ out) {
+conv_post_kernel(const float *__restrict__ x, const float *__restrict__ w, float bias, int c_in, int64_t L, int64_t o_lo, int64_t n_out,
+                 float slope, float *__restrict__ out) {
     const int64_t b = blockIdx.y;
-    const int64_t t0 = ((int64_t)blockIdx.x * blockDim.x + threadIdx.x) * POST_OUT;
-    const int64_t blk0 = (int64_t)blockIdx.x * blockDim.x * POST_OUT;
+    const int64_t t0 = o_lo + ((int64_t)blockIdx.x * blockDim.x + threadIdx.x) * POST_OUT;
+    const int64_t blk0 = o_lo + (int64_t)blockIdx.x * blockDim.x * POST_OUT;
+    const int64_t o_hi = o_lo + n_out;
     const float *xb = x + b * c_in * L;
-    const bool fast = (L & 3) == 0 && (c_in & 3) == 0 && blk0 >= 4 && blk0 + (int64_t)blockDim.x * POST_OUT + 4 <= L;
+    const bool fast = (L & 3) == 0 && (c_in & 3) == 0 && ((o_lo | n_out) & 3) == 0 && blk0 >= 4 &&
+                      blk0 + (int64_t)blockDim.x * POST_OUT + 4 <= L && blk0 + (int64_t)blockDim.x * POST_OUT <= o_hi;
     if (fast) {
         float acc[POST_OUT];
 #pragma unroll
@@ -307,10 +311,10 @@
                 }
             }
         }
-        *reinterpret_cast<f32x4 *>(out + b * L + t0) = f32x4{tanhf(acc[0]), tanhf(acc[1]), tanhf(acc[2]), tanhf(acc[3])};
+        *reinterpret_cast<f32x4 *>(out + b * n_out + (t0 - o_lo)) = f32x4{tanhf(acc[0]), tanhf(acc[1]), tanhf(acc[2]), tanhf(acc[3])};
         return;
     }
-    if (t0 >= L) return;
+    if (t0 >= o_hi) return;
     float acc[POST_OUT];
 #pragma unroll
     for (int o = 0; o < POST_OUT; ++o) acc[o] = bias;
@@ -333,7 +337,7 @@
     }
 #pragma unroll
     for (int o = 0; o < POST_OUT; ++o)
-        if (t0 + o < L) out[b * L + t0 + o] = tanhf(acc[o]);
+        if (t0 + o < o_hi) out[b * n_out + (t0 - o_lo) + o] = tanhf(acc[o]);
 }
 
 int launch_unfold_src(const float *har, int batch, int64_t L, int64_t S, int64_t P, int k_valid, int k_rows, int64_t nq, float *V,
@@ -352,9 +356,10 @@
 }
 
 int launch_conv_post(const float *x, const float *w, float bias, int batch, int c_in, int64_t L, float slope, float *out,
-                     hipStream_t stream) {
-    hipLaunchKernelGGL(conv_post_kernel, dim3((unsigned)ceil_div(L, 256 * POST_OUT), batch), dim3(256), 0, stream, x, w, bias, c_in, L, slope,
-                       out);
+                     hipStream_t stream, int64_t o_lo, int64_t n_out) {
+    if (n_out < 0) n_out = L - o_lo;
+    hipLaunchKernelGGL(conv_post_kernel, dim3((unsigned)ceil_div(n_out, 256 * POST_OUT), batch), dim3(256), 0, stream, x, w, bias, c_in, L,
+                       o_lo, n_out, slope, out);
     RVC_LAUNCH_CHECK();
     return 0;
 }
@@ -665,14 +670,14 @@
     const int most = nk - 1 < MAX_BRANCH_LANES ? nk - 1 : MAX_BRANCH_LANES;
     return want < 0 || want > most ? most : want;
 }
-Layout make_layout(const rvc_decoder *d, int batch, int64_t T) {
+Layout make_layout(const rvc_decoder *d, int batch, int64_t T, int64_t Tw) {
     Layout l;
     Carve c;
-    const int64_t L = T * d->upp;
+    const int64_t L = Tw * d->upp;
     l.har = c.take((size_t)batch * L * 4);
     l.carry = c.take((size_t)batch * T * 4);
     l.biasp = c.take((size_t)batch * d->cfg.upsample_initial_channel * 4);
-    int64_t len = T, max_cl = (int64_t)d->cfg.upsample_initial_channel * T, max_v = 0;
+    int64_t len = Tw, max_cl = (int64_t)std::max(d->cfg.upsample_initial_channel, d->cfg.in_channels) * Tw, max_v = 0;
     for (const Stage &s : d->stages) {
         const int64_t nq = len + 1;
         max_v = std::max<int64_t>(max_v, (int64_t)s.vk_rows * nq);
@@ -696,7 +701,7 @@
 extern "C" int rvc_decoder_workspace_bytes(const rvc_decoder *dec, int batch, int64_t n_frames, size_t *bytes) {
     if (!dec || !bytes || batch <= 0 || n_frames <= 0) return fail("rvc_decoder_workspace_bytes: bad argument");
     if (!dec->finalized) return fail("rvc_decoder_workspace_bytes: decoder not finalized");
-    *bytes = dec->cfg.kind == RVC_DEC_REFINE ? refine_workspace_bytes(dec, batch, n_frames) : make_layout(dec, batch, n_frames).total;
+    *bytes = dec->cfg.kind == RVC_DEC_REFINE ? refine_workspace_bytes(dec, batch, n_frames) : make_layout(dec, batch, n_frames, n_frames).total;
     return 0;
 }
 
@@ -747,21 +752,43 @@
     return 0;
 }
 
-extern "C" int rvc_decoder_forward(rvc_decoder *d, const float *z_dev, const float *f0_dev, const float *g_dev,
-                                   const rvc_decoder_noise *noise, int batch, int64_t T, float *out_dev,
-                                   void *workspace_dev, size_t workspace_bytes, void *stream_) {
-    if (!d || !z_dev || !f0_dev || !g_dev || !noise || !out_dev || !workspace_dev) return fail("rvc_decoder_forward: null pointer");
-    ConcurrencyScope scope(d->concurrency.load(std::memory_order_relaxed));
-    if (!d->finalized) return fail("rvc_decoder_forward: decoder not finalized");
-    if (batch <= 0 || T <= 0) return fail("rvc_decoder_forward: empty batch");
-    if (!noise->src_randn_dev) return fail("rvc_decoder_forward: src_randn_dev is required");
-    if (d->cfg.kind == RVC_DEC_REFINE)
-        return refine_forward(d, z_dev, f0_dev, g_dev, noise, batch, T, out_dev, workspace_dev, workspace_bytes, (hipStream_t)stream_);
+namespace {
+int window_margin(const rvc_decoder_config &c) {
+    auto fdiv = [](int64_t a, int64_t b) { return a >= 0 ? a / b : -((-a + b - 1) / b); };
+    int64_t upp = 1;
+    for (int i = 0; i < c.n_ups; ++i) upp *= c.upsample_rates[i];
+    int64_t a = -3, b = upp - 1 + 3;
+    int64_t ha = 0, hb = upp - 1;
+    int64_t stride = 1;
+    for (int i = c.n_ups - 1; i >= 0; --i) {
+        const int rate = c.upsample_rates[i], ks = c.upsample_kernel_sizes[i];
+        const int pad = rate % 2 == 0 ? (ks - rate) / 2 : rate / 2 + rate % 2;
+        int64_t field = 0;
+        for (int m = 0; m < c.n_res_kernels; ++m) {
+            const int h = (c.res_kernel_sizes[m] - 1) / 2;
+            int64_t f = 0;
+            for (int j = 0; j < c.n_res_dilations; ++j) f += (int64_t)h * c.res_dilations[j] + h;
+            field = std::max(field, f);
+        }
+        a -= field; b += field;
+        const int64_t nc_k = stride == 1 ? 1 : stride * 2 - stride % 2, nc_pad = stride == 1 ? 0 : (nc_k - stride) / 2;
+        ha = std::min(ha, a * stride - nc_pad);
+        hb = std::max(hb, b * stride + nc_k - 1 - nc_pad);
+        a = -fdiv(-(a + pad - ks + 1), rate);
+        b = fdiv(b + pad, rate);
+        stride *= rate;
+    }
+    a -= 3; b += 3;
+    return (int)std::max(std::max(-a, b), std::max(-fdiv(ha, upp), fdiv(hb, upp)));
+}
+
+int decoder_run(rvc_decoder *d, const float *z_dev, const float *f0_dev, const float *g_dev, const rvc_decoder_noise *noise, int batch,
+                int64_t T, int64_t ext_lo, int64_t Tw, int64_t o_lo, int64_t n_out, float *out_dev, void *workspace_dev,
+                size_t workspace_bytes, hipStream_t stream) {
     const rvc_decoder_config &c = d->cfg;
     const bool mrf = c.kind == RVC_DEC_MRF;
     if (mrf && !noise->src_rand_dev) return fail("rvc_decoder_forward: src_rand_dev is required for the MRF decoder");
-    hipStream_t stream = (hipStream_t)stream_;
-    const Layout lay = make_layout(d, batch, T);
+    const Layout lay = make_layout(d, batch, T, Tw);
     if (workspace_bytes < lay.total) return fail("rvc_decoder_forward: workspace too small (%zu < %zu)", workspace_bytes, lay.total);
     char *ws = (char *)workspace_dev;
     float *har = (float *)(ws + lay.har);
@@ -773,14 +800,14 @@
     const int n_side = (lay.n_buf - 4) / 2;
     BranchLanes *lanes = nullptr;
     if (n_side > 0 && lanes_for(d, stream, n_side, &lanes)) return 1;
-    const int64_t L = T * d->upp;
+    const int64_t L = Tw * d->upp;
     const float sr = (float)c.sample_rate;
 
     if (!mrf) {
         hipLaunchKernelGGL(nsf_carry_kernel, dim3(batch), dim3(256), 0, stream, f0_dev, T, sr, (float)d->upp, carry);
         RVC_LAUNCH_CHECK();
         hipLaunchKernelGGL(nsf_source_kernel, dim3((unsigned)ceil_div(L, 256), batch), dim3(256), 0, stream, f0_dev, carry,
-                           noise->src_randn_dev, T, d->upp, sr, d->lin_w[0], d->lin_b, har);
+                           noise->src_randn_dev, T, ext_lo, Tw, d->upp, sr, d->lin_w[0], d->lin_b, har);
         RVC_LAUNCH_CHECK();
     } else {
         MrfSrcParams sp;
@@ -788,6 +815,7 @@
         sp.p1 = (double *)(ws + lay.p1); sp.p2 = (double *)(ws + lay.p2); sp.wraps = (int *)(ws + lay.wraps);
         sp.tot_unused = nullptr;
         sp.T = T; sp.upp = d->upp; sp.dim = d->dim; sp.sr = sr;
+        sp.i0 = ext_lo; sp.Tw = Tw;
         for (int h = 0; h < MRF_MAX_DIM; ++h) sp.lin_w[h] = d->lin_w[h];
         sp.lin_b = d->lin_b;
         hipLaunchKernelGGL(mrf_prefix_kernel<1>, dim3(batch), dim3(256), 0, stream, sp);
@@ -796,7 +824,7 @@
         RVC_LAUNCH_CHECK();
         hipLaunchKernelGGL(mrf_prefix_kernel<3>, dim3(batch), dim3(256), 0, stream, sp);
         RVC_LAUNCH_CHECK();
-        hipLaunchKernelGGL(mrf_source_kernel, dim3((unsigned)T, batch), dim3(256), 0, stream, sp);
+        hipLaunchKernelGGL(mrf_source_kernel, dim3((unsigned)Tw, batch), dim3(256), 0, stream, sp);
         RVC_LAUNCH_CHECK();
     }
     if (d->tap_stage == -1 && d->tap_dev)
@@ -807,16 +835,21 @@
                        c.gin_channels, c0, biasp);
     RVC_LAUNCH_CHECK();
     float *cur = buf[0];
+    if (Tw != T) {
+        RVC_HIP(hipMemcpy2DAsync(buf[1], (size_t)Tw * 4, z_dev + ext_lo, (size_t)T * 4, (size_t)Tw * 4, (size_t)batch * c.in_channels,
+                                 hipMemcpyDeviceToDevice, stream));
+        z_dev = buf[1];
+    }
     {
         ConvParams p;
-        p.x1 = z_dev; p.c1 = c.in_channels; p.slope1 = 1.f; p.x1_bstride = (int64_t)c.in_channels * T; p.l_in = T;
+        p.x1 = z_dev; p.c1 = c.in_channels; p.slope1 = 1.f; p.x1_bstride = (int64_t)c.in_channels * Tw; p.l_in = Tw;
         p.w = d->pre.w.p; p.bias = biasp; p.bias_bstride = c0;
-        p.y = cur; p.y_bstride = (int64_t)c0 * T; p.m_total = c0; p.c_out = c0; p.n_cols = T; p.l_out = T;
+        p.y = cur; p.y_bstride = (int64_t)c0 * Tw; p.m_total = c0; p.c_out = c0; p.n_cols = Tw; p.l_out = Tw;
         p.kw = 7; p.dil = 1; p.padl = 3; p.batch = batch;
         if (launch_conv(p, stream)) return 1;
     }
 
-    int64_t len = T;
+    int64_t len = Tw;
     const int nd = c.n_res_dilations, nk = c.n_res_kernels;
     for (int i = 0; i < c.n_ups; ++i) {
         Stage &s = d->stages[i];
@@ -950,5 +983,53 @@
             RVC_HIP(hipMemcpyAsync(d->tap_dev, cur, (size_t)batch * bs * 4, hipMemcpyDeviceToDevice, stream));
     }
     if (len != L) return fail("decoder: internal length mismatch (%lld vs %lld)", (long long)len, (long long)L);
-    return launch_conv_post(cur, d->post_w.p, d->post_b, batch, d->post_cin, L, 0.01f, out_dev, stream);
-}
+    return launch_conv_post(cur, d->post_w.p, d->post_b, batch, d->post_cin, L, 0.01f, out_dev, stream, o_lo, n_out);
+}
+}
+
+extern "C" int rvc_decoder_forward(rvc_decoder *d, const float *z_dev, const float *f0_dev, const float *g_dev,
+                                   const rvc_decoder_noise *noise, int batch, int64_t T, float *out_dev,
+                                   void *workspace_dev, size_t workspace_bytes, void *stream_) {
+    if (!d || !z_dev || !f0_dev || !g_dev || !noise || !out_dev || !workspace_dev) return fail("rvc_decoder_forward: null pointer");
+    ConcurrencyScope scope(d->concurrency.load(std::memory_order_relaxed));
+    if (!d->finalized) return fail("rvc_decoder_forward: decoder not finalized");
+    if (batch <= 0 || T <= 0) return fail("rvc_decoder_forward: empty batch");
+    if (!noise->src_randn_dev) return fail("rvc_decoder_forward: src_randn_dev is required");
+    if (d->cfg.kind == RVC_DEC_REFINE)
+        return refine_forward(d, z_dev, f0_dev, g_dev, noise, batch, T, out_dev, workspace_dev, workspace_bytes, (hipStream_t)stream_);
+    return decoder_run(d, z_dev, f0_dev, g_dev, noise, batch, T, 0, T, 0, T * d->upp, out_dev, workspace_dev, workspace_bytes,
+                       (hipStream_t)stream_);
+}
+
+extern "C" int rvc_decoder_window_margin(const rvc_decoder_config *cfg, int *frames) {
+    if (!cfg || !frames) return fail("rvc_decoder_window_margin: null pointer");
+    if (cfg->kind != RVC_DEC_NSF && cfg->kind != RVC_DEC_MRF && cfg->kind != RVC_DEC_REFINE)
+        return fail("rvc_decoder_window_margin: unknown decoder kind %d", cfg->kind);
+    if (cfg->n_ups < 1 || cfg->n_ups > 8) return fail("rvc_decoder_window_margin: n_ups out of range");
+    if (cfg->n_res_kernels < 1 || cfg->n_res_kernels > 4 || cfg->n_res_dilations < 1 || cfg->n_res_dilations > 4)
+        return fail("rvc_decoder_window_margin: resblock configuration out of range");
+    for (int i = 0; i < cfg->n_ups; ++i)
+        if (cfg->upsample_rates[i] < 1 || cfg->upsample_kernel_sizes[i] < cfg->upsample_rates[i])
+            return fail("rvc_decoder_window_margin: upsample stage %d: rate %d, kernel %d", i, cfg->upsample_rates[i], cfg->upsample_kernel_sizes[i]);
+    *frames = cfg->kind == RVC_DEC_REFINE ? -1 : window_margin(*cfg);
+    return 0;
+}
+
+extern "C" int rvc_decoder_forward_window(rvc_decoder *d, const float *z_dev, const float *f0_dev, const float *g_dev,
+                                          const rvc_decoder_noise *noise, int batch, int64_t T, int64_t keep_lo, int64_t keep_hi,
+                                          float *out_dev, void *workspace_dev, size_t workspace_bytes, void *stream_) {
+    if (!d || !z_dev || !f0_dev || !g_dev || !noise || !out_dev || !workspace_dev) return fail("rvc_decoder_forward_window: null pointer");
+    ConcurrencyScope scope(d->concurrency.load(std::memory_order_relaxed));
+    if (!d->finalized) return fail("rvc_decoder_forward_window: decoder not finalized");
+    if (batch <= 0 || T <= 0) return fail("rvc_decoder_forward_window: empty batch");
+    if (keep_lo < 0 || keep_lo >= keep_hi || keep_hi > T)
+        return fail("rvc_decoder_forward_window: frames [%lld, %lld) are not a window of [0, %lld)", (long long)keep_lo, (long long)keep_hi, (long long)T);
+    if (!noise->src_randn_dev) return fail("rvc_decoder_forward_window: src_randn_dev is required");
+    if (d->cfg.kind == RVC_DEC_REFINE)
+        return fail("rvc_decoder_forward_window: RefineGAN's receptive field is not covered; use rvc_decoder_forward");
+    if (d->tap_dev) return fail("rvc_decoder_forward_window: a debug tap is set (rvc_decoder_set_tap); use rvc_decoder_forward");
+    const int64_t m = window_margin(d->cfg);
+    const int64_t ext_lo = std::max<int64_t>(0, keep_lo - m), ext_hi = std::min<int64_t>(T, keep_hi + m);
+    return decoder_run(d, z_dev, f0_dev, g_dev, noise, batch, T, ext_lo, ext_hi - ext_lo, (keep_lo - ext_lo) * d->upp,
+                       (keep_hi - keep_lo) * d->upp, out_dev, workspace_dev, workspace_bytes, (hipStream_t)stream_);
+}
diff --git a/codename-rvc-fork-3_amd/rvc_amd/_native.py b/codename-rvc-fork-3_amd/rvc_amd/_native.py
--- a/codename-rvc-fork-3_amd/rvc_amd/_native.py
+++ b/codename-rvc-fork-3_amd/rvc_amd/_native.py
@@ -82,6 +82,9 @@
     "rvc_decoder_workspace_bytes": (c_int, [c_void_p, c_int, c_int64, POINTER(c_size_t)]),
     "rvc_decoder_forward": (c_int, [c_void_p, c_void_p, c_void_p, c_void_p, POINTER(DecoderNoise), c_int, c_int64,
                                     c_void_p, c_void_p, c_size_t, c_void_p]),
+    "rvc_decoder_window_margin": (c_int, [POINTER(DecoderConfig), POINTER(c_int)]),
+    "rvc_decoder_forward_window": (c_int, [c_void_p, c_void_p, c_void_p, c_void_p, POINTER(DecoderNoise), c_int, c_int64, c_int64,
+                                           c_int64, c_void_p, c_void_p, c_size_t, c_void_p]),
     "rvc_decoder_set_tap": (c_int, [c_void_p, c_int, c_void_p]),
     "rvc_decoder_set_concurrency_hint": (c_int, [c_void_p, c_int]),
     "rvc_decoder_set_branch_parallel": (c_int, [c_void_p, c_int]),
@@ -979,6 +982,36 @@
 DEC_ARITHMETIC = {"exact": 0, "fp16x2": 1}
 
 
+def _decoder_config(vocoder, sr, *, in_channels=192, upsample_initial_channel=512, gin_channels=256,
+                    upsample_rates=(12, 10, 2, 2), upsample_kernel_sizes=(24, 20, 4, 4), res_kernel_sizes=(3, 7, 11),
+                    res_dilations=(1, 3, 5), weight_storage: str = "f32") -> DecoderConfig:
+    cfg = DecoderConfig()
+    cfg.kind = DEC_KINDS[vocoder]
+    cfg.sample_rate = sr
+    cfg.in_channels = in_channels
+    cfg.upsample_initial_channel = upsample_initial_channel
+    cfg.gin_channels = gin_channels
+    cfg.n_ups = len(upsample_rates)
+    for i, (u, k) in enumerate(zip(upsample_rates, upsample_kernel_sizes)):
+        cfg.upsample_rates[i] = int(u)
+        cfg.upsample_kernel_sizes[i] = int(k)
+    cfg.n_res_kernels = len(res_kernel_sizes)
+    for i, k in enumerate(res_kernel_sizes):
+        cfg.res_kernel_sizes[i] = int(k)
+    cfg.weight_storage = {"f32": 0, "bf16": 1}[weight_storage]
+    cfg.n_res_dilations = len(res_dilations)
+    for i, d in enumerate(res_dilations):
+        cfg.res_dilations[i] = int(d)
+    return cfg
+
+
+def decoder_window_margin(vocoder: str, sr: int = 48000, **config) -> int:
+    cfg = _decoder_config(vocoder, sr, **config)
+    frames = c_int()
+    _check(_lib.rvc_decoder_window_margin(ctypes.byref(cfg), ctypes.byref(frames)), "rvc_decoder_window_margin")
+    return frames.value
+
+
 class Decoder:
 
     def __init__(self, vocoder: str, sr: int, folded_weights: dict, *, in_channels=192, upsample_initial_channel=512,
@@ -989,23 +1022,10 @@
             raise NativeError("rvc_amd.Decoder needs a HIP device (no CPU fallback)")
         if arithmetic not in DEC_ARITHMETIC:
             raise NativeError(f"rvc_amd.Decoder: arithmetic must be one of {sorted(DEC_ARITHMETIC)}, got {arithmetic!r}")
-        cfg = DecoderConfig()
-        cfg.kind = DEC_KINDS[vocoder]
-        cfg.sample_rate = sr
-        cfg.in_channels = in_channels
-        cfg.upsample_initial_channel = upsample_initial_channel
-        cfg.gin_channels = gin_channels
-        cfg.n_ups = len(upsample_rates)
-        for i, (u, k) in enumerate(zip(upsample_rates, upsample_kernel_sizes)):
-            cfg.upsample_rates[i] = int(u)
-            cfg.upsample_kernel_sizes[i] = int(k)
-        cfg.n_res_kernels = len(res_kernel_sizes)
-        for i, k in enumerate(res_kernel_sizes):
-            cfg.res_kernel_sizes[i] = int(k)
-        cfg.weight_storage = {"f32": 0, "bf16": 1}[weight_storage]
-        cfg.n_res_dilations = len(res_dilations)
-        for i, d in enumerate(res_dilations):
-            cfg.res_dilations[i] = int(d)
+        cfg = self._cfg = _decoder_config(vocoder, sr, in_channels=in_channels, upsample_initial_channel=upsample_initial_channel,
+                                          gin_channels=gin_channels, upsample_rates=upsample_rates,
+                                          upsample_kernel_sizes=upsample_kernel_sizes, res_kernel_sizes=res_kernel_sizes,
+                                          res_dilations=res_dilations, weight_storage=weight_storage)
         self._h = c_void_p()
         self.vocoder = vocoder
         _check(_lib.rvc_decoder_create(ctypes.byref(cfg), ctypes.byref(self._h)), "rvc_decoder_create")
@@ -1036,8 +1056,14 @@
         _check(_lib.rvc_decoder_set_tap(self._h, stage, tap.data_ptr() if tap is not None else None),
                "rvc_decoder_set_tap")
 
+    def window_margin(self) -> int:
+        frames = c_int()
+        _check(_lib.rvc_decoder_window_margin(ctypes.byref(self._cfg), ctypes.byref(frames)), "rvc_decoder_window_margin")
+        return frames.value
+
     def forward(self, z: torch.Tensor, f0: torch.Tensor, g: torch.Tensor, *, src_randn: torch.Tensor,
-                src_rand: torch.Tensor | None = None, adain_randn: torch.Tensor | None = None) -> torch.Tensor:
+                src_rand: torch.Tensor | None = None, adain_randn: torch.Tensor | None = None,
+                keep: tuple | None = None) -> torch.Tensor:
         z, f0, g = _dev_f32(z, "z"), _dev_f32(f0, "f0"), _dev_f32(g, "g")
         b, _, t = z.shape
         noise = DecoderNoise()
@@ -1049,10 +1075,17 @@
         if adain_randn is not None:
             adain_randn = _dev_f32(adain_randn, "adain_randn")
             noise.adain_randn_dev = adain_randn.data_ptr()
-        out = torch.empty((b, 1, t * self.upp), dtype=torch.float32, device=z.device)
         need = c_size_t()
         _check(_lib.rvc_decoder_workspace_bytes(self._h, b, t, ctypes.byref(need)), "rvc_decoder_workspace_bytes")
         ws = _ws.get("decoder", need.value, z.device)
+        if keep is not None:
+            lo, hi = int(keep[0]), int(keep[1])
+            out = torch.empty((b, 1, max(hi - lo, 0) * self.upp), dtype=torch.float32, device=z.device)
+            _check(_lib.rvc_decoder_forward_window(self._h, z.data_ptr(), f0.data_ptr(), g.data_ptr(), ctypes.byref(noise), b, t,
+                                                   lo, hi, out.data_ptr(), ws.data_ptr(), ws.numel(), _stream()),
+                   "rvc_decoder_forward_window")
+            return out
+        out = torch.empty((b, 1, t * self.upp), dtype=torch.float32, device=z.device)
         _check(_lib.rvc_decoder_forward(self._h, z.data_ptr(), f0.data_ptr(), g.data_ptr(), ctypes.byref(noise), b, t,
                                         out.data_ptr(), ws.data_ptr(), ws.numel(), _stream()), "rvc_decoder_forward")
         return out
diff --git a/codename-rvc-fork-3_amd/rvc_amd/infer/infer.py b/codename-rvc-fork-3_amd/rvc_amd/infer/infer.py
--- a/codename-rvc-fork-3_amd/rvc_amd/infer/infer.py
+++ b/codename-rvc-fork-3_amd/rvc_amd/infer/infer.py
@@ -41,6 +41,7 @@
         self.loaded_model = None
         self.dec_weight_dtype = "f32"
         self.dec_arithmetic = "exact"
+        self.trim_vocoder_pad = True
         self.branch_streams = 0
 
     def load_hubert(self, embedder_model: str, embedder_model_custom: str = None):
@@ -109,6 +110,8 @@
             if audio_max > 1:
                 audio /= audio_max
         file_index = index_path.strip().strip('"').strip("\n").strip('"').strip().replace("trained", "added")
+
+        self.vc.trim_vocoder_pad = bool(self.trim_vocoder_pad)
 
         def run(chunk):
             return self.vc.pipeline(model=self.hubert_model, net_g=self.net_g, sid=sid, audio=chunk, pitch=pitch,
diff --git a/codename-rvc-fork-3_amd/rvc_amd/infer/pipeline.py b/codename-rvc-fork-3_amd/rvc_amd/infer/pipeline.py
--- a/codename-rvc-fork-3_amd/rvc_amd/infer/pipeline.py
+++ b/codename-rvc-fork-3_amd/rvc_amd/infer/pipeline.py
@@ -174,6 +174,7 @@
         self._coarse_thr = torch.from_numpy(self._coarse_thresholds()).to(self.device)
         self.index_search = "exact"
         self.debug_taps = None
+        self.trim_vocoder_pad = True
         self.ref_freqs = REF_FREQS
         self.autotune = Autotune(self.ref_freqs)
         self.note_dict = self.autotune.note_dict
@@ -281,7 +282,7 @@
         feats = F.interpolate(feats.permute(0, 2, 1), scale_factor=2).permute(0, 2, 1)
         return feats, feats0, n_audio
 
-    def _synthesize(self, net_g, sid, feats, feats0, n_audio, pitch, pitchf, protect, noise):
+    def _synthesize(self, net_g, sid, feats, feats0, n_audio, pitch, pitchf, protect, noise, trim=0):
         p_len = min(n_audio // self.window, feats.shape[1])
         pitch, pitchf = pitch[:, :p_len], pitchf[:, :p_len]
         if protect < 0.5:
@@ -291,8 +292,17 @@
             feats = feats * pitchff.unsqueeze(-1) + feats0 * (1 - pitchff.unsqueeze(-1))
             feats = feats.to(feats0.dtype)
         p_len_t = torch.full((1,), p_len, device=self.device, dtype=torch.long)
-        return net_g.infer(feats.float(), p_len_t, pitch, pitchf.float(), sid, noise=noise,
-                           phone_lengths_host=[p_len])[0][0, 0]
+        upp = getattr(net_g, "upp", 0)
+        n_out = p_len * upp
+        window = (trim > 0 and self.trim_vocoder_pad and self.debug_taps is None and upp > 0 and n_out > 2 * trim and feats.shape[1] == p_len
+                  and getattr(net_g, "vocoder", None) != "RefineGAN")
+        if not window:
+            seg = net_g.infer(feats.float(), p_len_t, pitch, pitchf.float(), sid, noise=noise, phone_lengths_host=[p_len])[0][0, 0]
+            return seg[trim:-trim] if trim > 0 else seg
+        keep_lo, keep_hi = trim // upp, -((trim - n_out) // upp)
+        seg = net_g.infer(feats.float(), p_len_t, pitch, pitchf.float(), sid, noise=noise, phone_lengths_host=[p_len],
+                          keep_frames=(keep_lo, keep_hi))[0][0, 0]
+        return seg[trim - keep_lo * upp: n_out - trim - keep_lo * upp]
 
     def voice_conversion(self, model, net_g, sid, audio0, pitch, pitchf, index, big_npy, index_rate, version, protect,
                          noise=None, as_tensor=False):
@@ -422,8 +432,8 @@
                 if noise_seed is not None:
                     for _ in range(12):
                         torch.rand([])
-                seg = self._synthesize(net_g, sid, feats, feats0, n_audio, pitch[:, ps], pitchf[:, ps], protect, noise)
-                audio_opt.append(seg[self.t_pad_tgt: -self.t_pad_tgt])
+                audio_opt.append(self._synthesize(net_g, sid, feats, feats0, n_audio, pitch[:, ps], pitchf[:, ps], protect, noise,
+                                                  trim=self.t_pad_tgt))
         out = torch.cat(audio_opt) if len(audio_opt) > 1 else audio_opt[0]
         if volume_envelope != 1:
             out = AudioProcessor.change_rms(audio, self.sample_rate, out, self.sample_rate, volume_envelope)
diff --git a/codename-rvc-fork-3_amd/rvc_amd/lib/algorithm/synthesizers.py b/codename-rvc-fork-3_amd/rvc_amd/lib/algorithm/synthesizers.py
--- a/codename-rvc-fork-3_amd/rvc_amd/lib/algorithm/synthesizers.py
+++ b/codename-rvc-fork-3_amd/rvc_amd/lib/algorithm/synthesizers.py
@@ -117,7 +117,7 @@
 
     @torch.no_grad()
     def infer(self, phone, phone_lengths, pitch=None, nsff0=None, sid=None, rate=None, noise=None, *,
-              phone_lengths_host=None):
+              phone_lengths_host=None, keep_frames=None):
         if self.dec is None:
             raise RuntimeError("Synthesizer.infer before load_state_dict(...).to('cuda:N')")
         w = self.w
@@ -137,5 +137,5 @@
         z = flow_reverse(w, z_p, x_mask, g, half=self.inter_channels // 2, hidden=self.hidden_channels, full=full)
         o = self.dec.forward((z * x_mask).contiguous(), nsff0.float().contiguous(), g[:, :, 0].contiguous(),
                              src_randn=nz["src_randn"].contiguous(), src_rand=nz.get("src_rand"),
-                             adain_randn=nz.get("adain_randn"))
+                             adain_randn=nz.get("adain_randn"), keep=keep_frames if rate is None else None)
         return o, x_mask, (z, z_p, m_p, logs_p)
diff --git a/include/rvc_amd.h b/include/rvc_amd.h
--- a/include/rvc_amd.h
+++ b/include/rvc_amd.h
@@ -114,6 +114,11 @@
 int rvc_decoder_forward(rvc_decoder *dec, const float *z_dev, const float *f0_dev, const float *g_dev,
                         const rvc_decoder_noise *noise, int batch, int64_t n_frames, float *out_dev,
                         void *workspace_dev, size_t workspace_bytes, void *stream);
+
+int rvc_decoder_window_margin(const rvc_decoder_config *cfg, int *frames);
+int rvc_decoder_forward_window(rvc_decoder *dec, const float *z_dev, const float *f0_dev, const float *g_dev,
+                               const rvc_decoder_noise *noise, int batch, int64_t n_frames, int64_t keep_lo, int64_t keep_hi,
+                               float *out_dev, void *workspace_dev, size_t workspace_bytes, void *stream);
 
 int rvc_decoder_set_concurrency_hint(rvc_decoder *dec, int utterances_in_flight);
 
```
